# leosampaio/sketchformer

Hardware: AMD Instinct MI355X
Metric: stroke-tokens/sec training step, d_model=128 L=200 B=128, 1/2/4/8 GPU (higher is better)
Workload: dtype f32; 1 GPU; cfg2: sketch-transformer-tf2 4L/8H/d128/dff512 L=200 V=1004 C=345 dropout=0.1, fwd+bwd+Adam(WarmupDecay); global_batch=128, per_gpu_batch=128, seq_len=200, parallelism=dp1, hip_graph=0, dense_gemm_arithmetic=fp32 operands split exactly into 3 bf16 pieces, 6 product...

## Files before the change

### include/skf.h

```cpp
#ifndef SKF_H_
#define SKF_H_
#include <stddef.h>
#include <stdint.h>
#ifdef __cplusplus
extern "C" {
#endif

typedef void* skf_stream_t;

#define SKF_OK 0
#define SKF_EINVAL (-1)
#define SKF_EUNSUPPORTED (-2)
#define SKF_EHIP (-3)

const char* skf_last_error(void);
int skf_version(void);
int skf_device_info(char* name_host, size_t name_len, int* n_devices_host);

int skf_profiler_enable(int on);
int skf_profiler_report(char* buf_host, size_t len);

#define SKF_PREC_F32 0
#define SKF_PREC_BF16X3 3
#define SKF_PREC_BF16X6 6
// ... 25 lines not shown
                      int splits, float* bias_grad, int bias_grad_accumulate, void* workspace, size_t workspace_bytes,
                      int precision, const int* row_blocks, int row_block_rows, void* relu_bits_out, const void* relu_bits_in,
                      skf_stream_t stream);
int skf_gemm_ln_residual_supported(int M, int N, int K, int precision);
int skf_gemm_ln_residual_f32(int M, int N, int K, const float* A, int lda, const float* W, int ldw, const float* bias,
                             const float* x, const float* gamma, const float* beta, float* z, float* out, float* stats,
                             float rate, unsigned site, const void* step_state, int precision, skf_stream_t stream);
int skf_ffn_fused_supported(int M, int d, int dff, int precision);
size_t skf_ffn_image_bytes(int d, int dff, int precision);
size_t skf_ffn_relu_bits_bytes(int M, int d, int dff, int precision);
int skf_ffn_weight_images(int n, const float* const* W1, const int* ld1, const float* const* W2, const int* ld2,
                          const int* transpose, void* const* images, int d, int dff, int precision, skf_stream_t stream);
int skf_ffn_fused_fwd_f32(int M, int d, int dff, const float* x, const void* image, const float* b1, const float* b2,
                          float* h, void* relu_bits_out, const float* gamma, const float* beta, float* z, float* out,
                          float* stats, float rate, unsigned site, const void* step_state, int precision, skf_stream_t stream);
int skf_ffn_fused_bwd_f32(int M, int d, int dff, const float* dy, const void* image_t, const void* relu_bits_in,
                          float* dh, float* dx, int accumulate, const int* row_blocks, int row_block_rows,
                          int precision, skf_stream_t stream);
int skf_ffn_fused_fwd_proj_f32(int M, int d, int dff, const float* x, const void* image, const float* b1, const float* b2,
                               float* h, void* relu_bits_out, const float* gamma, const float* beta, float* z, float* out,
                               float* stats, float rate, unsigned site, const void* step_state, const void* proj_image,
                               const float* proj_bias, int proj_n, float* proj_out, int precision, skf_stream_t stream);
typedef struct SkfFfnBlockFwd {
  uint32_t struct_size; int32_t M, d, dff, precision;
  const float* x; const void* image; const float* b1; const float* b2; float* h; void* relu_bits_out;
  const float* gamma; const float* beta; float* z; float* out; float* stats;
  float rate; uint32_t site; const void* step_state;
  const void* pre_image; const float* pre_bias; const float* pre_residual; const float* pre_gamma; const float* pre_beta;
  float* pre_z; float* pre_out; float* pre_stats; uint32_t pre_site; int32_t proj_n;
  const void* proj_image; const float* proj_bias; float* proj_out;
} SkfFfnBlockFwd;
int skf_ffn_block_fwd_f32(const SkfFfnBlockFwd* block, skf_stream_t stream);
int skf_ffn_fused_ln_partials(int M);
int skf_ffn_fused_bwd_ln_f32(int M, int d, int dff, const float* dout, const float* z, const float* stats, const float* gamma,
                             float rate, unsigned site, const void* step_state, const void* image_t, const void* relu_bits_in,
                             float* dy, float* dh, float* dx, float* ln_partials, size_t ln_partials_bytes,
                             const int* row_blocks, int row_block_rows, int precision, skf_stream_t stream);
size_t skf_dense_image_bytes(int K, int N, int precision);
int skf_dense_weight_images(int n, const float* const* src, const int* ld, const int* transpose, const int* K, const int* N,
                            void* const* images, int precision, skf_stream_t stream);
int skf_layernorm_bwd_dgrad_supported(int M, int d, int precision);
int skf_layernorm_bwd_dgrad_partials(int M);
int skf_layernorm_bwd_dgrad_f32(int M, int d, const float* dout, const float* z, const float* stats, const float* gamma,
                                float rate, unsigned site, const void* step_state, const void* image_t, float* dz, float* dy,
                                float* da, float* ln_partials, size_t ln_partials_bytes, const int* row_blocks,
                                int row_block_rows, int precision, skf_stream_t stream);
int skf_layernorm_bwd_dgrad_lead_f32(int M, int d, const float* dout, const float* lead_a, const void* lead_image_t, const float* z,
                                     const float* stats, const float* gamma, float rate, unsigned site, const void* step_state,
                                     const void* image_t, float* dz, float* dy, float* da, float* ln_partials, size_t ln_partials_bytes,
                                     const int* row_blocks, int row_block_rows, int precision, skf_stream_t stream);
int skf_gemm_wgrad_partial_rows(int M, int N, int K, const float* A, int lda, const float* B, int ldb, int splits,
                                int with_bias_grad, float* slab, size_t slab_bytes, int* splits_used_host, int precision,
                                const int* row_blocks, int row_block_rows, skf_stream_t stream);
typedef struct SkfWgradProblem {
  const float* A; const float* B; float* slab; size_t slab_bytes; const int* row_blocks;
  int32_t M, N, K, lda, ldb, splits, with_bias_grad, row_block_rows, splits_used, pad;
} SkfWgradProblem;
int skf_gemm_wgrad_partial_group(SkfWgradProblem* probs, int n, int precision, skf_stream_t stream);
int skf_splitk_reduce(const float* slab, int splits, int M, int N, float* C, int ldc, int accumulate, float* bias_grad,
                      int bias_grad_accumulate, skf_stream_t stream);
int skf_splitk_reduce_blocks(int M, int N);
int skf_splitk_reduce_batch(const SkfReduceDesc* descs_dev, int ndesc, int total_blocks, skf_stream_t stream);

int skf_attention_fwd(const float* Q, int ldq, const float* K, int ldk, const float* V, int ldv,
                      const unsigned char* key_mask, int key_mask_ld, int causal, int B, int H, int Lq, int Lk, int dh,
                      float* O, int ldo, float* stats, int precision, skf_stream_t stream);
int skf_attention_bwd(const float* Q, int ldq, const float* K, int ldk, const float* V, int ldv, const float* O, int ldo,
                      const float* dO, int lddo, const float* stats, const unsigned char* key_mask, int key_mask_ld,
                      int causal, int B, int H, int Lq, int Lk, int dh, float* dQ, int lddq, float* dK, int lddk,
                      float* dV, int lddv, int precision, skf_stream_t stream);
int skf_attention_bwd_rows(const float* Q, int ldq, const float* K, int ldk, const float* V, int ldv, const float* O, int ldo,
                           const float* dO, int lddo, const float* stats, const unsigned char* key_mask, int key_mask_ld,
                           int causal, int B, int H, int Lq, int Lk, int dh, float* dQ, int lddq, float* dK, int lddk,
                           float* dV, int lddv, int precision, const int* q_live_len, skf_stream_t stream);
int skf_sample_order(const unsigned char* mask_a, int lda, int La, const unsigned char* mask_b, int ldb, int Lb, int B, int* order,
                     skf_stream_t stream);
int skf_attention_fwd_ordered(const float* Q, int ldq, const float* K, int ldk, const float* V, int ldv,
                              const unsigned char* key_mask, int key_mask_ld, int causal, int B, int H, int Lq, int Lk, int dh,
                              float* O, int ldo, float* stats, int precision, const int* sample_order, skf_stream_t stream);
int skf_attention_bwd_ordered(const float* Q, int ldq, const float* K, int ldk, const float* V, int ldv, const float* O, int ldo,
                              const float* dO, int lddo, const float* stats, const unsigned char* key_mask, int key_mask_ld,
                              int causal, int B, int H, int Lq, int Lk, int dh, float* dQ, int lddq, float* dK, int lddk,
                              float* dV, int lddv, int precision, const int* q_live_len, const int* sample_order, skf_stream_t stream);
int skf_attention_weights(const float* Q, int ldq, const float* K, int ldk, const unsigned char* key_mask, int key_mask_ld,
                          int causal, int B, int H, int Lq, int Lk, int dh, float* W, skf_stream_t stream);
int skf_attention_fwd_float_mask(const float* Q, int ldq, const float* K, int ldk, const float* V, int ldv, const float* mask,
                                 long mask_stride_b, long mask_stride_h, long mask_stride_q, int B, int H, int Lq, int Lk, int dh,
                                 float* O, int ldo, float* W, skf_stream_t stream);
int skf_row_mean(const float* a, const float* b, long rows, int cols, int mode, float* out, skf_stream_t stream);

int skf_embed_fwd(const long long* tokens, int tok_ld, int B, int L, const float* table, int vocab, int d,
                  const float* pos, float* out, float rate, unsigned site, const void* step_state, skf_stream_t stream);
int skf_embed_bwd(const long long* tokens, int tok_ld, int B, int L, const float* dx, int vocab, int d, float* dtable,
                  float rate, unsigned site, const void* step_state, skf_stream_t stream);
size_t skf_embed_sort_workspace_bytes(int B, int L, int vocab);
int skf_embed_sort(const long long* tokens, int tok_ld, int B, int L, int vocab, float* zero_table, int d, void* ws,
                   size_t ws_bytes, skf_stream_t stream);
int skf_embed_bwd_sorted(const void* ws, int B, int L, const float* dx, int vocab, int d, float* dtable, float rate,
                         unsigned site, const void* step_state, skf_stream_t stream);
int skf_padding_mask(const long long* tokens, int tok_ld, int B, int L, unsigned char* out, skf_stream_t stream);

int skf_layernorm_residual_fwd(const float* x, float* y_inout_z, const float* gamma, const float* beta, float* out,
                               float* stats, int rows, int d, float rate, unsigned site, const void* step_state,
                               skf_stream_t stream);
size_t skf_layernorm_bwd_workspace_bytes(int rows, int d);
int skf_layernorm_residual_bwd(const float* dout, const float* z, const float* stats, const float* gamma, float* dz,
                               float* dy, float* dgamma, float* dbeta, int rows, int d, float rate, unsigned site,
                               const void* step_state, void* workspace, size_t workspace_bytes, skf_stream_t stream);
int skf_layernorm_residual_bwd_rows(const float* dout, const float* z, const float* stats, const float* gamma, float* dz,
                                    float* dy, float* dgamma, float* dbeta, int rows, int d, float rate, unsigned site,
                                    const void* step_state, void* workspace, size_t workspace_bytes, const int* live_len,
                                    int rows_per_sample, skf_stream_t stream);
int skf_colsum(const float* in, int nrows, int ld, int ncols, float* out, int accumulate, skf_stream_t stream);

int skf_softmax_ce(float* logits, int ld, int rows, int ncls, const long long* target, int tgt_ld, int tgt_cols,
                   int tgt_off, int mask_pad, float scale, float* row_loss, float* row_hit, float* probs_out,
                   int write_grad, skf_stream_t stream);
int skf_metrics_update(const float* recon_loss, const float* recon_hit, int recon_rows, float recon_weight,
                       const float* class_loss, const float* class_hit, int class_rows, float class_weight,
                       const float* recon_scalar ,
                       float* metrics, skf_stream_t stream);

int skf_padding_mask_continuous(const float* x, int x_ld_rows, int B, int L, unsigned char* out, skf_stream_t stream);
int skf_embed_continuous_fwd(const float* x, int x_ld_rows, int B, int L, const float* W, const float* bias, int d,
                             const float* pos, float* out, float rate, unsigned site, const void* step_state,
                             skf_stream_t stream);
size_t skf_embed_continuous_bwd_workspace_bytes(int rows, int d);
int skf_embed_continuous_bwd(const float* x, int x_ld_rows, int B, int L, const float* dx, int d, float* dW, float* dbias,
                             float rate, unsigned site, const void* step_state, void* workspace, size_t workspace_bytes,
                             skf_stream_t stream);
int skf_continuous_loss(float* pred_inout_grad, const float* target, int tgt_ld_rows, int tgt_cols, int tgt_off, int rows,
                        float weight, float* row_loc, float* row_ce, float* row_mask, float* scalars, int write_grad,
                        skf_stream_t stream);

int skf_pool_fwd(const float* u, const float* Vw, const float* x, int B, int L, int U, int d, float* a_out, float* emb,
                 skf_stream_t stream);
int skf_pool_bwd(float* u_inout_dpre, const float* Vw, const float* x, const float* a, const float* demb, int B, int L,
                 int U, int d, float* dx, float* dV, void* workspace, size_t workspace_bytes, skf_stream_t stream);
int skf_expander_fwd(const float* emb, const float* w, const float* bias, int B, int L, int d, float* pre,
                     skf_stream_t stream);
int skf_expander_bwd(const float* dpre, const float* emb, const float* w, int B, int L, int d, float* demb,
                     int demb_accumulate, float* dw, float* dbias, void* workspace, size_t workspace_bytes,
                     skf_stream_t stream);

size_t skf_step_state_bytes(void);
int skf_step_prologue(void* step_state, int schedule, float p0, float p1, float p2, float p3, float beta1, float beta2,
                      unsigned seed, skf_stream_t stream);
int skf_step_epilogue(void* step_state, skf_stream_t stream);
unsigned skf_step_drop_key(unsigned seed, long long iterations, unsigned micro);
int skf_adam_step(float* w, const float* g, float* m, float* v, size_t n, const void* step_state, float grad_scale,
                  float beta1, float beta2, float eps, skf_stream_t stream);
int skf_sgd_momentum_step(float* w, const float* g, float* velocity, size_t n, const void* step_state, float grad_scale,
                          float momentum, skf_stream_t stream);
#define SKF_MICRO_KEEP 0
#define SKF_MICRO_NEXT 1
#define SKF_MICRO_ZERO 2
int skf_grad_accumulate(float* dst, const float* a, const float* b, size_t n, void* step_state, int micro_op, skf_stream_t stream);
int skf_weight_average_validate(float decay);
float skf_ema_decay_at(float decay, int num_updates, long long iterations);
int skf_ema_update(float* shadow, const float* w, size_t n, float decay, int num_updates, const void* step_state, const void* skip,
                   skf_stream_t stream);
int skf_buffer_swap(float* a, float* b, size_t n, skf_stream_t stream);

int skf_dropout(const float* x, float* y, size_t n, float rate, unsigned site, const void* step_state, skf_stream_t stream);
int skf_dropout_keep_mask(unsigned drop_key, unsigned site, float rate, size_t n, unsigned char* out_host);

// ... 358 lines not shown
```

### sketchformer_amd/_lib.py

```python
import ctypes as C
import os

HERE = os.path.dirname(os.path.abspath(__file__))
LIB_PATH = os.path.join(HERE, "libskf.so")

SKF_OK = 0
PREC_F32, PREC_BF16X3, PREC_BF16X6 = 0, 3, 6


def default_precision():
    e = os.environ.get("SKF_GEMM_PRECISION", "bf16x6").lower()
    try:
        return {"f32": PREC_F32, "bf16x6": PREC_BF16X6, "bf16x3": PREC_BF16X3, "0": 0, "3": 3, "6": 6}[e]
    except KeyError:
        raise ValueError("SKF_GEMM_PRECISION must be f32, bf16x6 or bf16x3 (got %r)" % e)


class SkfError(RuntimeError):
    pass


ATTN_TWO_PASS = 0x100
MODEL_DECODE_LAYERWISE = 1
MODEL_FFN_LAUNCHES = 2
# ... 65 lines not shown

    def __init__(self, *args, **kw):
        super().__init__(*args, **kw)
        if not self.struct_size:
            self.struct_size = C.sizeof(SkfPrefix)


class SkfReduceDesc(C.Structure):
    _fields_ = [("slab", C.c_void_p), ("C", C.c_void_p), ("bias_grad", C.c_void_p),
                ("splits", C.c_int32), ("M", C.c_int32), ("N", C.c_int32), ("ldc", C.c_int32), ("block_begin", C.c_int32),
                ("pad", C.c_int32)]


class SkfCastDesc(C.Structure):
    _fields_ = [("src", C.c_void_p), ("dst", C.c_void_p), ("dst_t", C.c_void_p),
                ("R", C.c_int32), ("C", C.c_int32), ("ld_src", C.c_int32), ("ld_dst", C.c_int32), ("ld_t", C.c_int32),
                ("block_begin", C.c_int32), ("blocks_x", C.c_int32), ("pad", C.c_int32)]


MICRO_KEEP, MICRO_NEXT, MICRO_ZERO = 0, 1, 2
ACCUM_FIRST, ACCUM_ADD, ACCUM_CLOSE, ACCUM_RESET = 0, 1, 2, 3
BEAM_MAX = 8


class SkfParamEntry(C.Structure):
    _fields_ = [("name", C.c_char * 96), ("offset", C.c_int64), ("rows", C.c_int32), ("cols", C.c_int32),
                ("row_stride", C.c_int32)]


_P = C.c_void_p
_I = C.c_int
_F = C.c_float
_Z = C.c_size_t
_U = C.c_uint
_L = C.c_longlong
_D = C.c_double

SIGNATURES = {
    "skf_last_error": (C.c_char_p, []),
    "skf_version": (_I, []),
    "skf_device_info": (_I, [C.c_char_p, _Z, C.POINTER(_I)]),
    "skf_profiler_enable": (_I, [_I]),
    "skf_profiler_report": (_I, [C.c_char_p, _Z]),
    "skf_gemm_workspace_bytes": (_Z, [_I, _I, _I, _I, _I]),
    "skf_gemm_default_splits": (_I, [_I, _I, _I]),
    "skf_gemm_wgrad_partial": (_I, [_I, _I, _I, _P, _I, _P, _I, _I, _I, _P, _Z, _P, _I, _P]),
    "skf_gemm_wgrad_partial_group": (_I, [_P, _I, _I, _P]),
    "skf_gemm_wgrad_partial_rows": (_I, [_I, _I, _I, _P, _I, _P, _I, _I, _I, _P, _Z, _P, _I, _P, _I, _P]),
    "skf_gemm_f32_rows": (_I, [_I, _I, _I, _I, _I, _P, _I, _P, _I, _P, _I, _P, _I, _P, _I, _I, _I, _P, _I, _P, _Z, _I, _P, _I, _P]),
    "skf_gemm_relu_bits_bytes": (_Z, [_I, _I, _I, _I]),
    "skf_gemm_f32_bits": (_I, [_I, _I, _I, _I, _I, _P, _I, _P, _I, _P, _I, _P, _I, _P, _I, _I, _I, _P, _I, _P, _Z, _I, _P, _I, _P, _P, _P]),
    "skf_gemm_ln_residual_supported": (_I, [_I, _I, _I, _I]),
    "skf_gemm_ln_residual_f32": (_I, [_I, _I, _I, _P, _I, _P, _I, _P, _P, _P, _P, _P, _P, _P, _F, _U, _P, _I, _P]),
    "skf_ffn_fused_supported": (_I, [_I, _I, _I, _I]),
    "skf_ffn_image_bytes": (_Z, [_I, _I, _I]),
    "skf_ffn_relu_bits_bytes": (_Z, [_I, _I, _I, _I]),
    "skf_ffn_weight_images": (_I, [_I, _P, _P, _P, _P, _P, _P, _I, _I, _I, _P]),
    "skf_ffn_fused_fwd_f32": (_I, [_I, _I, _I, _P, _P, _P, _P, _P, _P, _P, _P, _P, _P, _P, _F, _U, _P, _I, _P]),
    "skf_ffn_fused_bwd_f32": (_I, [_I, _I, _I, _P, _P, _P, _P, _P, _I, _P, _I, _I, _P]),
    "skf_ffn_fused_ln_partials": (_I, [_I]),
    "skf_ffn_fused_bwd_ln_f32": (_I, [_I, _I, _I, _P, _P, _P, _P, _F, _U, _P, _P, _P, _P, _P, _P, _P, _Z, _P, _I, _I, _P]),
    "skf_dense_image_bytes": (_Z, [_I, _I, _I]),
    "skf_dense_weight_images": (_I, [_I, _P, _P, _P, _P, _P, _P, _I, _P]),
    "skf_layernorm_bwd_dgrad_supported": (_I, [_I, _I, _I]),
    "skf_layernorm_bwd_dgrad_partials": (_I, [_I]),
    "skf_layernorm_bwd_dgrad_f32": (_I, [_I, _I, _P, _P, _P, _P, _F, _U, _P, _P, _P, _P, _P, _P, _Z, _P, _I, _I, _P]),
    "skf_layernorm_bwd_dgrad_lead_f32": (_I, [_I, _I, _P, _P, _P, _P, _P, _P, _F, _U, _P, _P, _P, _P, _P, _P, _Z, _P, _I, _I, _P]),
    "skf_ffn_fused_fwd_proj_f32": (_I, [_I, _I, _I, _P, _P, _P, _P, _P, _P, _P, _P, _P, _P, _P, _F, _U, _P, _P, _P, _I, _P, _I, _P]),
    "skf_ffn_block_fwd_f32": (_I, [C.POINTER(SkfFfnBlockFwd), _P]),
    "skf_target_live_len": (_I, [_P, _I, _I, _I, _P, _P]),
    "skf_row_blocks_bytes": (_Z, [_I, _I]),
    "skf_row_blocks_build": (_I, [_P, _I, _I, _I, _P, _P]),
    "skf_splitk_reduce": (_I, [_P, _I, _I, _I, _P, _I, _I, _P, _I, _P]),
    "skf_splitk_reduce_blocks": (_I, [_I, _I]),
    "skf_splitk_reduce_batch": (_I, [_P, _I, _I, _P]),
    "skf_gemm_f32": (_I, [_I, _I, _I, _I, _I, _P, _I, _P, _I, _P, _I, _P, _I, _P, _I, _I, _I, _P, _I, _P, _Z, _I, _P]),
    "skf_attention_fwd": (_I, [_P, _I, _P, _I, _P, _I, _P, _I, _I, _I, _I, _I, _I, _I, _P, _I, _P, _I, _P]),
    "skf_attention_bwd": (_I, [_P, _I, _P, _I, _P, _I, _P, _I, _P, _I, _P, _P, _I, _I, _I, _I, _I, _I, _I,
                               _P, _I, _P, _I, _P, _I, _I, _P]),
    "skf_attention_bwd_rows": (_I, [_P, _I, _P, _I, _P, _I, _P, _I, _P, _I, _P, _P, _I, _I, _I, _I, _I, _I, _I, _P, _I, _P, _I, _P, _I, _I, _P, _P]),
    "skf_attention_fwd_ordered": (_I, [_P, _I, _P, _I, _P, _I, _P, _I, _I, _I, _I, _I, _I, _I, _P, _I, _P, _I, _P, _P]),
    "skf_attention_bwd_ordered": (_I, [_P, _I, _P, _I, _P, _I, _P, _I, _P, _I, _P, _P, _I, _I, _I, _I, _I, _I, _I, _P, _I, _P, _I, _P, _I, _I, _P, _P, _P]),
    "skf_sample_order": (_I, [_P, _I, _I, _P, _I, _I, _I, _P, _P]),
    "skf_attention_weights": (_I, [_P, _I, _P, _I, _P, _I, _I, _I, _I, _I, _I, _I, _P, _P]),
    "skf_attention_fwd_float_mask": (_I, [_P, _I, _P, _I, _P, _I, _P, C.c_long, C.c_long, C.c_long, _I, _I, _I, _I, _I, _P, _I, _P, _P]),
    "skf_row_mean": (_I, [_P, _P, C.c_long, _I, _I, _P, _P]),
    "skf_embed_fwd": (_I, [_P, _I, _I, _I, _P, _I, _I, _P, _P, _F, _U, _P, _P]),
    "skf_embed_bwd": (_I, [_P, _I, _I, _I, _P, _I, _I, _P, _F, _U, _P, _P]),
    "skf_embed_sort_workspace_bytes": (_Z, [_I, _I, _I]),
    "skf_embed_sort": (_I, [_P, _I, _I, _I, _I, _P, _I, _P, _Z, _P]),
    "skf_embed_bwd_sorted": (_I, [_P, _I, _I, _P, _I, _I, _P, _F, _U, _P, _P]),
    "skf_padding_mask": (_I, [_P, _I, _I, _I, _P, _P]),
    "skf_layernorm_residual_fwd": (_I, [_P, _P, _P, _P, _P, _P, _I, _I, _F, _U, _P, _P]),
    "skf_layernorm_bwd_workspace_bytes": (_Z, [_I, _I]),
    "skf_layernorm_residual_bwd": (_I, [_P, _P, _P, _P, _P, _P, _P, _P, _I, _I, _F, _U, _P, _P, _Z, _P]),
    "skf_layernorm_residual_bwd_rows": (_I, [_P, _P, _P, _P, _P, _P, _P, _P, _I, _I, _F, _U, _P, _P, _Z, _P, _I, _P]),
    "skf_colsum": (_I, [_P, _I, _I, _I, _P, _I, _P]),
    "skf_softmax_ce": (_I, [_P, _I, _I, _I, _P, _I, _I, _I, _I, _F, _P, _P, _P, _I, _P]),
    "skf_metrics_update": (_I, [_P, _P, _I, _F, _P, _P, _I, _F, _P, _P, _P]),
    "skf_padding_mask_continuous": (_I, [_P, _I, _I, _I, _P, _P]),
    "skf_embed_continuous_fwd": (_I, [_P, _I, _I, _I, _P, _P, _I, _P, _P, _F, _U, _P, _P]),
    "skf_embed_continuous_bwd_workspace_bytes": (_Z, [_I, _I]),
    "skf_embed_continuous_bwd": (_I, [_P, _I, _I, _I, _P, _I, _P, _P, _F, _U, _P, _P, _Z, _P]),
    "skf_continuous_loss": (_I, [_P, _P, _I, _I, _I, _I, _F, _P, _P, _P, _P, _I, _P]),
    "skf_pool_fwd": (_I, [_P, _P, _P, _I, _I, _I, _I, _P, _P, _P]),
    "skf_pool_bwd": (_I, [_P, _P, _P, _P, _P, _I, _I, _I, _I, _P, _P, _P, _Z, _P]),
    "skf_expander_fwd": (_I, [_P, _P, _P, _I, _I, _I, _P, _P]),
    "skf_expander_bwd": (_I, [_P, _P, _P, _I, _I, _I, _P, _I, _P, _P, _P, _Z, _P]),
    "skf_config_size": (_Z, []),
    "skf_model_set_flags": (_I, [_P, C.c_uint32]),
    "skf_step_state_bytes": (_Z, []),
    "skf_step_prologue": (_I, [_P, _I, _F, _F, _F, _F, _F, _F, _U, _P]),
    "skf_step_epilogue": (_I, [_P, _P]),
    "skf_step_drop_key": (_U, [_U, _L, _U]),
    "skf_adam_step": (_I, [_P, _P, _P, _P, _Z, _P, _F, _F, _F, _F, _P]),
    "skf_sgd_momentum_step": (_I, [_P, _P, _P, _Z, _P, _F, _F, _P]),
    "skf_grad_accumulate": (_I, [_P, _P, _P, _Z, _P, _I, _P]),
    "skf_weight_average_validate": (_I, [_F]),
    "skf_ema_decay_at": (_F, [_F, _I, _L]),
    "skf_ema_update": (_I, [_P, _P, _Z, _F, _I, _P, _P, _P]),
    "skf_buffer_swap": (_I, [_P, _P, _Z, _P]),
    "skf_segment_plan_chunks": (_I, [_P, _I]),
    "skf_segment_plan_bytes": (_Z, [_I, _I]),
    "skf_segment_plan_build": (_I, [_P, _I, _P, _Z]),
    "skf_segment_norms_workspace_bytes": (_Z, [_I, _I]),
    "skf_segment_stats_floats": (_Z, [_I]),
    "skf_gradient_clip_validate": (_I, [_I, _F, _F]),
    "skf_segment_norms": (_I, [_P, _P, _I, _I, _F, _I, _F, _I, _P, _Z, _P, _P]),
    "skf_segment_scale": (_I, [_P, _P, _I, _I, _P, _P, _P]),
    "skf_adam_step_clipped": (_I, [_P, _P, _P, _P, _Z, _P, _F, _P, _F, _P, _F, _F, _F, _I, _P]),
    "skf_sgd_momentum_step_clipped": (_I, [_P, _P, _P, _Z, _P, _F, _P, _F, _P, _F, _I, _P]),
    "skf_dropout": (_I, [_P, _P, _Z, _F, _U, _P, _P]),
    "skf_dropout_keep_mask": (_I, [_U, _U, _F, _Z, _P]),
    "skf_attention_decode": (_I, [_P, _I, _P, _P, _I, C.c_longlong, _P, _I, _P, _I, _I, _I, _I, _I, _P, _I, _P, _P, _P, _I,
                                  _I, _P]),
    "skf_decode_init": (_I, [_P, _I, _P, _I, _P, _I, _P, _P, _I, C.c_longlong, _P, _P]),
    "skf_decode_embed": (_I, [_P, _P, _I, _I, _P, _I, _P, _P, _I, _P, _P, _P, _P]),
    "skf_decode_select_tokens": (_I, [_P, _I, _I, _I, _I, _I, C.c_longlong, _P, _I, _P, _I, _P, _P, _P, _P, _P]),
    "skf_sample_uniform": (_F, [_U, _U, _U]),
    "skf_decode_sample_tokens": (_I, [_P, _I, _I, _I, _I, _I, C.c_longlong, _P, _I, _P, _I, _P, _P, _P, _P, C.POINTER(SkfSampling), _P, _P]),
    "skf_decode_select_continuous": (_I, [_P, _I, _I, _I, _I, _P, _I, _P, _I, _P, _P, _P, _P]),
    "skf_gemm_bf16": (_I, [_I, _I, _I, _P, _I, _P, _I, _P, _I, _P, _I, _P, _I, _I, _P, _I, _P]),
    "skf_gemm_bf16_tile_rows": (_I, [_I, _I, _I, _I]),
    "skf_gemm_bf16_rows": (_I, [_I, _I, _I, _P, _I, _P, _I, _P, _I, _P, _I, _P, _I, _I, _P, _I, _P, _I, _P]),
    "skf_gemm_bf16_relu_bits_bytes": (_Z, [_I, _I]),
    "skf_gemm_bf16_bits": (_I, [_I, _I, _I, _P, _I, _P, _I, _P, _I, _P, _I, _P, _I, _I, _P, _I, _P, _I, _P, _P, _I, _P]),
    "skf_gemm_bf16_wgrad_rows": (_I, [_I, _I, _I, _P, _I, _P, _I, _P, _I, _P, _P, _Z, _P, _P]),
    "skf_gemm_bf16_wgrad_partial_rows": (_I, [_I, _I, _I, _P, _I, _P, _I, _I, _I, _P, _Z, _P, _P, _P]),
    "skf_gemm_bf16_wgrad_splits": (_I, [_I, _I, _I]),
    "skf_gemm_bf16_wgrad_workspace_bytes": (_Z, [_I, _I, _I, _I]),
    "skf_gemm_bf16_wgrad_partial": (_I, [_I, _I, _I, _P, _I, _P, _I, _I, _I, _P, _Z, _P, _P]),
    "skf_gemm_bf16_wgrad": (_I, [_I, _I, _I, _P, _I, _P, _I, _P, _I, _P, _P, _Z, _P]),
    "skf_attention_bf16_fwd": (_I, [_P, _I, _P, _I, _P, _I, _P, _I, _I, _I, _I, _I, _I, _I, _P, _I, _P, _P, _P]),
    "skf_attention_bf16_bwd_workspace_bytes": (_Z, [_I, _I, _I]),
    "skf_attention_bf16_bwd": (_I, [_P, _I, _P, _I, _P, _I, _P, _I, _P, _P, _I, _P, _P, _I, _I, _I, _I, _I, _I, _I,
                                    _P, _I, _P, _I, _P, _I, _P, _Z, _P]),
    "skf_attention_bf16_bwd_rows": (_I, [_P, _I, _P, _I, _P, _I, _P, _I, _P, _P, _I, _P, _P, _I, _I, _I, _I, _I, _I, _I, _P, _I, _P, _I, _P, _I, _P, _Z, _P, _P]),
    "skf_attention_bf16_fwd_ordered": (_I, [_P, _I, _P, _I, _P, _I, _P, _I, _I, _I, _I, _I, _I, _I, _P, _I, _P, _P, _P, _P]),
    "skf_attention_bf16_bwd_ordered": (_I, [_P, _I, _P, _I, _P, _I, _P, _I, _P, _P, _I, _P, _P, _I, _I, _I, _I, _I, _I, _I, _P, _I, _P, _I, _P, _I, _P, _Z, _P, _P, _P]),
    "skf_embed_fwd_bf16": (_I, [_P, _I, _I, _I, _P, _I, _I, _P, _P, _F, _U, _P, _P]),
    "skf_embed_bwd_sorted_bf16": (_I, [_P, _I, _I, _P, _I, _I, _P, _F, _U, _P, _P]),
    "skf_layernorm_residual_fwd_bf16": (_I, [_P, _P, _P, _P, _P, _P, _I, _I, _F, _U, _P, _P]),
    "skf_layernorm_bwd_bf16_workspace_bytes": (_Z, [_I, _I]),
    "skf_layernorm_residual_bwd_bf16": (_I, [_P, _P, _P, _P, _P, _P, _P, _P, _I, _I, _F, _U, _P, _P, _Z, _P]),
    "skf_layernorm_residual_bwd_bf16_rows": (_I, [_P, _P, _P, _P, _P, _P, _P, _P, _I, _I, _F, _U, _P, _P, _Z, _P, _I, _P]),
    "skf_softmax_ce_bf16": (_I, [_P, _I, _I, _I, _P, _I, _I, _I, _I, _F, _P, _P, _I, _P]),
# ... 118 lines not shown
```

### sketchformer_amd/csrc/skf_attention.hip

```cpp
#include <stdlib.h>
#include "skf_common.h"
#include <type_traits>
#include "skf_attention_params.h"

namespace {


__device__ __forceinline__ f32x4 mfma16(float a, float b, f32x4 c) {
  return __builtin_amdgcn_mfma_f32_16x16x4f32(a, b, c, 0, 0, 0);
}

typedef __bf16 attn_bf16x8 __attribute__((ext_vector_type(8)));
typedef unsigned attn_u32x4 __attribute__((ext_vector_type(4)));
typedef unsigned attn_u32x2 __attribute__((ext_vector_type(2)));
__device__ __forceinline__ f32x4 mfma_bf16(attn_u32x4 a, attn_u32x4 b, f32x4 c) {
  return __builtin_amdgcn_mfma_f32_16x16x32_bf16(__builtin_bit_cast(attn_bf16x8, a), __builtin_bit_cast(attn_bf16x8, b), c, 0, 0, 0);
}
constexpr int KPP = 32;

template <int DH, int MAXT, bool SPLIT>
__global__ __launch_bounds__(256, MAXT <= 13 ? 4 : 1) void attn_fwd_kernel(AttnParams p) {
  static_assert(!SPLIT || DH == 16, "split S^T path is written for dh = 16");
  constexpr int NC = DH / 16;
  constexpr int LD = SPLIT ? 3 * KPP / 4 : DH + 4;
  extern __shared__ __attribute__((aligned(16))) float smem[];
  int bh = skf_xcd_remap(blockIdx.x, gridDim.x);
  if (p.order) { const int k = skf_deal_rank(blockIdx.x, p.H); bh = min(max(p.order[k / p.H], 0), p.B - 1) * p.H + k % p.H; }
  const int b = bh / p.H, h = bh % p.H;
  const int nkt = (p.Lk + 15) >> 4, nqt = (p.Lq + 15) >> 4;
  const int VP = nkt * 16 + 8;
  float* Ks = smem;
  float* Vt = smem + nkt * 16 * LD;
  float* Ms = Vt + DH * VP;
  int* Tf = reinterpret_cast<int*>(Ms + nkt * 16);
  int* last_valid = Tf + nkt;
  const SkfSplitSel sel = skf_split_sel();
  const int tid = threadIdx.x, lane = tid & 63;
  const int wave = __builtin_amdgcn_readfirstlane(tid >> 6);
  const int i = lane & 15, g = lane >> 4;

  constexpr int NQ = SPLIT ? 2 : NC;
  float4 qnext[NQ];
  auto load_q = [&](int qt_, float4 (&dst)[NQ]) {
    const int row = qt_ * 16 + i, rc = row < p.Lq ? row : p.Lq - 1;
    const float* qp = p.Q + (size_t)(b * p.Lq + rc) * p.ldq + h * DH;
#pragma unroll
    for (int c = 0; c < NQ; ++c) {
      const float4 v = *reinterpret_cast<const float4*>(qp + (SPLIT ? (g & 1) * 8 + 4 * c : c * 16 + g * 4));
      dst[c] = row < p.Lq ? v : make_float4(0.f, 0.f, 0.f, 0.f);
    }
  };
  load_q((wave + bh) & 3, qnext);
  const int last_key = p.Lk - 1;
  const unsigned char* kmp = p.key_mask ? p.key_mask + (size_t)b * p.key_mask_ld
                                        : reinterpret_cast<const unsigned char*>(p.K + (size_t)b * p.Lk * p.ldk);
  const unsigned char mk0 = kmp[min(tid, last_key)];
  constexpr int SB = 4;
  const int stage_total = nkt * 16 * (DH / 4);
  for (int e0 = tid; e0 < stage_total; e0 += 256 * SB) {
    float4 kvb[SB], vvb[SB];
#pragma unroll
    for (int u = 0; u < SB; ++u) {
      const int e = e0 + u * 256, rc = min(e / (DH / 4), last_key), c4 = (e % (DH / 4)) * 4;
      kvb[u] = *reinterpret_cast<const float4*>(p.K + (size_t)(b * p.Lk + rc) * p.ldk + h * DH + c4);
      vvb[u] = *reinterpret_cast<const float4*>(p.V + (size_t)(b * p.Lk + rc) * p.ldv + h * DH + c4);
    }
#pragma unroll
    for (int u = 0; u < SB; ++u) {
      const int e = e0 + u * 256, row = e / (DH / 4), c4 = (e % (DH / 4)) * 4;
      if (e >= stage_total) continue;
      float4 kv = kvb[u], vv = vvb[u];
      if (row >= p.Lk) { kv = make_float4(0.f, 0.f, 0.f, 0.f); vv = kv; }
      if constexpr (SPLIT) {
        unsigned lo[3], hi[3];
        skf_split2<3>(kv.x, kv.y, lo, sel);
        skf_split2<3>(kv.z, kv.w, hi, sel);
        char* kp = reinterpret_cast<char*>(Ks);
#pragma unroll
        for (int q = 0; q < 3; ++q)
          *reinterpret_cast<attn_u32x2*>(kp + (size_t)q * nkt * 16 * KPP + row * KPP + c4 * 2) = (attn_u32x2){lo[q], hi[q]};
      } else {
        *reinterpret_cast<float4*>(&Ks[row * LD + c4]) = kv;
      }
      Vt[(c4 + 0) * VP + row] = vv.x; Vt[(c4 + 1) * VP + row] = vv.y; Vt[(c4 + 2) * VP + row] = vv.z; Vt[(c4 + 3) * VP + row] = vv.w;
    }
  }
  {
    int lv = -1;
    auto mask_keys = [&](int key0 , unsigned char mb) {
      const int key = key0 + lane;
      float mv = -INFINITY;
      if (key < p.Lk) mv = (p.key_mask && mb) ? -1e9f : 0.f;
      if (key < nkt * 16) Ms[key] = mv;
      const unsigned long long open = __ballot(mv == 0.f), masked = __ballot(key < nkt * 16 && mv != 0.f);
      if (open) lv = key0 + 63 - __builtin_clzll(open);
      const int t = (key0 >> 4) + (lane & 3);
      if (lane < 4 && t < nkt) Tf[t] = ((unsigned)(masked >> (16 * (lane & 3))) & 0xffffu) != 0u;
    };
    mask_keys(64 * wave, mk0);
    if constexpr (MAXT * 16 > 256)
      for (int key0 = 64 * wave + 256; key0 < nkt * 16; key0 += 256) mask_keys(key0, kmp[min(key0 + lane, last_key)]);
    if (lane == 0) last_valid[wave] = lv;
  }
  __syncthreads();

  const bool can_skip = p.causal && Ms[0] == 0.f;
  const int lastk = max(max(last_valid[0], last_valid[1]), max(last_valid[2], last_valid[3]));
  const int nkt_eff = (lastk >= 0 && (!p.causal || can_skip)) ? (lastk >> 4) + 1 : nkt;
  const float c2 = 1.44269504088896340736f / sqrtf((float)DH);

  const char* kp = reinterpret_cast<const char*>(Ks);
  const int plane_b = nkt * 16 * KPP, lane_k = i * KPP + (g & 1) * 16;
  const char* ka3 = kp + (g < 2 ? plane_b : 0) + lane_k;
  const char* ka2 = kp + (g < 2 ? plane_b : 2 * plane_b) + lane_k;
  const char* ka1 = kp + lane_k;
  const __amdgpu_buffer_rsrc_t o_rsrc = __builtin_amdgcn_make_buffer_rsrc(p.O + (size_t)b * p.Lq * p.ldo, 0, (unsigned)(p.Lq * p.ldo) * 4u, 0x00020000);
  const __amdgpu_buffer_rsrc_t st_rsrc = __builtin_amdgcn_make_buffer_rsrc(p.stats ? p.stats + (size_t)bh * p.Lq * 2 : p.O, 0,
                                                                           p.stats ? (unsigned)p.Lq * 8u : 0u, 0x00020000);
  for (int qt = (wave + bh) & 3; qt < nqt; qt += 4) {
    const int q0 = qt * 16, qrow = q0 + i;
    const bool qok = qrow < p.Lq;
    float4 qcur[NQ];
#pragma unroll
    for (int c = 0; c < NQ; ++c) qcur[c] = qnext[c];
    load_q(qt + 4, qnext);
    float4 qf[NC];
    attn_u32x4 qb1, qb2, qb3;
    if constexpr (SPLIT) {
      const float4 qa = make_float4(qcur[0].x * c2, qcur[0].y * c2, qcur[0].z * c2, qcur[0].w * c2);
      const float4 qc = make_float4(qcur[1].x * c2, qcur[1].y * c2, qcur[1].z * c2, qcur[1].w * c2);
      unsigned d0[3], d1[3], d2[3], d3[3];
      skf_split2<3>(qa.x, qa.y, d0, sel); skf_split2<3>(qa.z, qa.w, d1, sel);
      skf_split2<3>(qc.x, qc.y, d2, sel); skf_split2<3>(qc.z, qc.w, d3, sel);
      const attn_u32x4 p0 = {d0[0], d1[0], d2[0], d3[0]}, p1 = {d0[1], d1[1], d2[1], d3[1]}, p2 = {d0[2], d1[2], d2[2], d3[2]};
      const bool first = g < 2;
      qb1 = first ? p0 : p1; qb2 = p0; qb3 = first ? p1 : p2;
    } else {
#pragma unroll
      for (int c = 0; c < NC; ++c) qf[c] = qcur[c];
    }
    const int nt = min(can_skip ? qt + 1 : nkt, nkt_eff);
    float s[MAXT][4];
    float mx = -INFINITY;
#pragma unroll
    for (int kt = 0; kt < MAXT; ++kt) {
      if (kt < nt) {
        f32x4 acc = {0.f, 0.f, 0.f, 0.f};
        if constexpr (SPLIT) {
          const attn_u32x4 a3 = *reinterpret_cast<const attn_u32x4*>(ka3 + kt * 16 * KPP);
          const attn_u32x4 a2 = *reinterpret_cast<const attn_u32x4*>(ka2 + kt * 16 * KPP);
          const attn_u32x4 a1 = *reinterpret_cast<const attn_u32x4*>(ka1 + kt * 16 * KPP);
          acc = mfma_bf16(a3, qb3, acc);
          acc = mfma_bf16(a2, qb2, acc);
          acc = mfma_bf16(a1, qb1, acc);
        } else {
#pragma unroll
          for (int c = 0; c < NC; ++c) {
            const float4 kf = *reinterpret_cast<const float4*>(&Ks[(kt * 16 + i) * LD + c * 16 + g * 4]);
            acc = mfma16(kf.x, qf[c].x, acc);
            acc = mfma16(kf.y, qf[c].y, acc);
            acc = mfma16(kf.z, qf[c].z, acc);
            acc = mfma16(kf.w, qf[c].w, acc);
          }
        }
        const bool need_mask = __builtin_amdgcn_readfirstlane(Tf[kt]) != 0 || (p.causal && kt >= qt);
        if (need_mask) {
          const float4 m4 = *reinterpret_cast<const float4*>(&Ms[kt * 16 + g * 4]);
          const float mr[4] = {m4.x, m4.y, m4.z, m4.w};
#pragma unroll
          for (int r = 0; r < 4; ++r) {
            const int key = kt * 16 + g * 4 + r;
            const float m = fminf(mr[r], (p.causal && key > qrow) ? -1e9f : 0.f);
            const float v = m < 0.f ? m : (SPLIT ? acc[r] : acc[r] * c2);
            s[kt][r] = v;
            mx = fmaxf(mx, v);
          }
        } else {
#pragma unroll
          for (int r = 0; r < 4; ++r) { s[kt][r] = SPLIT ? acc[r] : acc[r] * c2; mx = fmaxf(mx, s[kt][r]); }
        }
      }
    }
    mx = fmaxf(mx, __shfl_xor(mx, 16, 64));
    mx = fmaxf(mx, __shfl_xor(mx, 32, 64));
    float sum = 0.f;
    f32x4 o[NC];
#pragma unroll
    for (int c = 0; c < NC; ++c) o[c] = (f32x4){0.f, 0.f, 0.f, 0.f};
#pragma unroll
    for (int kt = 0; kt < MAXT; ++kt)
      if (kt < nt) {
        float pe[4];
#pragma unroll
        for (int r = 0; r < 4; ++r) { pe[r] = __builtin_amdgcn_exp2f(s[kt][r] - mx); sum += pe[r]; }
#pragma unroll
        for (int c = 0; c < NC; ++c) {
          const float4 vt = *reinterpret_cast<const float4*>(&Vt[(c * 16 + i) * VP + kt * 16 + g * 4]);
          o[c] = mfma16(vt.x, pe[0], o[c]);
          o[c] = mfma16(vt.y, pe[1], o[c]);
          o[c] = mfma16(vt.z, pe[2], o[c]);
          o[c] = mfma16(vt.w, pe[3], o[c]);
        }
      }
    sum += __shfl_xor(sum, 16, 64);
    sum += __shfl_xor(sum, 32, 64);
    const float rinv = 1.0f / sum;
#pragma unroll
    for (int c = 0; c < NC; ++c) {
      const f32x4 ov = {o[c][0] * rinv, o[c][1] * rinv, o[c][2] * rinv, o[c][3] * rinv};
      __builtin_amdgcn_raw_buffer_store_b128(__builtin_bit_cast(attn_u32x4, ov), o_rsrc,
                                             qok ? (unsigned)(qrow * p.ldo + h * DH + c * 16 + g * 4) * 4u : 0x7ffffff0u, 0, 0);
    }
    __builtin_amdgcn_raw_buffer_store_b64((attn_u32x2){__builtin_bit_cast(unsigned, mx), __builtin_bit_cast(unsigned, rinv)}, st_rsrc,
                                          (qok && g == 0) ? (unsigned)qrow * 8u : 0x7ffffff0u, 0, 0);
  }
}

constexpr int kAttnBwdWaves = 2;
template <int DH, int KTW, bool CAUSAL>
__global__ __launch_bounds__(256, kAttnBwdWaves) void attn_bwd_kernel(AttnParams p) {
  constexpr int NC = DH / 16;
  constexpr int LD = DH + 4;
  constexpr int TLD = 20;
  extern __shared__ __attribute__((aligned(16))) float smem[];
  int bh = skf_xcd_remap(blockIdx.x, gridDim.x);
  if (p.order) { const int k = skf_deal_rank(blockIdx.x, p.H); bh = min(max(p.order[k / p.H], 0), p.B - 1) * p.H + k % p.H; }
  const int b = bh / p.H, h = bh % p.H;
  const int nkt = (p.Lk + 15) >> 4, nqt_all = (p.Lq + 15) >> 4;
  const int nqt = p.q_live ? min(nqt_all, (max(p.q_live[b], 0) + 15) >> 4) : nqt_all;
  const int QR = nqt_all * 16;
  constexpr int RLD = DH + 1;
  float* Qs = smem;
  float* dOs = Qs + QR * LD;
  float* Red = dOs + QR * LD;
  float* Mx = Red + 2 * 4 * 16 * RLD;
  float* Ri = Mx + QR;
  float* Dl = Ri + QR;
  float* Tr = Dl + QR;
  const int tid = threadIdx.x, lane = tid & 63;
  const int wave = __builtin_amdgcn_readfirstlane(tid >> 6);
  const int i = lane & 15, g = lane >> 4;

  const unsigned char* km = p.key_mask ? p.key_mask + (size_t)b * p.key_mask_ld : nullptr;
  const int last_row = p.Lk - 1;
  const unsigned char* kmp = km ? km : reinterpret_cast<const unsigned char*>(p.K + (size_t)b * p.Lk * p.ldk);
  const int wv = (wave + bh) & 3;
  float4 kb[KTW][NC], vb[KTW][NC];
  float kraw[KTW][NC][4];
// ... 210 lines not shown
          *reinterpret_cast<float4*>(p.dV + (size_t)(b * p.Lk + krow) * p.lddv + h * DH + c * 16 + g * 4) =
              make_float4(dVt[j][c][0], dVt[j][c][1], dVt[j][c][2], dVt[j][c][3]);
        }
      }
    }
  };
  kg_pass(0, std::true_type());
  for (int kg = 4 * KTW; kg < nkt; kg += 4 * KTW) kg_pass(kg, std::false_type());
  __syncthreads();
  if (!CAUSAL && KTW > 1 && nkt == 4 * (KTW - 1) + 1) {
    float* sh = Qs + wave * 2 * DH * 16;
#pragma unroll
    for (int c = 0; c < NC; ++c)
#pragma unroll
      for (int r = 0; r < 4; ++r) {
        sh[(c * 16 + g * 4 + r) * 16 + i] = dK_shared[c][r];
        sh[DH * 16 + (c * 16 + g * 4 + r) * 16 + i] = dV_shared[c][r];
      }
    __syncthreads();
    const int krow0 = (nkt - 1) * 16;
    for (int e = tid; e < 2 * DH * 16; e += 256) {
      const int which = e / (DH * 16), dd = (e % (DH * 16)) / 16, kk = e % 16;
      const float v = Qs[e] + Qs[2 * DH * 16 + e] + Qs[4 * DH * 16 + e] + Qs[6 * DH * 16 + e];
      if (krow0 + kk < p.Lk) {
        float* dst = which ? p.dV : p.dK;
        const int ld = which ? p.lddv : p.lddk;
        dst[(size_t)(b * p.Lk + krow0 + kk) * ld + h * DH + dd] = v;
      }
    }
    __syncthreads();
  }
}

size_t fwd_smem(int DH, int Lk, bool split) {
  const size_t n16 = (size_t)(Lk + 15) / 16 * 16;
  const size_t krow = split ? 3 * KPP / 4 : DH + 4;
  return (n16 * krow + (size_t)DH * (n16 + 8) + n16 + n16 / 16 + 4) * sizeof(float);
}
size_t bwd_smem(int DH, int Lq) {
  const size_t QR = (size_t)(Lq + 15) / 16 * 16;
  return (2 * QR * (DH + 4) + (size_t)2 * 4 * 16 * (DH + 1) + 3 * QR + (size_t)4 * (64 / DH) * 16 * 20 + 4) * sizeof(float);
}

template <typename K>
int set_smem(K kfn, size_t bytes) {
  SKF_HIP(hipFuncSetAttribute((const void*)kfn, hipFuncAttributeMaxDynamicSharedMemorySize, (int)bytes));
  return SKF_OK;
}

inline bool mfma_head(int dh) { return dh == 16 || dh == 32 || dh == 64; }
bool fwd_split(int dh, int precision) { return dh == 16 && precision != SKF_PREC_F32; }
int check_common(const AttnParams& p, int dh) {
  SKF_CHECK_ARG(mfma_head(dh) || skf_attention_any_supported(dh, p.Lq, p.Lk), "head dim must be 16, 32, 64 (MFMA kernels) or any size <= 128 with sequences <= 1024 (fallback)");
  SKF_CHECK_ARG(p.B > 0 && p.H > 0 && p.Lq > 0 && p.Lk > 0, "empty problem");
  SKF_CHECK_ARG((p.ldq & 3) == 0 && (p.ldk & 3) == 0 && (p.ldv & 3) == 0 && (p.ldo & 3) == 0, "row strides must be multiples of 4");
  SKF_CHECK_ARG(!p.causal || p.Lq == p.Lk, "causal attention needs Lq == Lk");
  return SKF_OK;
}

}

int skf_attention_fwd_max_lk(int dh, int precision) {
  int best = 0;
  for (int L = 16; L <= 512; L += 16)
    if (fwd_smem(dh, L, fwd_split(dh, precision)) <= kAttnLdsBytes) best = L;
  return best;
}
int skf_attention_bwd_max_lq(int dh) {
  int best = 0;
  for (int L = 16; L <= 512; L += 16)
    if (bwd_smem(dh, L) <= kAttnLdsBytes) best = L;
  return best;
}

extern "C" int skf_attention_fwd(const float* Q, int ldq, const float* K, int ldk, const float* V, int ldv,
                                 const unsigned char* key_mask, int key_mask_ld, int causal, int B, int H, int Lq, int Lk,
                                 int dh, float* O, int ldo, float* stats, int precision, skf_stream_t stream) {
  return skf_attention_fwd_ordered(Q, ldq, K, ldk, V, ldv, key_mask, key_mask_ld, causal, B, H, Lq, Lk, dh, O, ldo, stats, precision, nullptr, stream);
}

extern "C" int skf_attention_fwd_ordered(const float* Q, int ldq, const float* K, int ldk, const float* V, int ldv,
                                         const unsigned char* key_mask, int key_mask_ld, int causal, int B, int H, int Lq, int Lk,
                                         int dh, float* O, int ldo, float* stats, int precision, const int* sample_order, skf_stream_t stream) {
  AttnParams p{};
  p.order = (B & 7) == 0 ? sample_order : nullptr;
  p.Q = Q; p.K = K; p.V = V; p.O = O; p.ldq = ldq; p.ldk = ldk; p.ldv = ldv; p.ldo = ldo;
  p.key_mask = key_mask; p.key_mask_ld = key_mask_ld; p.causal = causal; p.B = B; p.H = H; p.Lq = Lq; p.Lk = Lk; p.stats = stats;
  int rc = check_common(p, dh);
  if (rc) return rc;
  SKF_CHECK_ARG(Q && K && V && O, "null operand");
  if (!mfma_head(dh)) return skf_attention_fwd_any(p, dh, (hipStream_t)stream);
  SKF_CHECK_ARG(Lk <= 512, "Lk > 512 not supported");
  SKF_CHECK_ARG((double)Lq * ldo * 4 < 2147483648.0, "one sample's output rows exceed 32-bit byte offsets");
  const bool split = fwd_split(dh, precision);
  const size_t smem = fwd_smem(dh, Lk, split);
  SKF_CHECK_ARG(smem <= kAttnLdsBytes, "K/V of one head do not fit in LDS");
  hipStream_t st = (hipStream_t)stream;
  dim3 grid(B * H), block(256);
#define SKF_ATTN_FWD(DHV, MT, SP)                               \
  {                                                             \
    auto kfn = attn_fwd_kernel<DHV, MT, SP>;                    \
    if ((rc = set_smem(kfn, smem))) return rc;                  \
    hipLaunchKernelGGL(kfn, grid, block, smem, st, p);          \
  }
  static const char* const tags[3] = {"attn_fwd<dh16>", "attn_fwd<dh32>", "attn_fwd<dh64>"};
  const double visited = skf_prof_attention_fraction(key_mask, key_mask_ld, causal, B, Lq, Lk, nullptr, 16, 16);
  SkfProfScope ps(st, tags[dh == 16 ? 0 : dh == 32 ? 1 : 2], 4.0 * B * H * (double)Lq * Lk * dh,
                  4.0 * B * H * dh * (2.0 * Lq + 2.0 * Lk));
  ps.done(4.0 * B * H * (double)Lq * Lk * dh * visited, 4.0 * B * H * dh * (2.0 * Lq + 2.0 * Lk));
  const bool small = Lk <= 208;
  if (dh == 16 && split) { if (small) SKF_ATTN_FWD(16, 13, true) else SKF_ATTN_FWD(16, 32, true) }
  else if (dh == 16) { if (small) SKF_ATTN_FWD(16, 13, false) else SKF_ATTN_FWD(16, 32, false) }
  else if (dh == 32) { if (small) SKF_ATTN_FWD(32, 13, false) else SKF_ATTN_FWD(32, 32, false) }
  else { if (small) SKF_ATTN_FWD(64, 13, false) else SKF_ATTN_FWD(64, 32, false) }
#undef SKF_ATTN_FWD
  SKF_LAUNCH_CHECK();
  return SKF_OK;
}

extern "C" int skf_attention_bwd(const float* Q, int ldq, const float* K, int ldk, const float* V, int ldv,
                                 const float* O, int ldo, const float* dO, int lddo, const float* stats,
                                 const unsigned char* key_mask, int key_mask_ld, int causal, int B, int H, int Lq, int Lk,
                                 int dh, float* dQ, int lddq, float* dK, int lddk, float* dV, int lddv, int precision, skf_stream_t stream) {
  return skf_attention_bwd_ordered(Q, ldq, K, ldk, V, ldv, O, ldo, dO, lddo, stats, key_mask, key_mask_ld, causal, B, H, Lq, Lk, dh, dQ, lddq,
                                   dK, lddk, dV, lddv, precision, nullptr, nullptr, stream);
}

extern "C" int skf_attention_bwd_rows(const float* Q, int ldq, const float* K, int ldk, const float* V, int ldv,
                                      const float* O, int ldo, const float* dO, int lddo, const float* stats,
                                      const unsigned char* key_mask, int key_mask_ld, int causal, int B, int H, int Lq, int Lk,
                                      int dh, float* dQ, int lddq, float* dK, int lddk, float* dV, int lddv, int precision,
                                      const int* q_live_len, skf_stream_t stream) {
  return skf_attention_bwd_ordered(Q, ldq, K, ldk, V, ldv, O, ldo, dO, lddo, stats, key_mask, key_mask_ld, causal, B, H, Lq, Lk, dh, dQ, lddq,
                                   dK, lddk, dV, lddv, precision, q_live_len, nullptr, stream);
}

extern "C" int skf_attention_bwd_ordered(const float* Q, int ldq, const float* K, int ldk, const float* V, int ldv,
                                         const float* O, int ldo, const float* dO, int lddo, const float* stats,
                                         const unsigned char* key_mask, int key_mask_ld, int causal, int B, int H, int Lq, int Lk,
                                         int dh, float* dQ, int lddq, float* dK, int lddk, float* dV, int lddv, int precision,
                                         const int* q_live_len, const int* sample_order, skf_stream_t stream) {
  const bool two_pass = (precision & SKF_ATTN_TWO_PASS) != 0;
  precision &= ~SKF_ATTN_TWO_PASS;
  AttnParams p{};
  p.order = (B & 7) == 0 ? sample_order : nullptr;
  p.q_live = q_live_len;
  p.Q = Q; p.K = K; p.V = V; p.O = const_cast<float*>(O); p.ldq = ldq; p.ldk = ldk; p.ldv = ldv; p.ldo = ldo;
  p.key_mask = key_mask; p.key_mask_ld = key_mask_ld; p.causal = causal; p.B = B; p.H = H; p.Lq = Lq; p.Lk = Lk;
  p.stats = const_cast<float*>(stats);
  p.dO = dO; p.lddo = lddo; p.dQ = dQ; p.dK = dK; p.dV = dV; p.lddq = lddq; p.lddk = lddk; p.lddv = lddv;
  int rc = check_common(p, dh);
  if (rc) return rc;
  SKF_CHECK_ARG(Q && K && V && O && dO && stats && dQ && dK && dV, "null operand");
  SKF_CHECK_ARG((lddo & 3) == 0 && (lddq & 3) == 0 && (lddk & 3) == 0 && (lddv & 3) == 0, "row strides must be multiples of 4");
  if (!mfma_head(dh)) return skf_attention_bwd_any(p, dh, (hipStream_t)stream);
  SKF_CHECK_ARG(Lk <= 512, "Lk > 512 not supported");
  const bool split_mode = precision != SKF_PREC_F32;
  if (skf_attention_bwd3_supported(dh, Lq, Lk) && split_mode && !two_pass) return skf_attention_bwd3_launch(p, (hipStream_t)stream);
  const bool bwd2_shape = (dh == 16 && two_pass) || (dh == 32 && Lk <= 256 && Lq <= 256);
  if (bwd2_shape && split_mode && Lq <= 512) return skf_attention_bwd2_launch(p, dh, (hipStream_t)stream);
  const size_t smem = bwd_smem(dh, Lq);
  SKF_CHECK_ARG(smem <= kAttnLdsBytes, "Q/dO/dQ of one head do not fit in LDS");
  hipStream_t st = (hipStream_t)stream;
  dim3 grid(B * H), block(256);
#define SKF_ATTN_BWD(DHV)                                       \
  {                                                             \
    if (causal) {                                               \
      auto kfn = attn_bwd_kernel<DHV, 64 / DHV, true>;          \
      if ((rc = set_smem(kfn, smem))) return rc;                \
      hipLaunchKernelGGL(kfn, grid, block, smem, st, p);        \
    } else {                                                    \
      auto kfn = attn_bwd_kernel<DHV, 64 / DHV, false>;         \
      if ((rc = set_smem(kfn, smem))) return rc;                \
      hipLaunchKernelGGL(kfn, grid, block, smem, st, p);        \
    }                                                           \
  }
  static const char* const tags[3] = {"attn_bwd<dh16>", "attn_bwd<dh32>", "attn_bwd<dh64>"};
  const double visited = skf_prof_attention_fraction(key_mask, key_mask_ld, causal, B, Lq, Lk, q_live_len, 16, 16);
  SkfProfScope ps(st, tags[dh == 16 ? 0 : dh == 32 ? 1 : 2], 8.0 * B * H * (double)Lq * Lk * dh,
                  4.0 * B * H * dh * (4.0 * Lq + 4.0 * Lk));
  ps.done(8.0 * B * H * (double)Lq * Lk * dh * visited, 4.0 * B * H * dh * (4.0 * Lq + 4.0 * Lk));
  if (dh == 16) SKF_ATTN_BWD(16) else if (dh == 32) SKF_ATTN_BWD(32) else SKF_ATTN_BWD(64)
#undef SKF_ATTN_BWD
  SKF_LAUNCH_CHECK();
  return SKF_OK;
}
```

### sketchformer_amd/csrc/skf_attention_bwd3.hip

```cpp
#include <stdlib.h>
#include "skf_attention_params.h"

namespace {

typedef __bf16 b3_bf16x8 __attribute__((ext_vector_type(8)));
typedef unsigned b3_u32x8 __attribute__((ext_vector_type(8)));
typedef unsigned b3_u32x4 __attribute__((ext_vector_type(4)));
typedef unsigned b3_u32x2 __attribute__((ext_vector_type(2)));
typedef short b3_s4 __attribute__((ext_vector_type(4)));

constexpr int RP = 32;
constexpr int MAXT = 13;
constexpr int RMAX = MAXT * 16;
constexpr int PB = RMAX * RP;
constexpr int K_OFF = 0, V_OFF = 3 * PB, Q_OFF = 6 * PB, G_OFF = 9 * PB;
constexpr int NMX_OFF = 12 * PB, NDL_OFF = NMX_OFF + RMAX * 4, KBITS_OFF = NDL_OFF + RMAX * 4, CTL_OFF = KBITS_OFF + 16 * 4;
constexpr int SMEM_BYTES = CTL_OFF + 16 + 32;
constexpr float kLog2e = 1.44269504088896340736f, kLn2 = 0.69314718055994530942f;

__device__ __forceinline__ f32x4 mfma_x(b3_u32x4 a, b3_u32x4 b, f32x4 c) {
  return __builtin_amdgcn_mfma_f32_16x16x32_bf16(__builtin_bit_cast(b3_bf16x8, a), __builtin_bit_cast(b3_bf16x8, b), c, 0, 0, 0);
}
#define SKF_LDS(T, a) (*reinterpret_cast<T __attribute__((address_space(3)))*>(static_cast<uintptr_t>(a)))
__device__ __forceinline__ b3_u32x2 tr_read(unsigned a) {
  const b3_s4 v = __builtin_amdgcn_ds_read_tr16_b64_v4i16(reinterpret_cast<b3_s4 __attribute__((address_space(3)))*>(static_cast<uintptr_t>(a)));
  return __builtin_bit_cast(b3_u32x2, v);
}
__device__ __forceinline__ b3_u32x4 rd128(unsigned a) { return SKF_LDS(const b3_u32x4, a); }
__device__ __forceinline__ b3_u32x4 cat(b3_u32x2 a, b3_u32x2 b) { return (b3_u32x4){a[0], a[1], b[0], b[1]}; }

struct YOps { b3_u32x4 y00, y11, y20; };
__device__ __forceinline__ YOps y_ops(unsigned base , bool first) {
  YOps o;
  o.y00 = rd128(base);
  o.y11 = rd128(base + PB);
  o.y20 = rd128(base + (first ? 2 * PB : 0));
  return o;
}
__device__ __forceinline__ f32x4 dot_d(const b3_u32x4& x01, const b3_u32x4& x02, const YOps& y, f32x4 acc) {
  acc = mfma_x(x02, y.y20, acc);
  acc = mfma_x(x01, y.y11, acc);
  acc = mfma_x(x01, y.y00, acc);
  return acc;
}
struct TOps { b3_u32x4 x02, x11, x00; };
__device__ __forceinline__ TOps tr_ops(unsigned tr ) {
  TOps o;
  o.x02 = cat(tr_read(tr), tr_read(tr + 2 * PB));
  unsigned trb = tr;
  asm volatile("" : "+v"(trb));
  o.x11 = cat(tr_read(tr + PB), tr_read(trb + PB));
  unsigned trc = tr;
  asm volatile("" : "+v"(trc));
  o.x00 = cat(tr_read(trb), tr_read(trc));
  return o;
}
__device__ __forceinline__ f32x4 dot_rows(const TOps& t, const f32x4& y, f32x4 acc, const SkfSplitSel& sel) {
  unsigned lo[3], hi[3];
  skf_split2<3>(y[0], y[1], lo, sel);
  skf_split2<3>(y[2], y[3], hi, sel);
  const b3_u32x4 y01 = {lo[0], hi[0], lo[1], hi[1]}, y20 = {lo[2], hi[2], lo[0], hi[0]};
  acc = mfma_x(t.x02, y20, acc);
  acc = mfma_x(t.x11, y01, acc);
  acc = mfma_x(t.x00, y01, acc);
  return acc;
}

__device__ __forceinline__ void put_planes(unsigned dst, int row, int c4, const float4& v, const SkfSplitSel& sel) {
  unsigned lo[3], hi[3];
  skf_split2<3>(v.x, v.y, lo, sel);
  skf_split2<3>(v.z, v.w, hi, sel);
#pragma unroll
  for (int q = 0; q < 3; ++q) SKF_LDS(b3_u32x2, dst + q * PB + row * RP + c4 * 2) = (b3_u32x2){lo[q], hi[q]};
}
__device__ __forceinline__ float4 scaled(const float4& v, float s) { return make_float4(v.x * s, v.y * s, v.z * s, v.w * s); }

template <bool CAUSAL>
__global__ __launch_bounds__(512, 4) void attn_bwd3_kernel(AttnParams p) {
  extern __shared__ __attribute__((aligned(16))) char smem[];
  const int nkt = (p.Lk + 15) >> 4, nqt_all = (p.Lq + 15) >> 4;
  constexpr unsigned sbase = 0u;
  if ((unsigned)(uintptr_t)(__attribute__((address_space(3))) char*)smem != sbase) __builtin_trap();
  unsigned* Kbits = reinterpret_cast<unsigned*>(smem + KBITS_OFF);
  int* ctl = reinterpret_cast<int*>(smem + CTL_OFF);
  int* kscan = ctl + 4;
  const SkfSplitSel sel = skf_split_sel();
  const int tid = threadIdx.x, lane = tid & 63;
  const int wave = __builtin_amdgcn_readfirstlane(tid >> 6);
  const int j = lane & 15, g = lane >> 4;
  const bool first = g < 2;
  const float c2 = kLog2e * 0.25f;
  int bh = skf_xcd_remap(blockIdx.x, gridDim.x);
  if (p.order) { const int k = skf_deal_rank(blockIdx.x, p.H); bh = min(max(p.order[k / p.H], 0), p.B - 1) * p.H + k % p.H; }
  const int b = bh / p.H, h = bh % p.H;
  const int nqt = p.q_live ? min(nqt_all, (max(p.q_live[b], 0) + 15) >> 4) : nqt_all;
  const unsigned char mb = p.key_mask ? p.key_mask[(size_t)b * p.key_mask_ld + min(tid, p.Lk - 1)] : (unsigned char)0;
  if (tid == 256) { ctl[1] = 0; ctl[2] = 8; }
  if (wave < 4) {
    const unsigned long long padded = __ballot(tid < p.Lk && mb != 0), open = __ballot(tid < p.Lk && mb == 0);
    const unsigned word = (unsigned)(padded >> (16 * (lane & 3))) & 0xffffu;
    if (lane < 4) Kbits[4 * wave + lane] = word;
    const unsigned tiles = (unsigned)__ballot(lane < 4 && word != 0u);
    if (lane == 0) { kscan[wave] = (int)(tiles << (4 * wave)); kscan[4 + wave] = open ? 64 * wave + 63 - __builtin_clzll(open) : -1; }
  }
  __syncthreads();
  const b3_u32x4 kw = *reinterpret_cast<const b3_u32x4*>(kscan), lw = *reinterpret_cast<const b3_u32x4*>(kscan + 4);
  const unsigned k_masked = __builtin_amdgcn_readfirstlane((kw[0] | kw[1]) | (kw[2] | kw[3])) | ((p.Lk & 15) ? 1u << (nkt - 1) : 0u);
  const int lastk = __builtin_amdgcn_readfirstlane(max(max((int)lw[0], (int)lw[1]), max((int)lw[2], (int)lw[3])));
  const bool can_skip = CAUSAL && !(Kbits[0] & 1u);
  const int nkt_eff = (lastk >= 0 && (!CAUSAL || can_skip)) ? (lastk >> 4) + 1 : nkt;
  float4 kv[2], vv[2], qv[2], gv[2], ov[2];
  float2 sv[2];
  {
    const float* Qb = p.Q + (size_t)b * p.Lq * p.ldq + h * 16;
    const float* Kb = p.K + (size_t)b * p.Lk * p.ldk + h * 16;
    const float* Vb = p.V + (size_t)b * p.Lk * p.ldv + h * 16;
    const float* Ob = p.O + (size_t)b * p.Lq * p.ldo + h * 16;
    const float* dOb = p.dO + (size_t)b * p.Lq * p.lddo + h * 16;
    const float2* stats = reinterpret_cast<const float2*>(p.stats) + (size_t)bh * p.Lq;
#pragma unroll
    for (int u = 0; u < 2; ++u) {
      const int e = tid + 512 * u, row = e >> 2, c4 = (e & 3) * 4;
      const int rk = min(row, p.Lk - 1), rq = min(row, p.Lq - 1);
      kv[u] = vv[u] = qv[u] = gv[u] = ov[u] = make_float4(0.f, 0.f, 0.f, 0.f);
      sv[u] = make_float2(0.f, 0.f);
      if (row < nkt_eff * 16) {
        kv[u] = *reinterpret_cast<const float4*>(Kb + (size_t)rk * p.ldk + c4);
        vv[u] = *reinterpret_cast<const float4*>(Vb + (size_t)rk * p.ldv + c4);
      }
      if (row < nqt * 16) {
        qv[u] = *reinterpret_cast<const float4*>(Qb + (size_t)rq * p.ldq + c4);
        gv[u] = *reinterpret_cast<const float4*>(dOb + (size_t)rq * p.lddo + c4);
        ov[u] = *reinterpret_cast<const float4*>(Ob + (size_t)rq * p.ldo + c4);
        sv[u] = stats[rq];
      }
    }
  }
#pragma unroll
  for (int u = 0; u < 2; ++u) {
    const int e = tid + 512 * u, row = e >> 2;
    const bool nz = row < p.Lq && (gv[u].x != 0.f || gv[u].y != 0.f || gv[u].z != 0.f || gv[u].w != 0.f);
    if (__ballot(nz) != 0ull && lane == 0 && (e >> 6) < nqt) atomicOr(reinterpret_cast<unsigned*>(&ctl[1]), 1u << (e >> 6));
  }
#pragma unroll
  for (int u = 0; u < 2; ++u) {
    const int e = tid + 512 * u, row = e >> 2, c4 = (e & 3) * 4;
    if (row < nkt_eff * 16) {
      const float z = row < p.Lk ? 1.f : 0.f;
      put_planes(sbase + K_OFF, row, c4, scaled(kv[u], z), sel);
      __builtin_amdgcn_sched_barrier(0);
      put_planes(sbase + V_OFF, row, c4, scaled(vv[u], z), sel);
      __builtin_amdgcn_sched_barrier(0);
    } else if (row < p.Lk) {
      *reinterpret_cast<float4*>(p.dK + (size_t)(b * p.Lk + row) * p.lddk + h * 16 + c4) = make_float4(0.f, 0.f, 0.f, 0.f);
      *reinterpret_cast<float4*>(p.dV + (size_t)(b * p.Lk + row) * p.lddv + h * 16 + c4) = make_float4(0.f, 0.f, 0.f, 0.f);
    }
    const bool qok = row < p.Lq;
    const float ri = qok ? sv[u].y : 0.f;
    float dl = gv[u].x * ov[u].x + gv[u].y * ov[u].y + gv[u].z * ov[u].z + gv[u].w * ov[u].w;
    dl += __shfl_xor(dl, 1, 64);
    dl += __shfl_xor(dl, 2, 64);
    if (row < nqt * 16) {
      put_planes(sbase + Q_OFF, row, c4, scaled(qv[u], qok ? c2 : 0.f), sel);
      __builtin_amdgcn_sched_barrier(0);
      put_planes(sbase + G_OFF, row, c4, scaled(gv[u], ri), sel);
      __builtin_amdgcn_sched_barrier(0);
      if (c4 == 0) { SKF_LDS(float, sbase + NMX_OFF + row * 4) = qok ? -sv[u].x : -INFINITY; SKF_LDS(float, sbase + NDL_OFF + row * 4) = qok ? -dl * ri : 0.f; }
    } else if (qok) {
      *reinterpret_cast<float4*>(p.dQ + (size_t)(b * p.Lq + row) * p.lddq + h * 16 + c4) = make_float4(0.f, 0.f, 0.f, 0.f);
    }
  }
  __syncthreads();
  const unsigned q_live = (unsigned)ctl[1];

  const int nA = nqt, nB = nkt_eff, nm = nA < nB ? nA : nB, n_items = nA + nB;
  const int lane_d = j * RP + (g & 1) * 16;
  const int x01 = lane_d + (first ? 0 : PB), x02 = lane_d + (first ? 0 : 2 * PB);
  const int lane_t = (4 * g + (j >> 2)) * RP + (j & 3) * 8;

  for (int item = wave; item < n_items;) {
    int is_b, t;
    if (item < 2 * nm) { is_b = !(item & 1); t = item >> 1; }
    else { is_b = nB > nA; t = nm + (item - 2 * nm); }
    if (!is_b) {
      const int qt = nA - 1 - t, q = qt * 16 + j;
      const bool live = ((q_live >> qt) & 1u) != 0u;
      const unsigned qrow = sbase + qt * 16 * RP + lane_d;
      const YOps qo = y_ops(qrow + Q_OFF, first), go = y_ops(qrow + G_OFF, first);
      const float nmx = SKF_LDS(const float, sbase + NMX_OFF + q * 4), ndl = SKF_LDS(const float, sbase + NDL_OFF + q * 4);
      const int nt = min(can_skip ? qt + 1 : nkt, live ? nkt_eff : 0);
      const f32x4 s_seed = {nmx, nmx, nmx, nmx}, d_seed = {ndl, ndl, ndl, ndl};
      f32x4 dq = {0.f, 0.f, 0.f, 0.f};
      unsigned a1 = sbase + x01, a2 = sbase + x02, tr = sbase + lane_t;
      for (int kt = 0; kt < nt; ++kt, a1 += 16 * RP, a2 += 16 * RP, tr += 16 * RP) {
        const f32x4 sacc = dot_d(rd128(a1 + K_OFF), rd128(a2 + K_OFF), qo, s_seed);
        const f32x4 dpacc = dot_d(rd128(a1 + V_OFF), rd128(a2 + V_OFF), go, d_seed);
        const TOps kw = tr_ops(tr + K_OFF);
        f32x4 ds;
        if (((k_masked >> kt) & 1u) || (CAUSAL && kt >= qt)) {
          const unsigned bits = __builtin_amdgcn_readfirstlane(Kbits[kt]);
          const float mx = -nmx;
#pragma unroll
          for (int r4 = 0; r4 < 4; ++r4) {
            const int key = kt * 16 + 4 * g + r4;
            float m = key < p.Lk ? (((bits >> (4 * g + r4)) & 1u) ? -1e9f : 0.f) : -INFINITY;
            if (CAUSAL && key > q) m = fminf(m, -1e9f);
            const float tt = m < 0.f ? m - mx : sacc[r4];
            ds[r4] = __builtin_amdgcn_exp2f(tt) * dpacc[r4];
          }
        } else {
#pragma unroll
          for (int r4 = 0; r4 < 4; ++r4) ds[r4] = __builtin_amdgcn_exp2f(sacc[r4]) * dpacc[r4];
        }
        dq = dot_rows(kw, ds, dq, sel);
      }
      if (q < p.Lq)
        *reinterpret_cast<float4*>(p.dQ + (size_t)(b * p.Lq + q) * p.lddq + h * 16 + 4 * g) =
            make_float4(dq[0] * 0.25f, dq[1] * 0.25f, dq[2] * 0.25f, dq[3] * 0.25f);
    } else {
      const int kt = t, key = kt * 16 + j;
      const unsigned krow = sbase + kt * 16 * RP + lane_d;
      const YOps ko = y_ops(krow + K_OFF, first), vo = y_ops(krow + V_OFF, first);
      const unsigned kbits = __builtin_amdgcn_readfirstlane(Kbits[kt]);
      const float kadd = key < p.Lk ? (((kbits >> j) & 1u) ? -1e9f : 0.f) : -INFINITY;
      const bool tile_masked = ((k_masked >> kt) & 1u) != 0u;
      f32x4 dkt = {0.f, 0.f, 0.f, 0.f}, dvt = dkt;
      const int qt0 = (CAUSAL && can_skip) ? kt : 0;
      unsigned a1 = sbase + Q_OFF + x01 + qt0 * 16 * RP, a2 = sbase + Q_OFF + x02 + qt0 * 16 * RP, tr = sbase + Q_OFF + lane_t + qt0 * 16 * RP;
      unsigned st = sbase + NMX_OFF + (qt0 * 16 + 4 * g) * 4;
      for (int qt = qt0; qt < nqt; ++qt, a1 += 16 * RP, a2 += 16 * RP, tr += 16 * RP, st += 64) {
        if (!((q_live >> qt) & 1u)) continue;
        const f32x4 s_seed = SKF_LDS(const f32x4, st), d_seed = SKF_LDS(const f32x4, st + (NDL_OFF - NMX_OFF));
        const f32x4 sacc = dot_d(rd128(a1), rd128(a2), ko, s_seed);
        const f32x4 dpacc = dot_d(rd128(a1 + 3 * PB), rd128(a2 + 3 * PB), vo, d_seed);
        const TOps gw = tr_ops(tr + 3 * PB), qw = tr_ops(tr);
        f32x4 pr, ds;
        if (tile_masked || (CAUSAL && kt >= qt)) {
#pragma unroll
          for (int r4 = 0; r4 < 4; ++r4) {
            const float m = CAUSAL ? fminf(kadd, key > qt * 16 + 4 * g + r4 ? -1e9f : 0.f) : kadd;
            const float tt = m < 0.f ? m + s_seed[r4] : sacc[r4];
            pr[r4] = __builtin_amdgcn_exp2f(tt);
            ds[r4] = pr[r4] * dpacc[r4];
          }
        } else {
#pragma unroll
          for (int r4 = 0; r4 < 4; ++r4) { pr[r4] = __builtin_amdgcn_exp2f(sacc[r4]); ds[r4] = pr[r4] * dpacc[r4]; }
        }
        dvt = dot_rows(gw, pr, dvt, sel);
        dkt = dot_rows(qw, ds, dkt, sel);
      }
      if (key < p.Lk) {
        *reinterpret_cast<float4*>(p.dK + (size_t)(b * p.Lk + key) * p.lddk + h * 16 + 4 * g) =
            make_float4(dkt[0] * kLn2, dkt[1] * kLn2, dkt[2] * kLn2, dkt[3] * kLn2);
        *reinterpret_cast<float4*>(p.dV + (size_t)(b * p.Lk + key) * p.lddv + h * 16 + 4 * g) = make_float4(dvt[0], dvt[1], dvt[2], dvt[3]);
      }
// ... 27 lines not shown
```

### sketchformer_amd/csrc/skf_attention_params.h

```cpp
#pragma once
#include "skf_common.h"

struct AttnParams {
  const float* Q; const float* K; const float* V; float* O;
  int ldq, ldk, ldv, ldo;
  const unsigned char* key_mask;
  int key_mask_ld;
  int causal;
  int B, H, Lq, Lk;
  float* stats;
  const float* dO; int lddo;
  float* dQ; float* dK; float* dV;
  int lddq, lddk, lddv;
  const int* order;
  const int* q_live;
};

constexpr size_t kAttnLdsBytes = 160 * 1024;
int skf_attention_fwd_max_lk(int dh, int precision);
int skf_attention_bwd_max_lq(int dh);
size_t skf_attention_bwd2_smem(int dh, int Lq, int Lk);

int skf_attention_bwd2_launch(const AttnParams& p, int dh, hipStream_t st);

int skf_attention_bwd3_supported(int dh, int Lq, int Lk);
int skf_attention_bwd3_launch(const AttnParams& p, hipStream_t st);

int skf_attention_any_supported(int dh, int Lq, int Lk);
int skf_attention_fwd_any(const AttnParams& p, int dh, hipStream_t st);
int skf_attention_bwd_any(const AttnParams& p, int dh, hipStream_t st);
```

### sketchformer_amd/csrc/skf_common.h

```cpp
#pragma once
#include <hip/hip_runtime.h>
#include <hip/hip_ext.h>
#include <stdint.h>
#include <stdio.h>
#include "../../include/skf.h"

typedef float f32x4 __attribute__((ext_vector_type(4)));
typedef float f32x16 __attribute__((ext_vector_type(16)));

#define SKF_WAVE 64

void skf_set_error(const char* fmt, ...);

#define SKF_CHECK_ARG(cond, msg)                                   \
  do {                                                             \
    if (!(cond)) {                                                 \
      skf_set_error("%s: %s (%s)", __func__, msg, #cond);          \
      return SKF_EINVAL;                                           \
    }                                                              \
  } while (0)

#define SKF_LAUNCH_CHECK()                                          \
  do {                                                              \
    hipError_t e__ = hipGetLastError();                             \
    if (e__ != hipSuccess) {                                        \
      skf_set_error("%s: launch failed: %s", __func__, hipGetErrorString(e__)); \
      return SKF_EHIP;                                              \
    }                                                               \
  } while (0)

#define SKF_HIP(call)                                               \
  do {                                                              \
    hipError_t e__ = (call);                                        \
    if (e__ != hipSuccess) {                                        \
      skf_set_error("%s: %s failed: %s", __func__, #call, hipGetErrorString(e__)); \
      return SKF_EHIP;                                              \
    }                                                               \
  } while (0)

struct SkfProfScope {
  SkfProfScope(hipStream_t st, const char* tag, double flops, double bytes);
  ~SkfProfScope();
  void done(double flops_done, double bytes_done);
  bool active() const { return idx_ >= 0; }
  hipStream_t st_;
  int idx_;
};
double skf_prof_list_fraction(const int* list);
double skf_prof_attention_fraction(const unsigned char* key_mask, int mask_ld, int causal, int B, int Lq, int Lk,
                                   const int* q_live, int qtile, int ktile);

int skf_adam_step_launch(float* w, const float* g, float* m, float* v, size_t n, void* step_state, float grad_scale, float beta1, float beta2,
                         float eps, int advance, hipStream_t stream);
int skf_pool_bwd_partials(float* u_inout_dpre, const float* Vw, const float* x, const float* a, const float* demb, int B, int L, int U, int d,
                          float* dx, float* dV_part, hipStream_t s);
int skf_expander_bwd_partials(const float* dpre, const float* emb, const float* w, int B, int L, int d, float* demb, int demb_accumulate,
                              float* p1, float* p2, hipStream_t s);
int skf_stage_inputs_launch(const void* inp, void* dinp, const void* tar, void* dtar, size_t row, size_t src_row, size_t copy, int batch,
                            const void* labels, void* dlabels, hipStream_t st, unsigned char* emask = nullptr, unsigned char* dmask = nullptr,
                            int mask_L = 0);
int skf_counts_to_offsets_launch(const int* counts, int N, long long* out_offsets, hipStream_t stream);

static inline int skf_cdiv(long a, long b) { return (int)((a + b - 1) / b); }

constexpr size_t skf_ws_align(size_t n) { return (n + 255) & ~(size_t)255; }
struct SkfWsCarver {
  uintptr_t base;
  size_t used = 0;
  explicit SkfWsCarver(void* ws) : base((uintptr_t)ws) {}
  template <class T> T* take(size_t count) { T* p = (T*)(base + used); used += skf_ws_align(count * sizeof(T)); return p; }
};

struct SkfTailSlot {
  hipEvent_t event = nullptr;
  bool attached = false;
};
extern thread_local SkfTailSlot skf_tls_tail;
struct SkfTailScope {
  explicit SkfTailScope(hipEvent_t e) : saved_(skf_tls_tail) { skf_tls_tail = SkfTailSlot{e, false}; }
  ~SkfTailScope() { skf_tls_tail = saved_; }
  SkfTailScope(const SkfTailScope&) = delete;
  SkfTailScope& operator=(const SkfTailScope&) = delete;
  bool attached() const { return skf_tls_tail.attached; }
 private:
  SkfTailSlot saved_;
};
inline hipEvent_t skf_tail_defer() { hipEvent_t e = skf_tls_tail.event; skf_tls_tail.event = nullptr; return e; }
inline void skf_tail_resume(hipEvent_t e) { skf_tls_tail.event = e; }
inline hipEvent_t skf_tail_attach() {
  hipEvent_t e = skf_tls_tail.event;
  if (e) skf_tls_tail = SkfTailSlot{nullptr, true};
  return e;
}
#define SKF_LAUNCH_TAIL(kernel, grid, block, smem, stream, ...)                                        \
  do {                                                                                                 \
    if (hipEvent_t ev__ = skf_tail_attach()) {                                                         \
      hipExtLaunchKernelGGL(kernel, grid, block, smem, stream, nullptr, ev__, 0, __VA_ARGS__);         \
    } else {                                                                                           \
      hipLaunchKernelGGL(kernel, grid, block, smem, stream, __VA_ARGS__);                              \
    }                                                                                                  \
  } while (0)

struct SkfOncePerDevice {
  unsigned long long done = 0;
  static int device() {
    int dev = 0;
    return (hipGetDevice(&dev) == hipSuccess && dev >= 0 && dev < 64) ? dev : -1;
  }
  bool needed() const {
    const int dev = device();
    return dev < 0 || !((__atomic_load_n(&done, __ATOMIC_ACQUIRE) >> dev) & 1ull);
  }
  void mark() {
    const int dev = device();
    if (dev >= 0) __atomic_fetch_or(&done, 1ull << dev, __ATOMIC_RELEASE);
  }
};

__device__ __forceinline__ int skf_xcd_remap(int orig, int nwg) {
  const int xcd = orig & 7, q = nwg >> 3, r = nwg & 7;
  return (xcd < r ? xcd * (q + 1) : r * (q + 1) + (xcd - r) * q) + (orig >> 3);
}
__device__ __forceinline__ void skf_part_major(int lid, int ngroups, int nparts, int* g, int* w) {
  constexpr int G = 32;
  const int chunk = lid / (G * nparts), j = lid - chunk * G * nparts;
  const int gc = min(G, ngroups - chunk * G);
  *w = j / gc;
  *g = chunk * G + j - *w * gc;
}
__device__ __forceinline__ int skf_deal_rank(int bid, int H) {
  const int x = bid & 7, i = bid >> 3, m = i / H;
  return (x + 8 * m) * H + (i - m * H);
}
__device__ __forceinline__ float wave_sum(float v) {
#pragma unroll
  for (int o = 32; o > 0; o >>= 1) v += __shfl_xor(v, o, 64);
  return v;
}
__device__ __forceinline__ double wave_sum(double v) {
#pragma unroll
  for (int o = 32; o > 0; o >>= 1) v += __shfl_xor(v, o, 64);
  return v;
}
// ... 72 lines not shown
```

### sketchformer_amd/csrc/skf_model_bwd.hip

```cpp
#include "skf_model_internal.h"

namespace skf_model_detail {
namespace {

template <typename F>
int with_ready_event(SkfModel* M, bool want, hipEvent_t* ready, F call) {
  hipEvent_t e = (want && may_park(M)) ? M->sched.take_event() : nullptr;
  bool rode = false;
  const int rc = with_tail_event(M, e, &rode, call);
  *ready = rode ? e : nullptr;
  return rc;
}

int ffn_bwd(SkfModel* M, const DenseP& f1, const DenseP& f2, const float* x_in, const float* h, const float* dy,
            float* dh, float* dx_acc, int rows, hipStream_t s, const void* hbits, const void* image_t) {
  if (M->ctx.ffn_fused) {
    SKF_TRY(dense_wgrad(M, f2, h, f2.in, dy, f2.out, rows, s));
    SKF_TRY(M->sched.before_write(M, dh, s));
    SKF_TRY(M->sched.before_write(M, dx_acc, s));
    const int* blocks = M->ctx.live_blocks(rows, 16);
    hipEvent_t ready = nullptr;
    SKF_TRY(with_ready_event(M, M->sched.holding(), &ready, [&] {
      return skf_ffn_fused_bwd_f32(rows, M->cfg.d_model, M->cfg.dff, dy, image_t, hbits, dh, dx_acc, 1, blocks, blocks ? 16 : 0,
                                   M->cfg.gemm_precision, s);
// ... 90 lines not shown
    SKF_CHECK_ARG(!lead_a && !lead_image_t, "a lead operand needs the fused launch");
    SKF_TRY(ln_bwd(M, ln, dout, z, st, dz, dy, rows, rate, site, s));
    SKF_TRY(dense_wgrad(M, o, a_in, d, dy, d, rows, s));
    return dense_dgrad(M, o, dy, d, rows, da, d, 0, nullptr, 0, s);
  }
  float* part = M->red.take_ln_partial(M);
  if (!part) return SKF_EINVAL;
  SKF_TRY(M->sched.before_write(M, dz, s));
  SKF_TRY(M->sched.before_write(M, dy, s));
  SKF_TRY(M->sched.before_write(M, da, s));
  const int* blocks = M->ctx.live_blocks(rows, 16);
  SKF_TRY(skf_layernorm_bwd_dgrad_lead_f32(rows, d, dout, lead_a, lead_image_t, z, st, M->P(ln.g), rate, site, M->state, image_t, dz, dy, da, part,
                                           pbytes, blocks, blocks ? 16 : 0, M->cfg.gemm_precision, s));
  SKF_TRY(ln_partials_desc(M, ln, part, skf_layernorm_bwd_dgrad_partials(rows)));
  return dense_wgrad(M, o, a_in, d, dy, d, rows, s);
}

int build_row_lists(SkfModel* M, hipStream_t s) {
  const SkfConfig& c = M->cfg;
  const Plan& P = M->plan;
  M->ctx.lists_built = false;
  if (c.continuous || !do_recon(c) || c.gemm_precision == SKF_PREC_F32) return SKF_OK;
  const int B = c.batch, Le = c.seq_len, Ld = c.seq_len - 1;
  SKF_TRY(skf_target_live_len(M->at<long long>(P.tar), Le, B, Ld, M->at<int>(P.live_len), s));
  SKF_TRY(skf_row_blocks_build(M->at<int>(P.live_len), B, Ld, 16, M->at<int>(P.live16), s));
  SKF_TRY(skf_row_blocks_build(M->at<int>(P.live_len), B, Ld, 32, M->at<int>(P.live32), s));
  M->ctx.lists_built = true;
  return SKF_OK;
}

}

int run_backward(SkfModel* M, hipStream_t s) {
  M->ctx.begin_backward();
  M->sched.begin_backward();
  M->red.begin_step();
  const SkfConfig& c = M->cfg;
  const Layout& L = M->lay;
  const Plan& P = M->plan;
  const int B = c.batch, Le = c.seq_len, Ld = c.seq_len - 1, d = c.d_model, H = c.num_heads, dh = d / H;
  const int Me = B * Le, Md = B * Ld, N = c.num_layers;
  const float rate = c.dropout_rate;
  const long long* inp = M->at<long long>(P.inp);
  const long long* tar = M->at<long long>(P.tar);
  const unsigned char* emask = M->at<unsigned char>(P.enc_mask);
  const unsigned char* dmask = M->at<unsigned char>(P.dec_mask);
  float* G = M->at<float>(P.gA);
  float* G2 = M->at<float>(P.gB);
  float* dO = M->at<float>(P.do_);
  float* dpre = M->at<float>(P.dpre);
  float* demb = M->at<float>(P.demb);
  int layer_no = 0;

  const bool bott = has_bott(c), cls = has_cls(c), recon = do_recon(c);
  float* enc_out = M->at<float>(P.enc[N - 1].x2);
  const float* pre = bott ? M->at<float>(P.pre) : enc_out;
  const bool dec_emb_on_side = recon && M->sched.side && !c.continuous && P.emb_sort_bytes;
  if (recon) {
  if (!M->ctx.lists_built) SKF_TRY(build_row_lists(M, s));
  if (M->ctx.lists_built) M->ctx.set_live(Md, M->at<int>(P.live_len), 16, M->at<int>(P.live16), 32, M->at<int>(P.live32));
  M->ctx.lists_built = false;
  const float* dlog = M->at<float>(P.logits);
  SKF_TRY(dense_wgrad(M, L.out, M->at<float>(P.dec[N - 1].out3), d, dlog, L.out.out, Md, s));
  {
    hipEvent_t ready = nullptr;
    SKF_TRY(with_ready_event(M, true, &ready, [&] { return dense_dgrad(M, L.out, dlog, L.out.out, Md, G, d, 0, nullptr, 0, s); }));
    SKF_TRY(M->sched.issue(M, s, ready));
  }
  const unsigned char* cross_mask = c.blind_decoder_mask ? nullptr : emask;
  for (int i = N - 1; i >= 0; --i, ++layer_no) {
    const DecLayerP& w = L.dec[i];
    const DecAct& a = P.dec[i];
    const Plan::GradSet& gs = P.gs[layer_no % P.n_gs];
    float* dy3 = M->at<float>(gs.dy[0]); float* dy2 = M->at<float>(gs.dy[1]); float* dy1 = M->at<float>(gs.dy[2]);
    float* dqkv = M->at<float>(gs.dqkv); float* dkv2 = M->at<float>(gs.dkv2); float* dq2 = M->at<float>(gs.dq2);
    SKF_TRY(ffn_ln_bwd(M, w.ln3, w.f1, w.f2, G, M->at<float>(a.z3), M->at<float>(a.st3), M->at<float>(a.out2), M->at<float>(a.h), dy3,
                       M->at<float>(gs.dh), G2, Md, rate, site_dec(N, i, 2), s, hbits_of(M, a.hbits, Md), M->at<char>(a.img[1])));
    SKF_TRY(ln_oproj_bwd(M, w.ln2, w.mha2.o, G2, M->at<float>(a.z2), M->at<float>(a.st2), M->at<float>(a.o2), G, dy2, dO, Md, rate,
                         site_dec(N, i, 1), s, M->at<char>(a.img_o2)));
    const float* kv2 = M->at<float>(a.kv2);
    SKF_TRY(M->sched.before_write(M, dq2, s));
    SKF_TRY(M->sched.before_write(M, dkv2, s));
    const int* qlive = M->ctx.live_lengths(Md);
    SKF_TRY(skf_attention_bwd_ordered(M->at<float>(a.q2), d, kv2, 2 * d, kv2 + d, 2 * d, M->at<float>(a.o2), d, dO, d,
                                      M->at<float>(a.astats2), cross_mask, Le, 0, B, H, Ld, Le, dh, dq2, d, dkv2, 2 * d,
                                      dkv2 + d, 2 * d, M->cfg.gemm_precision, qlive, M->ctx.order, s));
    SKF_TRY(dense_wgrad(M, w.mha2.q, M->at<float>(a.out1), d, dq2, d, Md, s));
    const bool lead = row_owner_takes_ln(M, w.ln1, ln_oproj_partial_bytes(M, Md), Md, &w.mha1.o, &w.mha2.q);
    if (!lead) SKF_TRY(dense_dgrad(M, w.mha2.q, dq2, d, Md, G, d, 1, nullptr, 0, s));
    SKF_TRY(dense_wgrad(M, w.mha2.kv, pre, L.E, dkv2, 2 * d, Me, s));
    if (i == 0) {
      SKF_TRY(M->sched.before_read(M, dpre, s));
      SKF_TRY(dense_dgrad(M, w.mha2.kv, dkv2, 2 * d, Me, dpre, L.E, i != N - 1, nullptr, 0, s));
    } else SKF_TRY(dense_dgrad_deferred(M, w.mha2.kv, dkv2, 2 * d, Me, dpre, L.E, i != N - 1, s));
    SKF_TRY(ln_oproj_bwd(M, w.ln1, w.mha1.o, G, M->at<float>(a.z1), M->at<float>(a.st1), M->at<float>(a.o1), G2, dy1, dO, Md, rate,
                         site_dec(N, i, 0), s, M->at<char>(a.img_o1), lead ? dq2 : nullptr, lead ? M->at<char>(a.img_q2t) : nullptr));
    const float* qkv = M->at<float>(a.qkv);
    SKF_TRY(M->sched.before_write(M, dqkv, s));
    SKF_TRY(skf_attention_bwd_ordered(qkv, 3 * d, qkv + d, 3 * d, qkv + 2 * d, 3 * d, M->at<float>(a.o1), d, dO, d,
                                      M->at<float>(a.astats1), dmask, Ld, 1, B, H, Ld, Ld, dh, dqkv, 3 * d, dqkv + d, 3 * d,
                                      dqkv + 2 * d, 3 * d, M->cfg.gemm_precision, qlive, M->ctx.order, s));
    SKF_TRY(dense_wgrad(M, w.mha1.qkv, M->at<float>(a.x_in), d, dqkv, 3 * d, Md, s));
    const bool hold = M->ctx.ffn_fused && i > 0;
    hipEvent_t ready = nullptr;
    SKF_TRY(with_ready_event(M, !hold, &ready, [&] { return dense_dgrad(M, w.mha1.qkv, dqkv, 3 * d, Md, G2, d, 1, nullptr, 0, s); }));
    float* t = G; G = G2; G2 = t;
    if (i == 0 && dec_emb_on_side) {
      const float* dx0 = G;
      char* sorted = M->at<char>(P.emb_sort[1]);
      float* dtable = M->G(L.dec_emb);
      const int V = c.vocab_size;
      M->sched.queue_launch(dx0, [M, sorted, dtable, dx0, B, Ld, V, d, rate, N](hipStream_t on) {
        return skf_embed_bwd_sorted(sorted, B, Ld, dx0, V, d, dtable, rate, site_dec_embed(N), M->state, on);
      });
    }
    if (hold) SKF_TRY(M->sched.hold(M, s));
    else SKF_TRY(M->sched.issue(M, s, ready));
  }
  M->ctx.clear_live();
  if (M->ctx.metrics_deferred) {
    M->ctx.metrics_deferred = false;
    SKF_TRY(metrics_update(M, M->sched.side));
  }
  if (c.continuous) {
    SKF_TRY(skf_embed_continuous_bwd(M->at<float>(P.tar), Le, B, Ld, G, d, M->G(L.dec_embd.w), M->G(L.dec_embd.b), rate,
                                     site_dec_embed(N), M->state, M->at<char>(P.small_ws), P.small_ws_bytes, s));
  } else if (dec_emb_on_side) {
  } else if (P.emb_sort_bytes) {
    SKF_TRY(skf_embed_bwd_sorted(M->at<char>(P.emb_sort[1]), B, Ld, G, c.vocab_size, d, M->G(L.dec_emb), rate, site_dec_embed(N), M->state, s));
  } else {
    SKF_HIP(hipMemsetAsync(M->G(L.dec_emb), 0, (size_t)c.vocab_size * d * sizeof(float), s));
    SKF_TRY(skf_embed_bwd(tar, Le, B, Ld, G, c.vocab_size, d, M->G(L.dec_emb), rate, site_dec_embed(N), M->state, s));
  }
  if (M->n_buckets == 2) SKF_TRY(flush_wgrads(M, s, 0, false, true, dec_emb_on_side));
  SKF_TRY(M->sched.before_read(M, dpre, s));
  }
  const int E = L.E, Ua = L.Ua, U = c.lowerdim, NB = c.class_buffer_layers;
  hipEvent_t bott_ready = nullptr;
  if (bott) {
    const bool defer_sums = M->sched.side && Ua <= 4096;
    float* xp1 = M->at<float>(P.bott_part);
    float* xp2 = xp1 + (size_t)B * Le;
    float* pvp = xp2 + (size_t)B * Le;
    if (recon && defer_sums) {
      SKF_TRY(skf_expander_bwd_partials(dpre, M->at<float>(P.emb), M->P(L.exp_w), B, Le, E, demb, 0, xp1, xp2, s));
      SKF_TRY(colsum_desc(M, xp1, B, Le, M->G(L.exp_w)));
      SKF_TRY(colsum_desc(M, xp2, B, Le, M->G(L.exp_b)));
    } else if (recon)
      SKF_TRY(skf_expander_bwd(dpre, M->at<float>(P.emb), M->P(L.exp_w), B, Le, E, demb, 0, M->G(L.exp_w), M->G(L.exp_b),
                               M->at<char>(P.small_ws), P.small_ws_bytes, s));
    const int acc_emb = recon ? 1 : 0;
    const float* dcls = M->at<float>(P.cls_logits);
    if (cls && NB == 0) {
      SKF_TRY(dense_wgrad(M, L.cls, M->at<float>(P.emb), E, dcls, c.n_classes, B, s));
      SKF_TRY(dense_dgrad(M, L.cls, dcls, c.n_classes, B, demb, E, acc_emb, nullptr, 0, s));
    } else if (cls) {
      float* dz = M->at<float>(P.dcb[0]);
      float* dz2 = M->at<float>(P.dcb[1]);
      SKF_TRY(M->sched.before_write(M, dz, s));
      SKF_TRY(dense_wgrad(M, L.cls, M->at<float>(P.cb_f[NB - 1]), U, dcls, c.n_classes, B, s));
      SKF_TRY(dense_dgrad(M, L.cls, dcls, c.n_classes, B, dz, U, 0, M->at<float>(P.cb_h[NB - 1]), U, s));
      for (int i = NB - 1; i >= 0; --i) {
        SKF_TRY(skf_dropout(dz, dz, (size_t)B * U, c.class_dropout, site_class(N, i), M->state, s));
        const float* in = i == 0 ? M->at<float>(P.emb) : M->at<float>(P.cb_f[i - 1]);
        const int in_w = i == 0 ? E : U;
        SKF_TRY(dense_wgrad(M, L.cbuf[i], in, in_w, dz, U, B, s));
        if (i == 0) {
          SKF_TRY(dense_dgrad(M, L.cbuf[0], dz, U, B, demb, E, acc_emb, nullptr, 0, s));
        } else {
          SKF_TRY(M->sched.before_write(M, dz2, s));
          SKF_TRY(dense_dgrad(M, L.cbuf[i], dz, U, B, dz2, U, 0, M->at<float>(P.cb_h[i - 1]), U, s));
          float* t = dz; dz = dz2; dz2 = t;
        }
      }
    }
    const float* dpool = demb;
    if (c.attn_version == 2) {
      SKF_TRY(M->sched.before_write(M, M->at<float>(P.dpooled), s));
      SKF_TRY(dense_wgrad(M, L.bott_e, M->at<float>(P.pooled), d, demb, U, B, s));
      SKF_TRY(dense_dgrad(M, L.bott_e, demb, U, B, M->at<float>(P.dpooled), d, 0, nullptr, 0, s));
      dpool = M->at<float>(P.dpooled);
    }
    if (dec_emb_on_side) { G = G2; G2 = M->at<float>(P.gC); }
    SKF_TRY(M->sched.before_write(M, G, s));
    if (defer_sums) {
      SKF_TRY(skf_pool_bwd_partials(M->at<float>(P.u), M->P(L.bott_v), enc_out, M->at<float>(P.pool_a), dpool, B, Le, Ua, d, G, pvp, s));
      SKF_TRY(colsum_desc(M, pvp, B, Ua, M->G(L.bott_v)));
    } else
    SKF_TRY(skf_pool_bwd(M->at<float>(P.u), M->P(L.bott_v), enc_out, M->at<float>(P.pool_a), dpool, B, Le, Ua, d,
                         G, M->G(L.bott_v), M->at<char>(P.small_ws), P.small_ws_bytes, s));
    SKF_TRY(dense_wgrad(M, L.bott_w, enc_out, d, M->at<float>(P.u), Ua, Me, s));
    SKF_TRY(with_ready_event(M, true, &bott_ready, [&] { return dense_dgrad(M, L.bott_w, M->at<float>(P.u), Ua, Me, G, d, 1, nullptr, 0, s); }));
  } else {
    float* spare = (G == M->at<float>(P.gA)) ? M->at<float>(P.gB) : M->at<float>(P.gA);
    G = dpre; G2 = spare;
  }
  SKF_TRY(M->sched.issue(M, s, bott_ready));
  for (int i = N - 1; i >= 0; --i, ++layer_no) {
    const EncLayerP& w = L.enc[i];
    const EncAct& a = P.enc[i];
    const Plan::GradSet& gs = P.gs[layer_no % P.n_gs];
    float* dy2 = M->at<float>(gs.dy[0]); float* dy1 = M->at<float>(gs.dy[1]);
    float* dqkv = M->at<float>(gs.dqkv);
    SKF_TRY(ffn_ln_bwd(M, w.ln2, w.f1, w.f2, G, M->at<float>(a.z2), M->at<float>(a.st2), M->at<float>(a.x1), M->at<float>(a.h), dy2,
                       M->at<float>(gs.dh), G2, Me, rate, site_enc(i, 1), s, hbits_of(M, a.hbits, Me), M->at<char>(a.img[1])));
    if (i == 0) SKF_TRY(M->sched.issue(M, s, M->ctx.last_ready));
    M->ctx.last_ready = nullptr;
    {
      hipEvent_t ready = nullptr;
      SKF_TRY(with_ready_event(M, i == 0, &ready, [&] {
        return ln_oproj_bwd(M, w.ln1, w.mha.o, G2, M->at<float>(a.z1), M->at<float>(a.st1), M->at<float>(a.o), G, dy1, dO, Me, rate,
                            site_enc(i, 0), s, M->at<char>(a.img_o));
      }));
      if (i == 0) SKF_TRY(M->sched.issue(M, s, ready));
    }
    const float* qkv = M->at<float>(a.qkv);
    SKF_TRY(M->sched.before_write(M, dqkv, s));
    SKF_TRY(skf_attention_bwd_ordered(qkv, 3 * d, qkv + d, 3 * d, qkv + 2 * d, 3 * d, M->at<float>(a.o), d, dO, d,
                                      M->at<float>(a.astats), emask, Le, 0, B, H, Le, Le, dh, dqkv, 3 * d, dqkv + d, 3 * d,
                                      dqkv + 2 * d, 3 * d, M->cfg.gemm_precision, nullptr, M->ctx.order, s));
    SKF_TRY(dense_wgrad(M, w.mha.qkv, M->at<float>(a.x_in), d, dqkv, 3 * d, Me, s));
    if (i == 0) SKF_TRY(M->sched.issue(M, s, nullptr, !M->sched.holding()));
    SKF_TRY(dense_dgrad(M, w.mha.qkv, dqkv, 3 * d, Me, G, d, 1, nullptr, 0, s));
    if (M->ctx.ffn_fused && i > 0) SKF_TRY(M->sched.hold(M, s));
    else SKF_TRY(M->sched.issue(M, s));
    if (!M->ctx.ffn_fused && M->sched.side && N >= 2 && i == N / 2) SKF_TRY(flush_wgrads(M, s, -1, false, !M->sched.holding()));
  }
  if (c.continuous) {
    SKF_TRY(skf_embed_continuous_bwd(M->at<float>(P.inp), Le, B, Le, G, d, M->G(L.enc_embd.w), M->G(L.enc_embd.b), rate,
                                     site_enc_embed(), M->state, M->at<char>(P.small_ws), P.small_ws_bytes, s));
  } else {
    if (P.emb_sort_bytes) {
      SKF_TRY(skf_embed_bwd_sorted(M->at<char>(P.emb_sort[0]), B, Le, G, c.vocab_size, d, M->G(L.enc_emb), rate, site_enc_embed(),
                                   M->state, s));
    } else {
      SKF_HIP(hipMemsetAsync(M->G(L.enc_emb), 0, (size_t)c.vocab_size * d * sizeof(float), s));
      SKF_TRY(skf_embed_bwd(inp, Le, B, Le, G, c.vocab_size, d, M->G(L.enc_emb), rate, site_enc_embed(), M->state, s));
    }
  }
  return flush_wgrads(M, s, M->n_buckets - 1, true);
}

int issue_embed_sorts(SkfModel* M, hipStream_t s) {
  const SkfConfig& c = M->cfg;
  const Layout& L = M->lay;
  const Plan& P = M->plan;
  if (!P.emb_sort_bytes) return SKF_OK;
  const int B = c.batch, Le = c.seq_len, Ld = c.seq_len - 1, d = c.d_model;
  hipStream_t ss = s;
  if (M->sched.side && do_recon(c)) {
    hipEvent_t staged = (M->inputs_staged && M->inputs_staged_valid && !g_capturing) ? M->inputs_staged : nullptr;
    if (!staged) {
      staged = M->sched.take_event();
      SKF_CHECK_ARG(staged, "event allocation failed");
      SKF_HIP(hipEventRecord(staged, s));
    }
    SKF_HIP(hipStreamWaitEvent(M->sched.side, staged, 0));
    ss = M->sched.side;
    hipEvent_t masks = M->sched.take_event(), ready = M->sched.take_event();
    SKF_CHECK_ARG(masks && ready, "event allocation failed");
    SKF_TRY(forward_preamble(M, true, false, ss, masks));
    SKF_HIP(hipEventRecord(ready, ss));
    M->ctx.masks_ready = masks; M->ctx.pre_ready = ready;
  }
  SKF_TRY(skf_embed_sort(M->at<long long>(P.inp), Le, B, Le, c.vocab_size, M->G(L.enc_emb), d, M->at<char>(P.emb_sort[0]),
                         P.emb_sort_bytes, ss));
  if (do_recon(c))
    SKF_TRY(skf_embed_sort(M->at<long long>(P.tar), Le, B, Ld, c.vocab_size, M->G(L.dec_emb), d, M->at<char>(P.emb_sort[1]),
                           P.emb_sort_bytes, ss));
  return build_row_lists(M, ss);
}
}
```

### sketchformer_amd/csrc/skf_model_fwd.hip

```cpp
#include "skf_model_internal.h"

namespace skf_model_detail {

int classify_fwd(SkfModel* M, bool training, hipStream_t s) {
  const SkfConfig& c = M->cfg;
  const Layout& L = M->lay;
  const Plan& P = M->plan;
  const float* fc = M->at<float>(P.emb);
  for (int i = 0; i < c.class_buffer_layers; ++i) {
    float* h = M->at<float>(P.cb_h[i]);
    float* fdrop = M->at<float>(P.cb_f[i]);
    SKF_TRY(dense_fwd(M, L.cbuf[i], fc, c.batch, h, 1, s));
    const float r = training ? c.class_dropout : 0.f;
    SKF_TRY(skf_dropout(h, fdrop, (size_t)c.batch * c.lowerdim, r, site_class(c.num_layers, i), M->state, s));
    fc = fdrop;
  }
  return dense_fwd(M, L.cls, fc, c.batch, M->at<float>(P.cls_logits), 0, s);
}

int metrics_update(SkfModel* M, hipStream_t s) {
  const SkfConfig& c = M->cfg;
  const Plan& P = M->plan;
  const bool recon = do_recon(c);
  const float* recon_scalar = recon && c.continuous ? M->at<float>(P.cont_scal) + 3 : nullptr;
// ... 30 lines not shown
    if (with_backward) { one(f2, 1, d, F, M->at<char>(im[1])); one(f1, 1, F, d, M->at<char>(im[1]) + half); }
  };
  const bool dec = !encoder_only && do_recon(c);
  for (int i = 0; i < c.num_layers; ++i) {
    ffn(L.enc[i].f1, L.enc[i].f2, P.enc[i].img);
    if (i > 0) one(L.enc[i].mha.qkv, 0, d, 3 * d, M->at<char>(P.enc[i].img_qkv));
    one(L.enc[i].mha.o, 0, d, d, M->at<char>(P.enc[i].img_of));
    if (with_backward) one(L.enc[i].mha.o, 1, d, d, M->at<char>(P.enc[i].img_o));
  }
  if (dec)
    for (int i = 0; i < c.num_layers; ++i) {
      ffn(L.dec[i].f1, L.dec[i].f2, P.dec[i].img);
      if (i > 0) one(L.dec[i].mha1.qkv, 0, d, 3 * d, M->at<char>(P.dec[i].img_qkv));
      one(L.dec[i].mha2.o, 0, d, d, M->at<char>(P.dec[i].img_o2f));
      one(L.dec[i].mha1.o, 0, d, d, M->at<char>(P.dec[i].img_o1f)); one(L.dec[i].mha2.q, 0, d, d, M->at<char>(P.dec[i].img_q2));
      if (with_backward) { one(L.dec[i].mha1.o, 1, d, d, M->at<char>(P.dec[i].img_o1)); one(L.dec[i].mha2.o, 1, d, d, M->at<char>(P.dec[i].img_o2)); }
      if (with_backward) one(L.dec[i].mha2.q, 1, d, d, M->at<char>(P.dec[i].img_q2t));
    }
  return skf_dense_weight_images((int)src.size(), src.data(), ld.data(), tr.data(), K.data(), N.data(), img.data(), c.gemm_precision, s);
}
bool chains(const SkfModel* M, const DenseP& next) {
  return next.in == M->cfg.d_model && (next.out == 128 || next.out == 256 || next.out == 384) && next.ld == next.out;
}
int ffn_ln_fwd(SkfModel* M, const DenseP& f1, const DenseP& f2, const LnP& ln, const float* x, int rows, float* h, void* bits,
               const void* image, float* z, float* out, float* stats, float rate, unsigned site, hipStream_t s,
               const DenseP* next = nullptr, const void* next_image = nullptr, float* next_out = nullptr, bool* next_done = nullptr) {
  const int d = M->cfg.d_model;
  if (next_done) *next_done = false;
  if (M->ctx.ffn_fused && next && chains(M, *next)) {
    if (next_done) *next_done = true;
    return skf_ffn_fused_fwd_proj_f32(rows, d, M->cfg.dff, x, image, M->P(f1.b), M->P(f2.b), h, bits, M->P(ln.g), M->P(ln.b), z, out, stats,
                                      rate, site, M->state, next_image, M->P(next->b), next->out, next_out, M->cfg.gemm_precision, s);
  }
  if (M->ctx.ffn_fused)
    return skf_ffn_fused_fwd_f32(rows, d, M->cfg.dff, x, image, M->P(f1.b), M->P(f2.b), h, bits, M->P(ln.g), M->P(ln.b), z, out, stats,
                                 rate, site, M->state, M->cfg.gemm_precision, s);
  SKF_TRY(dense_fwd_relu_bits(M, f1, x, rows, h, bits, s));
  SKF_TRY(dense_fwd(M, f2, h, rows, z, 0, s));
  return skf_layernorm_residual_fwd(x, z, M->P(ln.g), M->P(ln.b), out, stats, rows, d, rate, site, M->state, s);
}

int attn_tail_ffn_fwd(SkfModel* M, const DenseP& o, const LnP& ln_a, const float* a, const float* x, float* z1, float* x1, float* st1,
                      unsigned site_a, const void* o_image, const DenseP& f1, const DenseP& f2, const LnP& ln, float* h, void* bits,
                      const void* image, float* z, float* out, float* stats, unsigned site, int rows, float rate, hipStream_t s,
                      const DenseP* next, const void* next_image, float* next_out, bool* next_done) {
  const int d = M->cfg.d_model;
  if (!M->ctx.ffn_fused || o.in != d || o.out != d || ln_a.b != ln_a.g + (size_t)d) {
    SKF_TRY(dense_ln_fwd(M, o, a, rows, x, z1, ln_a, x1, st1, rate, site_a, s));
    return ffn_ln_fwd(M, f1, f2, ln, x1, rows, h, bits, image, z, out, stats, rate, site, s, next, next_image, next_out, next_done);
  }
  SkfFfnBlockFwd b{};
  b.struct_size = sizeof(SkfFfnBlockFwd); b.M = rows; b.d = d; b.dff = M->cfg.dff; b.precision = M->cfg.gemm_precision;
  b.x = a; b.image = image; b.b1 = M->P(f1.b); b.b2 = M->P(f2.b); b.h = h; b.relu_bits_out = bits;
  b.gamma = M->P(ln.g); b.beta = M->P(ln.b); b.z = z; b.out = out; b.stats = stats; b.rate = rate; b.site = site; b.step_state = M->state;
  b.pre_image = o_image; b.pre_bias = M->P(o.b); b.pre_residual = x; b.pre_gamma = M->P(ln_a.g); b.pre_beta = M->P(ln_a.b);
  b.pre_z = z1; b.pre_out = x1; b.pre_stats = st1; b.pre_site = site_a;
  const bool chain = next && chains(M, *next);
  if (chain) { b.proj_image = next_image; b.proj_bias = M->P(next->b); b.proj_out = next_out; b.proj_n = next->out; }
  if (next_done) *next_done = chain;
  return skf_ffn_block_fwd_f32(&b, s);
}

}

int forward_preamble(SkfModel* M, bool with_backward, bool encoder_only, hipStream_t s, hipEvent_t masks_ready) {
  const SkfConfig& c = M->cfg;
  const Plan& P = M->plan;
  const int B = c.batch, Le = c.seq_len, Ld = c.seq_len - 1;
  unsigned char* emask = M->at<unsigned char>(P.enc_mask);
  unsigned char* dmask = M->at<unsigned char>(P.dec_mask);
  if (M->ctx.masks_staged) {
  } else if (c.continuous) {
    SKF_TRY(skf_padding_mask_continuous(M->at<float>(P.inp), Le, B, Le, emask, s));
    SKF_TRY(skf_padding_mask_continuous(M->at<float>(P.tar), Le, B, Ld, dmask, s));
  } else {
    SKF_TRY(skf_padding_mask(M->at<long long>(P.inp), Le, B, Le, emask, s));
    SKF_TRY(skf_padding_mask(M->at<long long>(P.tar), Le, B, Ld, dmask, s));
  }
  M->ctx.order = nullptr;
  if (B <= 4096) {
    SKF_TRY(skf_sample_order(emask, Le, Le, encoder_only ? nullptr : dmask, Ld, Ld, B, M->at<int>(P.order), s));
    M->ctx.order = M->at<int>(P.order);
  }
  if (masks_ready) SKF_HIP(hipEventRecord(masks_ready, s));
  M->ctx.ffn_fused = ffn_fused_on(M);
  if (M->ctx.ffn_fused) SKF_TRY(build_ffn_images(M, with_backward, encoder_only, s));
  return SKF_OK;
}

int run_forward(SkfModel* M, bool training, bool with_loss, hipStream_t s, bool encoder_only) {
  const SkfConfig& c = M->cfg;
  const Layout& L = M->lay;
  const Plan& P = M->plan;
  const int B = c.batch, Le = c.seq_len, Ld = c.seq_len - 1, d = c.d_model, H = c.num_heads, dh = d / H;
  const int Me = B * Le, Md = B * Ld, N = c.num_layers;
  const float rate = training ? c.dropout_rate : 0.f;
  const long long* inp = M->at<long long>(P.inp);
  const long long* tar = M->at<long long>(P.tar);
  unsigned char* emask = M->at<unsigned char>(P.enc_mask);
  unsigned char* dmask = M->at<unsigned char>(P.dec_mask);

  const float* inpf = M->at<float>(P.inp);
  const float* tarf = M->at<float>(P.tar);
  const hipEvent_t images_ready = M->ctx.pre_ready, masks_ready = M->ctx.masks_ready;
  if (!images_ready) SKF_TRY(forward_preamble(M, training && with_loss, encoder_only, s));
  const int* order = M->ctx.order;

  if (c.continuous)
    SKF_TRY(skf_embed_continuous_fwd(inpf, Le, B, Le, M->P(L.enc_embd.w), M->P(L.enc_embd.b), d, M->pos,
                                     M->at<float>(P.enc[0].x_in), rate, site_enc_embed(), M->state, s));
  else
    SKF_TRY(skf_embed_fwd(inp, Le, B, Le, M->P(L.enc_emb), c.vocab_size, d, M->pos, M->at<float>(P.enc[0].x_in), rate,
                          site_enc_embed(), M->state, s));
  bool enc_qkv_done = false;
  for (int i = 0; i < N; ++i) {
    const EncLayerP& w = L.enc[i];
    const EncAct& a = P.enc[i];
    float* x = M->at<float>(a.x_in);
    float* qkv = M->at<float>(a.qkv);
    if (!enc_qkv_done) SKF_TRY(dense_fwd(M, w.mha.qkv, x, Me, qkv, 0, s));
    if (i == 0 && images_ready) SKF_HIP(hipStreamWaitEvent(s, masks_ready, 0));
    SKF_TRY(skf_attention_fwd_ordered(qkv, 3 * d, qkv + d, 3 * d, qkv + 2 * d, 3 * d, emask, Le, 0, B, H, Le, Le, dh,
                                      M->at<float>(a.o), d, M->at<float>(a.astats), M->cfg.gemm_precision, order, s));
    const bool has_next = i + 1 < N;
    if (i == 0 && images_ready) SKF_HIP(hipStreamWaitEvent(s, images_ready, 0));
    SKF_TRY(attn_tail_ffn_fwd(M, w.mha.o, w.ln1, M->at<float>(a.o), x, M->at<float>(a.z1), M->at<float>(a.x1), M->at<float>(a.st1),
                              site_enc(i, 0), M->at<char>(a.img_of), w.f1, w.f2, w.ln2, M->at<float>(a.h), hbits_of(M, a.hbits, Me),
                              M->at<char>(a.img[0]), M->at<float>(a.z2), M->at<float>(a.x2), M->at<float>(a.st2), site_enc(i, 1), Me, rate, s,
                              has_next ? &L.enc[i + 1].mha.qkv : nullptr, has_next ? M->at<char>(P.enc[i + 1].img_qkv) : nullptr,
                              has_next ? M->at<float>(P.enc[i + 1].qkv) : nullptr, &enc_qkv_done));
  }
  float* enc_out = M->at<float>(P.enc[N - 1].x2);
  const int E = L.E, Ua = L.Ua;
  const bool bott = has_bott(c), cls = has_cls(c), recon = do_recon(c);
  if (bott) {
    SKF_TRY(dense_fwd(M, L.bott_w, enc_out, Me, M->at<float>(P.u), 2, s));
    SKF_TRY(skf_pool_fwd(M->at<float>(P.u), M->P(L.bott_v), enc_out, B, Le, Ua, d, M->at<float>(P.pool_a),
                         M->at<float>(c.attn_version == 2 ? P.pooled : P.emb), s));
    if (c.attn_version == 2)
      SKF_TRY(dense_fwd(M, L.bott_e, M->at<float>(P.pooled), B, M->at<float>(P.emb), 0, s));
  }
  const bool heads_on_side = with_loss && recon && M->sched.side;
  if (cls && !heads_on_side) SKF_TRY(classify_fwd(M, training, s));
  if (encoder_only || !recon) {
    if (encoder_only || !with_loss) {
      if (!cls) return SKF_OK;
      return skf_softmax_ce(M->at<float>(P.cls_logits), c.n_classes, B, c.n_classes, M->at<long long>(P.labels), 1, 1, 0, 0, 0.f,
                            M->at<float>(P.cls_loss), M->at<float>(P.cls_hit), M->at<float>(P.cls_probs), 0, s);
    }
  }
  float* pre = bott ? M->at<float>(P.pre) : enc_out;
  hipEvent_t dec_in_ready = nullptr;
  bool dec_in_recorded = false;
  if (recon && M->sched.side) {
    M->sched.rewind_events();
    dec_in_ready = M->sched.take_event();
    SKF_CHECK_ARG(dec_in_ready, "event allocation failed");
  }
  if (recon && bott) {
    SKF_TRY(with_tail_event(M, dec_in_ready, &dec_in_recorded,
                            [&] { return skf_expander_fwd(M->at<float>(P.emb), M->P(L.exp_w), M->P(L.exp_b), B, Le, E, pre, s); }));
  }

  if (recon) {
  if (c.continuous)
    SKF_TRY(skf_embed_continuous_fwd(tarf, Le, B, Ld, M->P(L.dec_embd.w), M->P(L.dec_embd.b), d, M->pos,
                                     M->at<float>(P.dec[0].x_in), rate, site_dec_embed(N), M->state, s));
  else
    SKF_TRY(skf_embed_fwd(tar, Le, B, Ld, M->P(L.dec_emb), c.vocab_size, d, M->pos, M->at<float>(P.dec[0].x_in), rate,
                          site_dec_embed(N), M->state, s));
  const unsigned char* cross_mask = c.blind_decoder_mask ? nullptr : emask;
  hipEvent_t kv_done = nullptr, kv_first = nullptr;
  if (M->sched.side) {
    kv_done = M->sched.take_event();
    kv_first = N > 1 ? M->sched.take_event() : kv_done;
    SKF_CHECK_ARG(dec_in_ready && kv_done && kv_first, "event allocation failed");
    if (!dec_in_recorded) SKF_HIP(hipEventRecord(dec_in_ready, s));
    SKF_HIP(hipStreamWaitEvent(M->sched.side, dec_in_ready, 0));
    if (cls && heads_on_side) {
      SKF_TRY(classify_fwd(M, training, M->sched.side));
      SKF_TRY(class_ce_with_grad(M, M->sched.side));
    }
    for (int i = 0; i < N; ++i) {
      SKF_TRY(dense_fwd(M, L.dec[i].mha2.kv, pre, Me, M->at<float>(P.dec[i].kv2), 0, M->sched.side));
      if (i == 0 && kv_first != kv_done) SKF_HIP(hipEventRecord(kv_first, M->sched.side));
    }
    SKF_HIP(hipEventRecord(kv_done, M->sched.side));
  }
  bool dec_qkv_done = false;
  for (int i = 0; i < N; ++i) {
    const DecLayerP& w = L.dec[i];
    const DecAct& a = P.dec[i];
    float* x = M->at<float>(a.x_in);
    float* qkv = M->at<float>(a.qkv);
    if (!dec_qkv_done) SKF_TRY(dense_fwd(M, w.mha1.qkv, x, Md, qkv, 0, s));
    SKF_TRY(skf_attention_fwd_ordered(qkv, 3 * d, qkv + d, 3 * d, qkv + 2 * d, 3 * d, dmask, Ld, 1, B, H, Ld, Ld, dh,
                                      M->at<float>(a.o1), d, M->at<float>(a.astats1), M->cfg.gemm_precision, order, s));
    const bool tail_proj = M->ctx.ffn_fused && w.mha1.o.in == d && w.mha1.o.out == d && chains(M, w.mha2.q) && w.mha2.q.out == d &&
                           w.ln1.b == w.ln1.g + (size_t)d;
    if (tail_proj) {
      SkfFfnBlockFwd tb{};
      tb.struct_size = sizeof(SkfFfnBlockFwd); tb.M = Md; tb.d = d; tb.dff = c.dff; tb.precision = c.gemm_precision;
      tb.x = M->at<float>(a.o1); tb.rate = rate; tb.step_state = M->state;
      tb.pre_image = M->at<char>(a.img_o1f); tb.pre_bias = M->P(w.mha1.o.b); tb.pre_residual = x; tb.pre_gamma = M->P(w.ln1.g); tb.pre_beta = M->P(w.ln1.b);
      tb.pre_z = M->at<float>(a.z1); tb.pre_out = M->at<float>(a.out1); tb.pre_stats = M->at<float>(a.st1); tb.pre_site = site_dec(N, i, 0);
      tb.proj_image = M->at<char>(a.img_q2); tb.proj_bias = M->P(w.mha2.q.b); tb.proj_out = M->at<float>(a.q2); tb.proj_n = d;
      SKF_TRY(skf_ffn_block_fwd_f32(&tb, s));
    } else {
      SKF_TRY(dense_ln_fwd(M, w.mha1.o, M->at<float>(a.o1), Md, x, M->at<float>(a.z1), w.ln1, M->at<float>(a.out1), M->at<float>(a.st1),
                           rate, site_dec(N, i, 0), s));
      SKF_TRY(dense_fwd(M, w.mha2.q, M->at<float>(a.out1), Md, M->at<float>(a.q2), 0, s));
    }
    float* kv2 = M->at<float>(a.kv2);
    if (!kv_done) SKF_TRY(dense_fwd(M, w.mha2.kv, pre, Me, kv2, 0, s));
    else if (i == 0) SKF_HIP(hipStreamWaitEvent(s, kv_first, 0));
    else if (i == 1) SKF_HIP(hipStreamWaitEvent(s, kv_done, 0));
    SKF_TRY(skf_attention_fwd_ordered(M->at<float>(a.q2), d, kv2, 2 * d, kv2 + d, 2 * d, cross_mask, Le, 0, B, H, Ld, Le, dh,
                                      M->at<float>(a.o2), d, M->at<float>(a.astats2), M->cfg.gemm_precision, order, s));
    const bool has_next = i + 1 < N;
    SKF_TRY(attn_tail_ffn_fwd(M, w.mha2.o, w.ln2, M->at<float>(a.o2), M->at<float>(a.out1), M->at<float>(a.z2), M->at<float>(a.out2),
                              M->at<float>(a.st2), site_dec(N, i, 1), M->at<char>(a.img_o2f), w.f1, w.f2, w.ln3, M->at<float>(a.h),
                              hbits_of(M, a.hbits, Md), M->at<char>(a.img[0]), M->at<float>(a.z3), M->at<float>(a.out3), M->at<float>(a.st3),
                              site_dec(N, i, 2), Md, rate, s, has_next ? &L.dec[i + 1].mha1.qkv : nullptr,
                              has_next ? M->at<char>(P.dec[i + 1].img_qkv) : nullptr, has_next ? M->at<float>(P.dec[i + 1].qkv) : nullptr,
                              &dec_qkv_done));
  }
  SKF_TRY(dense_fwd(M, L.out, M->at<float>(P.dec[N - 1].out3), Md, M->at<float>(P.logits), 0, s));
  }

  const long long* labels = M->at<long long>(P.labels);
  if (with_loss) {
    if (recon) {
      if (c.continuous) {
        SKF_TRY(skf_continuous_loss(M->at<float>(P.logits), tarf, Le, Ld, 1, Md, c.recon_weight, M->at<float>(P.recon_loss),
                                    M->at<float>(P.recon_hit), M->at<float>(P.row_mask), M->at<float>(P.cont_scal), 1, s));
      } else {
        SKF_TRY(skf_softmax_ce(M->at<float>(P.logits), c.vocab_size, Md, c.vocab_size, tar, Le, Ld, 1, 1,
                               c.recon_weight / (float)Md, M->at<float>(P.recon_loss), M->at<float>(P.recon_hit), nullptr, 1, s));
      }
    }
    if (cls && !heads_on_side) SKF_TRY(class_ce_with_grad(M, s));
    if (heads_on_side) M->ctx.metrics_deferred = true;
    else SKF_TRY(metrics_update(M, s));
  } else if (cls) {
    SKF_TRY(skf_softmax_ce(M->at<float>(P.cls_logits), c.n_classes, B, c.n_classes, labels, 1, 1, 0, 0, 0.f,
                           M->at<float>(P.cls_loss), M->at<float>(P.cls_hit), M->at<float>(P.cls_probs), 0, s));
  }
  return SKF_OK;
}

}
```

### sketchformer_amd/csrc/skf_model_internal.h

```cpp
#pragma once
#include <stdarg.h>
#include <stdlib.h>
#include <string.h>
#include <string>
#include <vector>
#include <map>
#include <algorithm>
#include <functional>
#include "skf_common.h"
#include "skf_attention_params.h"
#include "skf_decode_fused.h"

namespace skf_model_detail {

struct DenseP { size_t w, b; int in, out, ld; };
struct LnP { size_t g, b; };
struct SelfMhaP { DenseP qkv, o; };
struct CrossMhaP { DenseP q, kv, o; };
struct EncLayerP { SelfMhaP mha; DenseP f1, f2; LnP ln1, ln2; };
struct DecLayerP { SelfMhaP mha1; CrossMhaP mha2; DenseP f1, f2; LnP ln1, ln2, ln3; };

inline bool has_bott(const SkfConfig& c) { return c.lowerdim > 0; }
inline bool has_cls(const SkfConfig& c) { return c.lowerdim > 0 && c.do_classification != 0; }
inline bool do_recon(const SkfConfig& c) { return c.do_reconstruction != 0; }

struct Layout {
  size_t total = 0;
  size_t enc_emb = 0, dec_emb = 0;
  DenseP enc_embd{}, dec_embd{};
  std::vector<EncLayerP> enc;
  std::vector<DecLayerP> dec;
  DenseP bott_w{};
  size_t bott_v = 0;
  DenseP bott_e{};
  std::vector<DenseP> cbuf;
  size_t dec_off = 0;
  int E = 0, Ua = 0;
  DenseP cls{}, out{};
  size_t exp_w = 0, exp_b = 0;
  std::vector<SkfParamEntry> entries;
};

struct Bump {
  size_t off = 0;
  size_t take(size_t bytes) { size_t o = off; off += (bytes + 255) & ~(size_t)255; return o; }
};

struct DecodeAreas {
  size_t pre = 0;
  std::vector<size_t> kv2;
  std::vector<size_t> cache;
  size_t img = 0;
  size_t mask = 0, flags = 0;
  size_t limit = 0;
  size_t dyn = 0;
  size_t anc = 0, cand = 0, beam = 0;
  size_t pfx_tok = 0, pfx_len = 0;
};

struct EncAct { size_t x_in, qkv, o, z1, st1, astats, x1, h, z2, st2, x2, hbits, img[2], img_o, img_qkv, img_of; };
struct DecAct { size_t x_in, qkv, o1, z1, st1, astats1, out1, q2, kv2, o2, astats2, z2, st2, out2, h, z3, st3, out3, hbits, img[2], img_o1, img_o2, img_qkv, img_o2f, img_o1f, img_q2, img_q2t; };

struct Plan {
  size_t bytes = 0;
  size_t inp, tar, labels, enc_mask, dec_mask;
  size_t order;
  std::vector<EncAct> enc;
  std::vector<DecAct> dec;
  size_t u, pool_a, emb, pooled, dpooled, cls_logits, cls_probs, pre, logits;
  std::vector<size_t> cb_h, cb_f;
  size_t dcb[2];
  size_t recon_loss, recon_hit, cls_loss, cls_hit, row_mask, cont_scal;
  size_t gA, gB, gC, dqkv, dh, do_, dpre, dkv2, dq2, demb;
  struct GradSet { size_t dy[3], dh, dq2, dkv2, dqkv; };
  std::vector<GradSet> gs;
  int n_gs = 2;
  size_t gemm_ws, gemm_ws_bytes, small_ws, small_ws_bytes;
  size_t emb_sort[2] = {0, 0}, emb_sort_bytes = 0;
  size_t slab_arena, slab_arena_bytes, descs, n_wgrads;
  size_t ln_part, ln_part_stride;
  size_t bott_part = 0;
  DecodeAreas dca;
  size_t dc_x[2], dc_q, dc_o, dc_z, dc_out1, dc_out2, dc_h, dc_logits, dc_stats, dc_kvnew;
  size_t live_len = 0, live16 = 0, live32 = 0;
};

struct Img16 { size_t w = 0, wt = 0; int in = 0, out = 0, ld_src = 0, ldw = 0, ldt = 0; size_t src = 0; };
struct Enc16 { size_t x_in, qkv, o, olo, z1, st1, astats, x1, h, z2, st2, x2, hbits; };
struct Dec16 { size_t x_in, qkv, o1, olo1, z1, st1, astats1, out1, q2, kv2, o2, olo2, astats2, z2, st2, out2, h, z3, st3, out3, hbits; };

struct Plan16 {
  size_t bytes = 0;
  size_t inp = 0, tar = 0, labels = 0, enc_mask = 0, dec_mask = 0;
  std::vector<Enc16> enc;
  std::vector<Dec16> dec;
  size_t u = 0, pool_a = 0, emb = 0, cls_logits = 0, cls_probs = 0, pre = 0, logits = 0;
  int ld_logits = 0;
  size_t recon_loss = 0, recon_hit = 0, cls_loss = 0, cls_hit = 0;
  size_t gA = 0, gB = 0, dy = 0, dqkv = 0, dh = 0, dO = 0, dpre = 0, dkv2 = 0, dq2 = 0, demb = 0;
  size_t slab = 0, slab_bytes = 0, small_ws = 0, small_ws_bytes = 0, attn_ws = 0, attn_ws_bytes = 0, ln_ws = 0, ln_ws_bytes = 0;
  size_t cast_descs = 0, cast_descs_bytes = 0; int cast_n = 0, cast_blocks = 0; const float* cast_for = nullptr;
  const char* tables_ws = nullptr;
  size_t ln_slabs = 0, ln_descs = 0; int ln_n = 0, ln_n_dec = 0, ln_blocks_dec = 0, ln_blocks_enc = 0, ln_cursor = 0; bool ln_batched = false;
  DecodeAreas dca;
  size_t order = 0;
  size_t live_len = 0, live1 = 0, live64 = 0;
  size_t emb_sort[2] = {0, 0}, emb_sort_bytes = 0;
  std::map<size_t, Img16> img;
};

struct ReduceBatch {
  std::vector<SkfReduceDesc> descs;
  bool descs_uploaded = false;
  size_t slab_cursor = 0, desc_cursor = 0, ln_cursor = 0;
  int reduce_blocks = 0;
  size_t phase_desc_begin = 0;
  bool side_used = false;

  void begin_step();
  void reset();
  int add(const SkfReduceDesc& d, int blocks);
  float* take_ln_partial(SkfModel* M);
  float* take_slab(SkfModel* M, size_t bytes, size_t queued);
  size_t begin() const { return phase_desc_begin; }
  size_t end() const { return desc_cursor; }
  int blocks() const { return reduce_blocks; }
  void end_phase(bool final);
};

struct SideSched {
  hipStream_t side = nullptr;
  hipEvent_t fork_event = nullptr, join_event = nullptr;
  std::vector<hipEvent_t> events;
  size_t next_event = 0;
  struct SideEvent { hipEvent_t e; long seq; };
  long side_seq = 0, side_waited = 0;
  std::map<const void*, SideEvent> pending_readers;
  std::map<const void*, SideEvent> pending_writers;
  struct Queued { DenseP w; const float* x; int ldx; const float* dy; int lddy; int rows; int kind = 0; float* dx = nullptr; int lddx = 0; int accumulate = 0; const int* blocks32 = nullptr; std::function<int(hipStream_t)> run; };
  std::vector<Queued> wq;
  std::vector<Queued> wq_held;

  int create(bool captured);
  void destroy();
  hipEvent_t take_event();
  void rewind_events() { next_event = 0; }
  void begin_backward() { wq.clear(); wq_held.clear(); pending_readers.clear(); pending_writers.clear(); rewind_events(); }
  void queue_wgrad(const DenseP& w, const float* x, int ldx, const float* dy, int lddy, int rows, const int* blocks32) { wq.push_back(Queued{w, x, ldx, dy, lddy, rows, 0, nullptr, 0, 0, blocks32}); }
  void queue_dgrad(const DenseP& w, const float* dy, int lddy, int rows, float* dx, int lddx, int accumulate) { wq.push_back(Queued{w, nullptr, 0, dy, lddy, rows, 1, dx, lddx, accumulate}); }
  void queue_launch(const float* reads, std::function<int(hipStream_t)> run) { Queued q{}; q.dy = reads; q.kind = 2; q.run = std::move(run); wq.push_back(std::move(q)); }
  bool holding() const { return !wq_held.empty(); }
  int hold(SkfModel* M, hipStream_t s);
  int issue(SkfModel* M, hipStream_t s, hipEvent_t ready_recorded = nullptr, bool on_main = false);
  int issue_held(SkfModel* M, hipStream_t s, hipEvent_t ready_recorded = nullptr);
  int before_write(SkfModel* M, const void* buf, hipStream_t s) { return wait_side(M, false, buf, s); }
  int before_read(SkfModel* M, const void* buf, hipStream_t s) { return wait_side(M, true, buf, s); }
  int wait_side(SkfModel* M, bool writers, const void* buf, hipStream_t s);
  int join(hipStream_t s);
  bool fork_into_capture(hipStream_t s) { return hipEventRecord(fork_event, s) == hipSuccess && hipStreamWaitEvent(side, fork_event, 0) == hipSuccess; }
  bool join_capture(hipStream_t s) { return hipEventRecord(join_event, side) == hipSuccess && hipStreamWaitEvent(s, join_event, 0) == hipSuccess; }
};

struct StepCtx {
  bool lists_set = false;
  int live_rows = 0;
  const int* live_len = nullptr;
  struct LiveList { int granule; const int* blocks; } lists[2] = {};
  const int* order = nullptr;
  hipEvent_t pre_ready = nullptr, masks_ready = nullptr;
  bool lists_built = false;
  bool masks_staged = false;
  bool ffn_fused = false;
  bool metrics_deferred = false;
  hipEvent_t last_ready = nullptr;

  void reset() { *this = StepCtx(); }
  void begin_backward() { clear_live(); last_ready = nullptr; }
  void set_live(int rows, const int* len, int g0, const int* b0, int g1, const int* b1) { lists_set = true; live_rows = rows; live_len = len; lists[0] = {g0, b0}; lists[1] = {g1, b1}; }
  void clear_live() { lists_set = false; live_rows = 0; live_len = nullptr; lists[0] = lists[1] = LiveList{}; }
  bool live(int rows) const { return lists_set && rows == live_rows; }
  const int* live_lengths(int rows) const { return live(rows) ? live_len : nullptr; }
  const int* live_blocks(int rows, int granule) const {
    return !live(rows) ? nullptr : lists[0].granule == granule ? lists[0].blocks : lists[1].granule == granule ? lists[1].blocks : nullptr;
  }
};

}

struct SkfModel {
  SkfConfig cfg;
  uint32_t flags = 0;
  bool no_ln_fuse = false, no_relu_bits = false;
  skf_model_detail::StepCtx ctx;
  skf_model_detail::Layout lay;
  skf_model_detail::Plan plan;
  skf_model_detail::Plan16 p16;
  bool bf16 = false;
  float *params = nullptr, *grads = nullptr, *m = nullptr, *v = nullptr, *metrics = nullptr;
  const float* pos = nullptr;
  char* ws = nullptr;
  void* state = nullptr;
  hipGraphExec_t g_fb = nullptr, g_opt = nullptr, g_dec = nullptr;
  long long dec_dyn_host[2] = {0, 0};
  std::vector<int> dec_stream_host;
  std::vector<int> dec_pfx_len_host;
  float g_opt_scale = 0.f;
  struct Clip { bool on = false; int mode = 0, skip_nonfinite = 0, monitor = 0, n_chunks = 0; float threshold = 0.f, clipvalue = 0.f;
                float* stats = nullptr; void* plan = nullptr; void* norm_ws = nullptr; size_t norm_ws_bytes = 0; };
  Clip clip;
  hipGraphExec_t g_clip = nullptr;
  float g_clip_scale = 0.f;
  struct Avg { float* shadow = nullptr; float decay = 0.f; int num_updates = 0; bool live = false; };
  Avg avg;
  skf_model_detail::SideSched sched;
  hipEvent_t inputs_staged = nullptr;
  bool inputs_staged_valid = false;
  skf_model_detail::ReduceBatch red;
  hipEvent_t bucket_ready[2] = {nullptr, nullptr};
  int n_buckets = 1;

  struct Named { size_t off; int rows, cols, ld, bf16; };
  std::map<std::string, Named> named;
  void reg(const std::string& name, size_t off, size_t rows, size_t cols, size_t ld, int is_bf16) {
    named[name] = {off, (int)rows, (int)cols, (int)ld, is_bf16};
  }

  template <typename T> T* at(size_t off) const { return reinterpret_cast<T*>(ws + off); }
  float* P(size_t off) const { return params + off; }
  float* G(size_t off) const { return grads + off; }
};

#define SKF_TRY(call)            \
  do {                           \
    int rc__ = (call);           \
    if (rc__ != SKF_OK) return rc__; \
  } while (0)

namespace skf_model_detail {

extern thread_local int g_capturing;

inline unsigned site_enc_embed() { return 0; }
inline unsigned site_enc(int layer, int j) { return 1 + 2 * layer + j; }
inline unsigned site_dec_embed(int N) { return 1 + 2 * N; }
inline unsigned site_class(int N, int i) { return 2 + 5 * N + i; }
inline unsigned site_dec(int N, int layer, int j) { return 2 + 2 * N + 3 * layer + j; }

inline bool may_park(const SkfModel* M, bool needs_side = true) { return !g_capturing && (M->sched.side || !needs_side); }
template <typename F>
int with_tail_event(SkfModel* M, hipEvent_t e, bool* rode, F call, bool needs_side = true) {
  SkfTailScope scope(may_park(M, needs_side) ? e : nullptr);
// ... 55 lines not shown
```

### sketchformer_amd/csrc/skf_model_layout.hip

```cpp
#include "skf_model_internal.h"

namespace skf_model_detail {
namespace {

inline size_t pad4(size_t n) { return (n + 3) & ~(size_t)3; }

void add_entry(Layout& L, const std::string& name, size_t off, int rows, int cols, int stride) {
  SkfParamEntry e;
  memset(&e, 0, sizeof(e));
  snprintf(e.name, sizeof(e.name), "%s", name.c_str());
  e.offset = (int64_t)off; e.rows = rows; e.cols = cols; e.row_stride = stride;
  L.entries.push_back(e);
}

size_t alloc(Layout& L, size_t n) { size_t o = L.total; L.total += pad4(n); return o; }

DenseP dense(Layout& L, const std::string& name, int in, int out) {
  DenseP d; d.in = in; d.out = out; d.ld = out;
  d.w = alloc(L, (size_t)in * out); d.b = alloc(L, out);
  add_entry(L, name + "/kernel", d.w, in, out, out);
  add_entry(L, name + "/bias", d.b, 1, out, out);
  return d;
}

// ... 155 lines not shown
    a.img_qkv = b.take(skf_dense_image_bytes((int)d, 3 * (int)d, c.gemm_precision));
    a.img_of = b.take(skf_dense_image_bytes((int)d, (int)d, c.gemm_precision));
    a.x2 = 0;
    P.enc.push_back(a);
  }
  const size_t enc_out = b.take(Me * d * f);
  for (int i = 0; i < c.num_layers; ++i) P.enc[i].x2 = (i + 1 < c.num_layers) ? P.enc[i + 1].x_in : enc_out;
  P.u = b.take(Me * Ua * f); P.pool_a = b.take(B * L * f); P.emb = b.take(B * E * f);
  P.pooled = b.take(B * d * f); P.dpooled = b.take(B * d * f);
  for (int i = 0; i < c.class_buffer_layers; ++i) { P.cb_h.push_back(b.take(B * U * f)); P.cb_f.push_back(b.take(B * U * f)); }
  P.dcb[0] = b.take(B * U * f); P.dcb[1] = b.take(B * U * f);
  P.cls_logits = b.take(B * c.n_classes * f); P.cls_probs = b.take(B * c.n_classes * f);
  P.pre = b.take(Me * E * f);
  for (int i = 0; i < c.num_layers; ++i) {
    DecAct a;
    a.x_in = b.take(Md * d * f); a.qkv = b.take(Md * 3 * d * f); a.o1 = b.take(Md * d * f); a.z1 = b.take(Md * d * f);
    a.st1 = b.take(Md * 2 * f); a.astats1 = b.take(B * H * Ld * 2 * f); a.out1 = b.take(Md * d * f);
    a.q2 = b.take(Md * d * f); a.kv2 = b.take(Me * 2 * d * f); a.o2 = b.take(Md * d * f);
    a.astats2 = b.take(B * H * Ld * 2 * f); a.z2 = b.take(Md * d * f); a.st2 = b.take(Md * 2 * f);
    a.out2 = b.take(Md * d * f); a.h = b.take(Md * F * f); a.z3 = b.take(Md * d * f); a.st3 = b.take(Md * 2 * f);
    a.hbits = b.take(std::max(skf_gemm_relu_bits_bytes((int)Md, (int)F, (int)d, c.gemm_precision),
                              skf_ffn_relu_bits_bytes((int)Md, (int)d, (int)F, c.gemm_precision)));
    a.img[0] = b.take(skf_ffn_image_bytes((int)d, (int)F, c.gemm_precision)); a.img[1] = b.take(skf_ffn_image_bytes((int)d, (int)F, c.gemm_precision));
    a.img_o1 = b.take(skf_dense_image_bytes((int)d, (int)d, c.gemm_precision)); a.img_o2 = b.take(skf_dense_image_bytes((int)d, (int)d, c.gemm_precision));
    a.img_qkv = b.take(skf_dense_image_bytes((int)d, 3 * (int)d, c.gemm_precision));
    a.img_o2f = b.take(skf_dense_image_bytes((int)d, (int)d, c.gemm_precision));
    a.img_o1f = b.take(skf_dense_image_bytes((int)d, (int)d, c.gemm_precision)); a.img_q2 = b.take(skf_dense_image_bytes((int)d, (int)d, c.gemm_precision));
    a.img_q2t = b.take(skf_dense_image_bytes((int)d, (int)d, c.gemm_precision));
    a.out3 = 0;
    P.dec.push_back(a);
  }
  const size_t dec_out = b.take(Md * d * f);
  for (int i = 0; i < c.num_layers; ++i) P.dec[i].out3 = (i + 1 < c.num_layers) ? P.dec[i + 1].x_in : dec_out;
  P.logits = b.take(Md * Vout * f);
  P.recon_loss = b.take(Md * f); P.recon_hit = b.take(Md * f); P.cls_loss = b.take(B * f); P.cls_hit = b.take(B * f);
  P.row_mask = b.take(Md * f); P.cont_scal = b.take(64);
  P.gA = b.take(Me * d * f); P.gB = b.take(Me * d * f); P.gC = b.take(Me * d * f);
  P.dqkv = b.take(Me * 3 * d * f); P.dh = b.take(Me * F * f); P.do_ = b.take(Me * d * f);
  P.dpre = b.take(Me * E * f); P.dkv2 = b.take(Me * 2 * d * f); P.dq2 = b.take(Md * d * f); P.demb = b.take(B * E * f);
  {
    const size_t per_set = (3 * Me * d + Me * F + Md * d + Me * 2 * d + Me * 3 * d) * f;
    const size_t layers = (size_t)c.num_layers * (do_recon(c) ? 2 : 1);
    P.n_gs = (per_set * layers > ((size_t)8 << 30) || layers < 2) ? 2 : (int)layers;
    P.gs.resize(P.n_gs);
  }
  for (int k = 0; k < P.n_gs; ++k) {
    for (int j = 0; j < 3; ++j) P.gs[k].dy[j] = b.take(Me * d * f);
    P.gs[k].dh = k == 0 ? P.dh : b.take(Me * F * f);
    P.gs[k].dq2 = k == 0 ? P.dq2 : b.take(Md * d * f);
    P.gs[k].dkv2 = k == 0 ? P.dkv2 : b.take(Me * 2 * d * f);
    P.gs[k].dqkv = k == 0 ? P.dqkv : b.take(Me * 3 * d * f);
  }
  size_t g = 0;
  auto mx = [&](size_t v) { if (v > g) g = v; };
  mx(wgrad_ws(d, 3 * d, Me)); mx(wgrad_ws(d, d, Me)); mx(wgrad_ws(d, F, Me)); mx(wgrad_ws(F, d, Me));
  mx(wgrad_ws((int)E, 2 * d, Me)); mx(wgrad_ws(d, (int)Vout, Md));
  if (has_bott(c)) {
    mx(wgrad_ws(d, (int)Ua, Me));
    mx(wgrad_ws((int)E, c.n_classes, B)); mx(wgrad_ws(U, c.n_classes, B)); mx(wgrad_ws(d, U, B)); mx(wgrad_ws((int)E, U, B)); mx(wgrad_ws(U, U, B));
  }
  P.gemm_ws_bytes = g; P.gemm_ws = b.take(g);
  P.n_wgrads = 4 + 11 * (size_t)c.num_layers + (size_t)c.class_buffer_layers + 5 * (size_t)c.num_layers + 3;
  P.bott_part = b.take((2 * B * L + B * 4096) * f);
  P.ln_part_stride = (skf_layernorm_bwd_workspace_bytes((int)Me, (int)d) + 255) & ~(size_t)255;
  P.ln_part = b.take(5 * (size_t)c.num_layers * P.ln_part_stride);
  P.slab_arena_bytes = P.n_wgrads * ((g + 255) & ~(size_t)255);
  P.slab_arena = b.take(P.slab_arena_bytes);
  P.descs = b.take(P.n_wgrads * sizeof(SkfReduceDesc));
  size_t s = skf_layernorm_bwd_workspace_bytes((int)Me, (int)d);
  if (B * Ua * f > s) s = B * Ua * f;
  if (2 * B * L * f > s) s = 2 * B * L * f;
  if (c.continuous && skf_embed_continuous_bwd_workspace_bytes((int)Me, (int)d) > s) s = skf_embed_continuous_bwd_workspace_bytes((int)Me, (int)d);
  P.small_ws_bytes = s; P.small_ws = b.take(s);
  if (!c.continuous && c.vocab_size <= 12288 && c.d_model <= 512) {
    P.emb_sort_bytes = (skf_embed_sort_workspace_bytes((int)B, (int)L, c.vocab_size) + 255) & ~(size_t)255;
    P.emb_sort[0] = b.take(P.emb_sort_bytes); P.emb_sort[1] = b.take(P.emb_sort_bytes);
  }
  P.dca = take_decode_areas(b, c, false);
  P.dc_x[0] = b.take(B * d * f); P.dc_x[1] = b.take(B * d * f); P.dc_q = b.take(B * d * f); P.dc_o = b.take(B * d * f);
  P.dc_z = b.take(B * d * f); P.dc_out1 = b.take(B * d * f); P.dc_out2 = b.take(B * d * f); P.dc_h = b.take(B * F * f);
  P.dc_logits = b.take(B * Vout * f); P.dc_stats = b.take(B * 2 * f); P.dc_kvnew = b.take(B * 2 * d * f);
  P.live_len = b.take(B * sizeof(int));
  P.order = b.take(B * sizeof(int));
  P.live16 = b.take(skf_row_blocks_bytes(B * (L - 1), 16)); P.live32 = b.take(skf_row_blocks_bytes(B * (L - 1), 32));
  P.bytes = b.off;
  return P;
}

namespace {

inline int pad8(int n) { return (n + 7) & ~7; }

void add_img(Plan16& P, Bump& b, const DenseP& w) {
  Img16 im;
  im.in = w.in; im.out = w.out; im.ld_src = w.ld; im.src = w.w;
  im.ldw = pad8(w.out); im.ldt = pad8(w.in);
  im.w = b.take((size_t)w.in * im.ldw * 2);
  im.wt = b.take((size_t)w.out * im.ldt * 2);
  P.img[w.w] = im;
}

}

Plan16 build_plan16(const SkfConfig& c, const Layout& L) {
  Plan16 P;
  Bump b;
  const size_t B = c.batch, Ls = c.seq_len, Ld = c.seq_len - 1, d = c.d_model, F = c.dff, U = c.lowerdim;
  const size_t Me = B * Ls, Md = B * Ld, H = c.num_heads, f = sizeof(float), h2 = 2;
  const int N = c.num_layers;
  P.inp = b.take(B * Ls * 8); P.tar = b.take(B * Ls * 8); P.labels = b.take(B * 8);
  P.enc_mask = b.take(B * Ls); P.dec_mask = b.take(B * Ls);
  for (int i = 0; i < N; ++i) {
    Enc16 a;
    a.x_in = b.take(Me * d * h2); a.qkv = b.take(Me * 3 * d * h2); a.o = b.take(Me * d * h2); a.olo = b.take(Me * d * h2); a.z1 = b.take(Me * d * h2);
    a.st1 = b.take(Me * 2 * f); a.astats = b.take(B * H * Ls * 2 * f); a.x1 = b.take(Me * d * h2);
    a.h = b.take(Me * F * h2); a.z2 = b.take(Me * d * h2); a.st2 = b.take(Me * 2 * f); a.x2 = 0;
    a.hbits = b.take(skf_gemm_bf16_relu_bits_bytes((int)Me, (int)F));
    P.enc.push_back(a);
  }
  const size_t enc_out = b.take(Me * d * h2);
  for (int i = 0; i < N; ++i) P.enc[i].x2 = (i + 1 < N) ? P.enc[i + 1].x_in : enc_out;
  P.u = b.take(Me * U * h2); P.pool_a = b.take(B * Ls * f); P.emb = b.take(B * d * f);
  P.cls_logits = b.take(B * c.n_classes * f); P.cls_probs = b.take(B * c.n_classes * f);
  P.pre = b.take(Me * d * h2);
  for (int i = 0; i < N; ++i) {
    Dec16 a;
    a.x_in = b.take(Md * d * h2); a.qkv = b.take(Md * 3 * d * h2); a.o1 = b.take(Md * d * h2); a.olo1 = b.take(Md * d * h2); a.z1 = b.take(Md * d * h2);
    a.st1 = b.take(Md * 2 * f); a.astats1 = b.take(B * H * Ld * 2 * f); a.out1 = b.take(Md * d * h2);
    a.q2 = b.take(Md * d * h2); a.kv2 = b.take(Me * 2 * d * h2); a.o2 = b.take(Md * d * h2); a.olo2 = b.take(Md * d * h2);
    a.astats2 = b.take(B * H * Ld * 2 * f); a.z2 = b.take(Md * d * h2); a.st2 = b.take(Md * 2 * f);
    a.out2 = b.take(Md * d * h2); a.h = b.take(Md * F * h2); a.z3 = b.take(Md * d * h2); a.st3 = b.take(Md * 2 * f);
    a.hbits = b.take(skf_gemm_bf16_relu_bits_bytes((int)Md, (int)F));
    a.out3 = 0;
    P.dec.push_back(a);
  }
  const size_t dec_out = b.take(Md * d * h2);
  for (int i = 0; i < N; ++i) P.dec[i].out3 = (i + 1 < N) ? P.dec[i + 1].x_in : dec_out;
  P.ld_logits = pad8(c.vocab_size);
  P.logits = b.take(Md * (size_t)P.ld_logits * h2);
  P.recon_loss = b.take(Md * f); P.recon_hit = b.take(Md * f); P.cls_loss = b.take(B * f); P.cls_hit = b.take(B * f);
  P.gA = b.take(Me * d * h2); P.gB = b.take(Me * d * h2); P.dy = b.take(Me * d * h2); P.dO = b.take(Me * d * h2);
  P.dqkv = b.take(Me * 3 * d * h2); P.dh = b.take(Me * F * h2); P.dpre = b.take(Me * d * h2);
  P.dkv2 = b.take(Me * 2 * d * h2); P.dq2 = b.take(Md * d * h2); P.demb = b.take(B * d * f);
  size_t g = 0;
  auto mx = [&](int in, int out, size_t rows) {
    const size_t v = skf_gemm_bf16_wgrad_workspace_bytes(in, out, (int)rows, skf_gemm_bf16_wgrad_splits(in, out, (int)rows));
    if (v > g) g = v;
  };
  mx((int)d, (int)(3 * d), Me); mx((int)d, (int)d, Me); mx((int)d, (int)F, Me); mx((int)F, (int)d, Me); mx((int)d, (int)(2 * d), Me);
  mx((int)d, c.vocab_size, Md); mx((int)d, (int)U, Me);
  const size_t small = skf_gemm_workspace_bytes((int)d, c.n_classes, (int)B, 8, 1);
  if (small > g) g = small;
  P.slab_bytes = g; P.slab = b.take(g);
  size_t s = B * U * f;
  if (2 * B * Ls * f > s) s = 2 * B * Ls * f;
  P.small_ws_bytes = s; P.small_ws = b.take(s);
  P.attn_ws_bytes = skf_attention_bf16_bwd_workspace_bytes((int)B, (int)H, (int)Ls); P.attn_ws = b.take(P.attn_ws_bytes);
  P.ln_ws_bytes = skf_layernorm_bwd_bf16_workspace_bytes((int)Me, (int)d); P.ln_ws = b.take(P.ln_ws_bytes);
  P.cast_descs_bytes = 256 * sizeof(SkfCastDesc); P.cast_descs = b.take(P.cast_descs_bytes);
  P.ln_n = 5 * (int)c.num_layers; P.ln_n_dec = 3 * (int)c.num_layers;
  P.ln_slabs = b.take((size_t)P.ln_n * P.ln_ws_bytes); P.ln_descs = b.take((size_t)P.ln_n * sizeof(SkfReduceDesc));
  P.dca = take_decode_areas(b, c, true);
  P.live_len = b.take(B * sizeof(int));
  P.order = b.take(B * sizeof(int));
  P.live1 = b.take(skf_row_blocks_bytes((int)Md, 1)); P.live64 = b.take(skf_row_blocks_bytes((int)Md, 64));
  if (c.vocab_size <= 12288) {
// ... 15 lines not shown
```

### sketchformer_amd/csrc/skf_row_blocks.hip

```cpp
#include "skf_common.h"
#include "../../include/skf.h"

namespace {

__global__ __launch_bounds__(256) void target_live_len_kernel(const long long* __restrict__ tar, int tar_ld, int B, int Ld,
                                                              int* __restrict__ live_len) {
  const int lane = threadIdx.x & 63, b = blockIdx.x * 4 + (threadIdx.x >> 6);
  if (b >= B) return;
  int last = -1;
  for (int t = lane; t < Ld; t += 64)
    if (tar[(size_t)b * tar_ld + t + 1] != 0) last = t;
#pragma unroll
  for (int o = 32; o > 0; o >>= 1) last = max(last, __shfl_xor(last, o, 64));
  if (lane == 0) live_len[b] = last + 1;
}

__global__ __launch_bounds__(1024) void row_blocks_kernel(const int* __restrict__ live_len, int B, int rps, int g,
                                                          int* __restrict__ blocks) {
  __shared__ int part[1024];
  const int tid = threadIdx.x;
  const int rows = B * rps, nb = (rows + g - 1) / g;
  const int per = (nb + 1023) / 1024;
  auto is_live = [&](int k) -> bool {
    const int r0 = k * g, r1 = min(rows, r0 + g);
    for (int b = r0 / rps; b * rps < r1; ++b) {
      const int lo = max(r0, b * rps), hi = b * rps + live_len[b];
      if (lo < hi) return true;
    }
    return false;
  };
  int cnt = 0;
  for (int k = tid * per; k < min(nb, (tid + 1) * per); ++k) cnt += is_live(k) ? 1 : 0;
  part[tid] = cnt;
  __syncthreads();
  for (int off = 1; off < 1024; off <<= 1) {
    const int a = tid >= off ? part[tid - off] : 0;
    __syncthreads();
    part[tid] += a;
    __syncthreads();
  }
  const int nlive = part[1023];
  int lpos = part[tid] - cnt;
  for (int k = tid * per; k < min(nb, (tid + 1) * per); ++k) {
    const bool lv = is_live(k);
    blocks[2 + nb + k] = lv ? 1 : 0;
    if (lv) blocks[2 + lpos++] = k;
    else blocks[2 + nlive + (k - lpos)] = k;
  }
  if (tid == 0) { blocks[0] = nlive; blocks[1] = nb; }
}

__global__ __launch_bounds__(1024) void row_list_kernel(const int* __restrict__ live_len, int B, int rps, int* __restrict__ blocks) {
  extern __shared__ int pre[];
  __shared__ int part[1024];
  const int tid = threadIdx.x;
  const int per = (B + 1023) / 1024;
  int cnt = 0;
  for (int b = tid * per; b < min(B, (tid + 1) * per); ++b) cnt += min(max(live_len[b], 0), rps);
  part[tid] = cnt;
  __syncthreads();
  for (int off = 1; off < 1024; off <<= 1) {
    const int a = tid >= off ? part[tid - off] : 0;
    __syncthreads();
    part[tid] += a;
    __syncthreads();
  }
  int run = part[tid] - cnt;
  for (int b = tid * per; b < min(B, (tid + 1) * per); ++b) { pre[b] = run; run += min(max(live_len[b], 0), rps); }
  if (tid == 1023) pre[B] = part[1023];
  __syncthreads();
  const int rows = B * rps, nlive = pre[B];
  const int r = blockIdx.x * 1024 + tid;
  if (r < rows) {
    const int b = r / rps, t = r - b * rps, len = min(max(live_len[b], 0), rps);
    const bool lv = t < len;
    const int live_before = pre[b] + min(t, len);
    blocks[2 + (lv ? live_before : nlive + (r - live_before))] = r;
    blocks[2 + rows + r] = lv ? 1 : 0;
  }
  if (blockIdx.x == 0 && tid == 0) { blocks[0] = nlive; blocks[1] = rows; }
}

__device__ __forceinline__ void count_unmasked(const unsigned char* __restrict__ m, int ld, int L, int B, int* key, int tid) {
  if (!m) return;
  if (ld == L && L >= 4 && ((uintptr_t)m & 3) == 0) {
    const int total = B * L, n = (total + 3) >> 2;
    for (int i0 = tid; i0 < n; i0 += 4 * 1024) {
      unsigned v[4];
#pragma unroll
      for (int u = 0; u < 4; ++u) {
        const int i = i0 + 1024 * u, t0 = 4 * i;
        v[u] = 0x01010101u;
        if (t0 + 3 < total) v[u] = *reinterpret_cast<const unsigned*>(m + t0);
        else if (t0 < total) v[u] = (unsigned)m[t0] | (t0 + 1 < total ? (unsigned)m[t0 + 1] << 8 : 0x100u) | (t0 + 2 < total ? (unsigned)m[t0 + 2] << 16 : 0x10000u) | 0x1000000u;
      }
#pragma unroll
      for (int u = 0; u < 4; ++u) {
        const int t0 = 4 * (i0 + 1024 * u), b = t0 / L, split = (b + 1) * L - t0;
        int z0 = 0, z1 = 0;
#pragma unroll
        for (int e = 0; e < 4; ++e) {
          const int z = ((v[u] >> (8 * e)) & 0xffu) == 0u;
          if (e < split) z0 += z; else z1 += z;
        }
        if (z0) atomicAdd(&key[b], z0);
        if (z1) atomicAdd(&key[b + 1], z1);
      }
    }
  } else {
    const int n = B * L;
    for (int i = tid; i < n; i += 1024) {
      const int b = i / L, t = i - b * L;
      if (!m[(size_t)b * ld + t]) atomicAdd(&key[b], 1);
    }
  }
}
__global__ __launch_bounds__(1024) void sample_order_kernel(const unsigned char* __restrict__ ma, int lda, int La,
                                                            const unsigned char* __restrict__ mb, int ldb, int Lb, int B, int* __restrict__ order) {
  extern __shared__ int key[];
  int* rank = key + B;
  const int tid = threadIdx.x;
  for (int b = tid; b < 2 * B; b += 1024) key[b] = 0;
  __syncthreads();
  count_unmasked(ma, lda, La, B, key, tid);
  count_unmasked(mb, ldb, Lb, B, key, tid);
  __syncthreads();
  const int parts = B >= 1024 ? 1 : 1024 / B, per_pass = 1024 / parts;
  for (int b0 = 0; b0 < B; b0 += per_pass) {
    const int b = b0 + tid / parts, part = tid - (tid / parts) * parts;
    if (tid < per_pass * parts && b < B) {
      const int k = key[b];
      int cnt = 0;
      for (int j = part; j < B; j += parts) { const int kj = key[j]; cnt += (kj > k || (kj == k && j < b)) ? 1 : 0; }
      if (cnt) atomicAdd(&rank[b], cnt);
    }
  }
  __syncthreads();
  for (int b = tid; b < B; b += 1024) order[rank[b]] = b;
}

}

extern "C" int skf_sample_order(const unsigned char* mask_a, int lda, int La, const unsigned char* mask_b, int ldb, int Lb, int B, int* order,
                                skf_stream_t stream) {
  SKF_CHECK_ARG(order && B > 0 && B <= 4096 && (mask_a || mask_b), "bad argument (B <= 4096: the counts and ranks of a batch sit in 32 KB of LDS)");
  SKF_CHECK_ARG((!mask_a || (La > 0 && lda >= La)) && (!mask_b || (Lb > 0 && ldb >= Lb)), "bad mask shape");
  hipLaunchKernelGGL(sample_order_kernel, dim3(1), dim3(1024), (size_t)2 * B * sizeof(int), (hipStream_t)stream, mask_a, lda, La, mask_b, ldb, Lb, B, order);
  SKF_LAUNCH_CHECK();
  return SKF_OK;
}

extern "C" int skf_target_live_len(const long long* tar, int tar_ld, int B, int Ld, int* live_len, skf_stream_t stream) {
  SKF_CHECK_ARG(tar && live_len && B > 0 && Ld > 0 && tar_ld > Ld, "bad argument");
  hipLaunchKernelGGL(target_live_len_kernel, dim3(skf_cdiv(B, 4)), dim3(256), 0, (hipStream_t)stream, tar, tar_ld, B, Ld, live_len);
  SKF_LAUNCH_CHECK();
  return SKF_OK;
}

extern "C" size_t skf_row_blocks_bytes(int rows, int granule) {
  return granule > 0 ? (size_t)(2 + 2 * skf_cdiv(rows, granule)) * sizeof(int) : 0;
}

extern "C" int skf_row_blocks_build(const int* live_len, int B, int rows_per_sample, int granule, int* blocks, skf_stream_t stream) {
  SKF_CHECK_ARG(live_len && blocks && B > 0 && rows_per_sample > 0 && granule > 0, "bad argument");
  if (granule == 1 && B <= 8192)
    hipLaunchKernelGGL(row_list_kernel, dim3(skf_cdiv(B * rows_per_sample, 1024)), dim3(1024), (size_t)(B + 1) * sizeof(int), (hipStream_t)stream,
                       live_len, B, rows_per_sample, blocks);
  else
  hipLaunchKernelGGL(row_blocks_kernel, dim3(1), dim3(1024), 0, (hipStream_t)stream, live_len, B, rows_per_sample, granule, blocks);
  SKF_LAUNCH_CHECK();
  return SKF_OK;
}
```

### sketchformer_amd/ops.py

```python
import ctypes as C

import torch

from . import _lib


def _stream():
    return C.c_void_p(torch.cuda.current_stream().cuda_stream)


def _p(t):
    if t is None:
        return None
    if not t.is_cuda:
        raise _lib.SkfError("sketchformer_amd ops need CUDA(HIP) tensors; got a CPU tensor (no CPU fallback)")
    return C.c_void_p(t.data_ptr())


def _prec(precision):
    return _lib.default_precision() if precision is None else int(precision)


def _f32(t, name):
    if t.dtype != torch.float32:
# ... 102 lines not shown
def ema_update(shadow, w, decay, num_updates=False, state=None, skip=None):
    _flat_f32_pair(shadow, w, "shadow", "w")
    if num_updates and state is None:
        raise ValueError("num_updates reads `iterations`: it needs the step state")
    if skip is not None:
        _p(skip)
        if skip.element_size() != 4 or skip.numel() < 1 or skip.device != shadow.device:
            raise TypeError("skip must be a tensor of 4-byte words on the device of shadow")
    _lib.call("skf_ema_update", _p(shadow), _p(w), shadow.numel(), float(decay), int(bool(num_updates)), _p(state), _p(skip), _stream())
    return shadow


def buffer_swap(a, b):
    _flat_f32_pair(a, b, "a", "b")
    _lib.call("skf_buffer_swap", _p(a), _p(b), a.numel(), _stream())


def target_live_len(tar, Ld):
    assert tar.dtype == torch.int64 and tar.dim() == 2 and tar.shape[1] > Ld
    out = torch.empty(tar.shape[0], dtype=torch.int32, device=tar.device)
    _lib.call("skf_target_live_len", _p(tar), tar.stride(0), tar.shape[0], Ld, _p(out), _stream())
    return out


def row_blocks(live_len, rows_per_sample, granule):
    B = live_len.shape[0]
    n = _lib.load().skf_row_blocks_bytes(B * rows_per_sample, granule) // 4
    out = torch.empty(n, dtype=torch.int32, device=live_len.device)
    _lib.call("skf_row_blocks_build", _p(live_len), B, rows_per_sample, granule, _p(out), _stream())
    return out


def relu_bits(M, N, K, device, precision=None):
    n = _lib.load().skf_gemm_relu_bits_bytes(M, N, K, _prec(precision))
    return torch.zeros(n // 8, dtype=torch.int64, device=device) if n else None


def gemm(a, b, a_kcontig=True, b_kcontig=False, bias=None, act=0, relu_src=None, out=None, accumulate=False,
         splits=1, bias_grad=None, precision=None, row_blocks=None, row_block_rows=0, relu_bits_out=None, relu_bits_in=None):
    _f32(a, "a"); _f32(b, "b")
    M, K = (a.shape[0], a.shape[1]) if a_kcontig else (a.shape[1], a.shape[0])
    N = b.shape[0] if b_kcontig else b.shape[1]
    assert (b.shape[1] if b_kcontig else b.shape[0]) == K, "inner dimensions differ"
    if out is None:
        out = torch.empty(M, N, dtype=torch.float32, device=a.device)
    ws = None
    wsb = 0
    if splits > 1 or bias_grad is not None:
        wsb = _lib.load().skf_gemm_workspace_bytes(M, N, K, splits, 1)
        ws = _ws(wsb, a.device)
    if row_blocks is not None and (splits > 1 or bias_grad is not None):
        assert not a_kcontig and not b_kcontig
        used = C.c_int(0)
        _lib.call("skf_gemm_wgrad_partial_rows", M, N, K, _p(a), a.stride(0), _p(b), b.stride(0), splits,
                  int(bias_grad is not None), _p(ws), wsb, C.byref(used), _prec(precision), _p(row_blocks), row_block_rows, _stream())
        _lib.call("skf_splitk_reduce", _p(ws), used.value, M, N, _p(out), out.stride(0), int(accumulate), _p(bias_grad), 0, _stream())
        return out
    if relu_bits_out is not None or relu_bits_in is not None:
        _lib.call("skf_gemm_f32_bits", int(a_kcontig), int(b_kcontig), M, N, K, _p(a), a.stride(0), _p(b), b.stride(0),
                  _p(out), out.stride(0), _p(bias), act, _p(relu_src), relu_src.stride(0) if relu_src is not None else 0,
                  int(accumulate), splits, _p(bias_grad), 0, _p(ws), wsb, _prec(precision), _p(row_blocks), row_block_rows,
                  _p(relu_bits_out), _p(relu_bits_in), _stream())
        return out
    if row_blocks is not None:
        _lib.call("skf_gemm_f32_rows", int(a_kcontig), int(b_kcontig), M, N, K, _p(a), a.stride(0), _p(b), b.stride(0),
                  _p(out), out.stride(0), _p(bias), act, _p(relu_src), relu_src.stride(0) if relu_src is not None else 0,
                  int(accumulate), splits, _p(bias_grad), 0, _p(ws), wsb, _prec(precision), _p(row_blocks), row_block_rows, _stream())
        return out
    _lib.call("skf_gemm_f32", int(a_kcontig), int(b_kcontig), M, N, K, _p(a), a.stride(0), _p(b), b.stride(0),
              _p(out), out.stride(0), _p(bias), act, _p(relu_src), relu_src.stride(0) if relu_src is not None else 0,
              int(accumulate), splits, _p(bias_grad), 0, _p(ws), wsb, _prec(precision), _stream())
    return out


def sample_order(mask_a=None, mask_b=None):
    m = mask_a if mask_a is not None else mask_b
    out = torch.empty(m.shape[0], dtype=torch.int32, device=m.device)
    _lib.call("skf_sample_order", _p(mask_a), mask_a.stride(0) if mask_a is not None else 0, mask_a.shape[1] if mask_a is not None else 0,
              _p(mask_b), mask_b.stride(0) if mask_b is not None else 0, mask_b.shape[1] if mask_b is not None else 0, m.shape[0], _p(out),
              _stream())
    return out


def attention_fwd(q, k, v, num_heads, key_mask=None, causal=False, precision=None, sample_order=None):
    B, Lq, d = q.shape
    Lk = k.shape[1]
    o = torch.empty(B, Lq, d, dtype=torch.float32, device=q.device)
    stats = torch.empty(B, num_heads, Lq, 2, dtype=torch.float32, device=q.device)
    _lib.call("skf_attention_fwd_ordered", _p(q), q.stride(1), _p(k), k.stride(1), _p(v), v.stride(1), _p(key_mask),
              key_mask.stride(0) if key_mask is not None else 0, int(causal), B, num_heads, Lq, Lk, d // num_heads,
              _p(o), o.stride(1), _p(stats), _prec(precision), _p(sample_order), _stream())
    return o, stats


def attention_weights(q, k, num_heads, key_mask=None, causal=False):
    B, Lq, d = q.shape
    Lk = k.shape[1]
    w = torch.empty(B, num_heads, Lq, Lk, dtype=torch.float32, device=q.device)
    _lib.call("skf_attention_weights", _p(q), q.stride(1), _p(k), k.stride(1), _p(key_mask),
              key_mask.stride(0) if key_mask is not None else 0, int(causal), B, num_heads, Lq, Lk, d // num_heads, _p(w), _stream())
    return w


def attention_fwd_float_mask(q, k, v, num_heads, mask=None, return_weights=False):
    B, Lq, d = q.shape
    Lk = k.shape[1]
    o = torch.empty(B, Lq, d, dtype=torch.float32, device=q.device)
    w = torch.empty(B, num_heads, Lq, Lk, dtype=torch.float32, device=q.device) if return_weights else None
    sb = sh = sq = 0
    if mask is not None:
        mask = torch.as_tensor(mask, device=q.device).detach().to(torch.float32)
        while mask.dim() < 4:
            mask = mask[None]
        if mask.stride(-1) != 1 and mask.shape[-1] != 1:
            mask = mask.contiguous()
        mask = torch.broadcast_to(mask, (B, num_heads, Lq, Lk))
        if mask.stride(-1) != 1:
            mask = mask.contiguous()
        sb, sh, sq = mask.stride(0), mask.stride(1), mask.stride(2)
    _lib.call("skf_attention_fwd_float_mask", _p(q), q.stride(1), _p(k), k.stride(1), _p(v), v.stride(1), _p(mask), sb, sh, sq,
              B, num_heads, Lq, Lk, d // num_heads, _p(o), o.stride(1), _p(w), _stream())
    return o, w


def row_mean(a, b=None, mode=0):
    a = torch.as_tensor(a).detach().to(device="cuda", dtype=torch.float32).contiguous()
    if b is not None:
        b = torch.as_tensor(b, device=a.device).detach().to(torch.float32).expand_as(a).contiguous()
    cols = a.shape[-1]
    out = torch.empty(a.shape[:-1], dtype=torch.float32, device=a.device)
    _lib.call("skf_row_mean", _p(a), _p(b), a.numel() // cols, cols, int(mode), _p(out), _stream())
    return out


def attention_decode(q, k, v, num_heads, n_keys=None, key_mask=None, key_limit=None, key_limit_all=0, step=None,
                     k_new=None, v_new=None, limit_from_step=False):
    B, d = q.shape
    Lk = k.shape[1] if n_keys is None else int(n_keys)
    assert k.stride(0) == v.stride(0) and k.stride(1) == v.stride(1)
    o = torch.empty(B, d, dtype=torch.float32, device=q.device)
    _lib.call("skf_attention_decode", _p(q), q.stride(0), _p(k), _p(v), k.stride(1), k.stride(0), _p(key_mask),
              key_mask.stride(0) if key_mask is not None else 0, _p(key_limit), int(key_limit_all), B, num_heads, Lk,
              d // num_heads, _p(o), o.stride(0), _p(step), _p(k_new), _p(v_new), k_new.stride(0) if k_new is not None else 0,
              int(limit_from_step), _stream())
    return o


def attention_bwd(q, k, v, o, do, stats, num_heads, key_mask=None, causal=False, precision=None, q_live_len=None, two_pass=False,
                  sample_order=None):
    B, Lq, d = q.shape
    Lk = k.shape[1]
    dq = torch.full((B, Lq, d), float("nan"), dtype=torch.float32, device=q.device)
    dk = torch.empty(B, Lk, d, dtype=torch.float32, device=q.device)
    dv = torch.empty(B, Lk, d, dtype=torch.float32, device=q.device)
    _lib.call("skf_attention_bwd_ordered", _p(q), q.stride(1), _p(k), k.stride(1), _p(v), v.stride(1), _p(o), o.stride(1),
              _p(do), do.stride(1), _p(stats), _p(key_mask), key_mask.stride(0) if key_mask is not None else 0,
              int(causal), B, num_heads, Lq, Lk, d // num_heads, _p(dq), dq.stride(1), _p(dk), dk.stride(1),
              _p(dv), dv.stride(1), _prec(precision) | (_lib.ATTN_TWO_PASS if two_pass else 0), _p(q_live_len), _p(sample_order), _stream())
    return dq, dk, dv


def padding_mask(tokens, L=None):
    B, ld = tokens.shape
    L = L or ld
    out = torch.empty(B, L, dtype=torch.uint8, device=tokens.device)
    _lib.call("skf_padding_mask", _p(tokens), ld, B, L, _p(out), _stream())
    return out


def embed_fwd(tokens, table, pos, L=None, rate=0.0, site=0, state=None):
    B, ld = tokens.shape
    L = L or ld
    V, d = table.shape
    out = torch.empty(B, L, d, dtype=torch.float32, device=table.device)
    _lib.call("skf_embed_fwd", _p(tokens), ld, B, L, _p(table), V, d, _p(pos), _p(out), rate, site, _p(state), _stream())
    return out


def embed_bwd(tokens, dx, vocab, L=None, rate=0.0, site=0, state=None):
    B, ld = tokens.shape
    L = L or ld
    d = dx.shape[-1]
    dtable = torch.zeros(vocab, d, dtype=torch.float32, device=dx.device)
    _lib.call("skf_embed_bwd", _p(tokens), ld, B, L, _p(dx), vocab, d, _p(dtable), rate, site, _p(state), _stream())
    return dtable


def embed_bwd_sorted(tokens, dx, vocab, L=None, rate=0.0, site=0, state=None, prefill=None):
    B, ld = tokens.shape
    L = L or ld
    d = dx.shape[-1]
    dtable = torch.full((vocab, d), float("nan") if prefill is None else prefill, dtype=torch.float32, device=dx.device)
    nbytes = _lib.load().skf_embed_sort_workspace_bytes(B, L, vocab)
    ws = torch.empty((nbytes + 3) // 4, dtype=torch.int32, device=dx.device)
    _lib.call("skf_embed_sort", _p(tokens), ld, B, L, vocab, _p(dtable), d, _p(ws), nbytes, _stream())
    _lib.call("skf_embed_bwd_sorted", _p(ws), B, L, _p(dx), vocab, d, _p(dtable), rate, site, _p(state), _stream())
    return dtable


def layernorm_residual_fwd(x, y, gamma, beta, rate=0.0, site=0, state=None):
    d = x.shape[-1]
    rows = x.numel() // d
    z = y.clone()
    out = torch.empty_like(x)
    stats = torch.empty(rows, 2, dtype=torch.float32, device=x.device)
    _lib.call("skf_layernorm_residual_fwd", _p(x), _p(z), _p(gamma), _p(beta), _p(out), _p(stats), rows, d, rate, site,
              _p(state), _stream())
    return out, z, stats


def gemm_ln_residual(a, w, bias, x, gamma, beta, rate=0.0, site=0, state=None, precision=None):
    _f32(a, "a"); _f32(w, "w"); _f32(x, "x")
    M, K = a.shape
    N = w.shape[1]
    z = torch.empty(M, N, dtype=torch.float32, device=a.device)
    out = torch.empty_like(z)
    stats = torch.empty(M, 2, dtype=torch.float32, device=a.device)
    _lib.call("skf_gemm_ln_residual_f32", M, N, K, _p(a), a.stride(0), _p(w), w.stride(0), _p(bias), _p(x), _p(gamma), _p(beta),
              _p(z), _p(out), _p(stats), rate, site, _p(state), _prec(precision), _stream())
    return out, z, stats


def ffn_fused_supported(M, d, dff, precision=None):
    return bool(_lib.load().skf_ffn_fused_supported(M, d, dff, _prec(precision)))


def ffn_weight_images(pairs, transpose, precision=None):
    n = len(pairs)
    d, dff = pairs[0][0].shape
    nbytes = _lib.load().skf_ffn_image_bytes(d, dff, _prec(precision))
    if not nbytes:
        raise _lib.SkfError("no fused feed-forward path for d=%d dff=%d" % (d, dff))
    imgs = [torch.empty(nbytes, dtype=torch.uint8, device=pairs[0][0].device) for _ in range(n)]
    PA = C.c_void_p * n
    IA = C.c_int * n
    for w1, w2 in pairs:
        _f32(w1, "W1"); _f32(w2, "W2")
# ... 1036 lines not shown
```

Baseline: 7.283 million stroke-tokens/sec.

## Precompute per-sample key-mask scan table shared by attention forward and backward

Adds a small kernel that scans each key-padding mask once per step, in sample order, and writes a 64-byte record per sample: batch index, last valid key, key0 status, a bitmap of masked tiles, and packed per-key pad bits. The attention forward and backward kernels then read this record through scalar constant loads instead of loading and ballot-reducing the mask themselves, which drops a global load and a block barrier from each kernel's prologue. The forward kernel also uses the precomputed last key to limit K/V staging before the barrier. In exchange there is an extra launch, extra workspace, and more code paths guarded by dh, Lk and split conditions.

```diff
diff --git a/include/skf.h b/include/skf.h
--- a/include/skf.h
+++ b/include/skf.h
@@ -131,6 +131,18 @@
                               const float* dO, int lddo, const float* stats, const unsigned char* key_mask, int key_mask_ld,
                               int causal, int B, int H, int Lq, int Lk, int dh, float* dQ, int lddq, float* dK, int lddk,
                               float* dV, int lddv, int precision, const int* q_live_len, const int* sample_order, skf_stream_t stream);
+size_t skf_attention_key_scan_bytes(int B);
+int skf_attention_key_scan(const unsigned char* key_mask, int key_mask_ld, int Lk, const int* sample_order, int B, void* scan,
+                           skf_stream_t stream);
+int skf_attention_fwd_scanned(const float* Q, int ldq, const float* K, int ldk, const float* V, int ldv,
+                              const unsigned char* key_mask, int key_mask_ld, int causal, int B, int H, int Lq, int Lk, int dh,
+                              float* O, int ldo, float* stats, int precision, const int* sample_order, const void* key_scan,
+                              skf_stream_t stream);
+int skf_attention_bwd_scanned(const float* Q, int ldq, const float* K, int ldk, const float* V, int ldv, const float* O, int ldo,
+                              const float* dO, int lddo, const float* stats, const unsigned char* key_mask, int key_mask_ld,
+                              int causal, int B, int H, int Lq, int Lk, int dh, float* dQ, int lddq, float* dK, int lddk,
+                              float* dV, int lddv, int precision, const int* q_live_len, const int* sample_order, const void* key_scan,
+                              skf_stream_t stream);
 int skf_attention_weights(const float* Q, int ldq, const float* K, int ldk, const unsigned char* key_mask, int key_mask_ld,
                           int causal, int B, int H, int Lq, int Lk, int dh, float* W, skf_stream_t stream);
 int skf_attention_fwd_float_mask(const float* Q, int ldq, const float* K, int ldk, const float* V, int ldv, const float* mask,
diff --git a/sketchformer_amd/_lib.py b/sketchformer_amd/_lib.py
--- a/sketchformer_amd/_lib.py
+++ b/sketchformer_amd/_lib.py
@@ -171,6 +171,10 @@
     "skf_attention_fwd_ordered": (_I, [_P, _I, _P, _I, _P, _I, _P, _I, _I, _I, _I, _I, _I, _I, _P, _I, _P, _I, _P, _P]),
     "skf_attention_bwd_ordered": (_I, [_P, _I, _P, _I, _P, _I, _P, _I, _P, _I, _P, _P, _I, _I, _I, _I, _I, _I, _I, _P, _I, _P, _I, _P, _I, _I, _P, _P, _P]),
     "skf_sample_order": (_I, [_P, _I, _I, _P, _I, _I, _I, _P, _P]),
+    "skf_attention_key_scan_bytes": (_Z, [_I]),
+    "skf_attention_key_scan": (_I, [_P, _I, _I, _P, _I, _P, _P]),
+    "skf_attention_fwd_scanned": (_I, [_P, _I, _P, _I, _P, _I, _P, _I, _I, _I, _I, _I, _I, _I, _P, _I, _P, _I, _P, _P, _P]),
+    "skf_attention_bwd_scanned": (_I, [_P, _I, _P, _I, _P, _I, _P, _I, _P, _I, _P, _P, _I, _I, _I, _I, _I, _I, _I, _P, _I, _P, _I, _P, _I, _I, _P, _P, _P, _P]),
     "skf_attention_weights": (_I, [_P, _I, _P, _I, _P, _I, _I, _I, _I, _I, _I, _I, _P, _P]),
     "skf_attention_fwd_float_mask": (_I, [_P, _I, _P, _I, _P, _I, _P, C.c_long, C.c_long, C.c_long, _I, _I, _I, _I, _I, _P, _I, _P, _P]),
     "skf_row_mean": (_I, [_P, _P, C.c_long, _I, _I, _P, _P]),
diff --git a/sketchformer_amd/csrc/skf_attention.hip b/sketchformer_amd/csrc/skf_attention.hip
--- a/sketchformer_amd/csrc/skf_attention.hip
+++ b/sketchformer_amd/csrc/skf_attention.hip
@@ -25,9 +25,30 @@
   constexpr int LD = SPLIT ? 3 * KPP / 4 : DH + 4;
   extern __shared__ __attribute__((aligned(16))) float smem[];
   int bh = skf_xcd_remap(blockIdx.x, gridDim.x);
-  if (p.order) { const int k = skf_deal_rank(blockIdx.x, p.H); bh = min(max(p.order[k / p.H], 0), p.B - 1) * p.H + k % p.H; }
+  const int nkt = (p.Lk + 15) >> 4, nqt = (p.Lq + 15) >> 4;
+  constexpr bool SCAN = SPLIT && MAXT <= 13;
+  bool pre = false;
+  int pre_lastk = -1;
+  unsigned pre_key0 = 0u, k_masked = 0u, pre_kb[7] = {0u, 0u, 0u, 0u, 0u, 0u, 0u};
+  if constexpr (SCAN) {
+    typedef const __attribute__((address_space(4))) unsigned* const_u32p;
+    typedef const __attribute__((address_space(4))) int* const_i32p;
+    if (p.scan) {
+      const int k = skf_deal_rank(blockIdx.x, p.H);
+      const const_u32p rp = (const_u32p)(p.scan + k / p.H);
+      bh = min(max((int)rp[0], 0), p.B - 1) * p.H + k % p.H;
+      pre_lastk = min((int)rp[1], p.Lk - 1); pre_key0 = rp[2]; k_masked = rp[3];
+#pragma unroll
+      for (int j = 0; j < 7; ++j) pre_kb[j] = rp[4 + j];
+      pre = true;
+    } else if (!p.key_mask) {
+      if (p.order) { const int k = skf_deal_rank(blockIdx.x, p.H); bh = min(max(((const_i32p)p.order)[k / p.H], 0), p.B - 1) * p.H + k % p.H; }
+      pre_lastk = p.Lk - 1; pre_key0 = 1u; k_masked = (p.Lk & 15) ? 1u << (nkt - 1) : 0u;
+      pre = true;
+    }
+  }
+  if (!pre && p.order) { const int k = skf_deal_rank(blockIdx.x, p.H); bh = min(max(p.order[k / p.H], 0), p.B - 1) * p.H + k % p.H; }
   const int b = bh / p.H, h = bh % p.H;
-  const int nkt = (p.Lk + 15) >> 4, nqt = (p.Lq + 15) >> 4;
   const int VP = nkt * 16 + 8;
   float* Ks = smem;
   float* Vt = smem + nkt * 16 * LD;
@@ -54,9 +75,12 @@
   const int last_key = p.Lk - 1;
   const unsigned char* kmp = p.key_mask ? p.key_mask + (size_t)b * p.key_mask_ld
                                         : reinterpret_cast<const unsigned char*>(p.K + (size_t)b * p.Lk * p.ldk);
-  const unsigned char mk0 = kmp[min(tid, last_key)];
+  unsigned char mk0 = 0;
+  if (!pre) mk0 = kmp[min(tid, last_key)];
+  bool can_skip = p.causal && pre_key0 != 0u;
+  int nkt_eff = (pre && pre_lastk >= 0 && (!p.causal || can_skip)) ? (pre_lastk >> 4) + 1 : nkt;
   constexpr int SB = 4;
-  const int stage_total = nkt * 16 * (DH / 4);
+  const int stage_total = nkt_eff * 16 * (DH / 4);
   for (int e0 = tid; e0 < stage_total; e0 += 256 * SB) {
     float4 kvb[SB], vvb[SB];
 #pragma unroll
@@ -85,7 +109,14 @@
       Vt[(c4 + 0) * VP + row] = vv.x; Vt[(c4 + 1) * VP + row] = vv.y; Vt[(c4 + 2) * VP + row] = vv.z; Vt[(c4 + 3) * VP + row] = vv.w;
     }
   }
-  {
+  if (pre) {
+    if (tid < nkt * 16) {
+      unsigned dw = pre_kb[0];
+#pragma unroll
+      for (int j = 1; j < 7; ++j) dw = (tid >> 5) == j ? pre_kb[j] : dw;
+      Ms[tid] = tid < p.Lk ? (((dw >> (tid & 31)) & 1u) ? -1e9f : 0.f) : -INFINITY;
+    }
+  } else {
     int lv = -1;
     auto mask_keys = [&](int key0 , unsigned char mb) {
       const int key = key0 + lane;
@@ -104,9 +135,16 @@
   }
   __syncthreads();
 
-  const bool can_skip = p.causal && Ms[0] == 0.f;
-  const int lastk = max(max(last_valid[0], last_valid[1]), max(last_valid[2], last_valid[3]));
-  const int nkt_eff = (lastk >= 0 && (!p.causal || can_skip)) ? (lastk >> 4) + 1 : nkt;
+  if (!pre) {
+    can_skip = p.causal && Ms[0] == 0.f;
+    const int lastk = max(max(last_valid[0], last_valid[1]), max(last_valid[2], last_valid[3]));
+    nkt_eff = (lastk >= 0 && (!p.causal || can_skip)) ? (lastk >> 4) + 1 : nkt;
+    if constexpr (SCAN) {
+#pragma unroll
+      for (int t = 0; t < MAXT; ++t) k_masked |= (t < nkt && Tf[t] != 0) ? 1u << t : 0u;
+      k_masked = __builtin_amdgcn_readfirstlane(k_masked);
+    }
+  }
   const float c2 = 1.44269504088896340736f / sqrtf((float)DH);
 
   const char* kp = reinterpret_cast<const char*>(Ks);
@@ -163,7 +201,9 @@
             acc = mfma16(kf.w, qf[c].w, acc);
           }
         }
-        const bool need_mask = __builtin_amdgcn_readfirstlane(Tf[kt]) != 0 || (p.causal && kt >= qt);
+        bool need_mask = p.causal && kt >= qt;
+        if constexpr (SCAN) need_mask = need_mask || ((k_masked >> kt) & 1u) != 0u;
+        else need_mask = need_mask || __builtin_amdgcn_readfirstlane(Tf[kt]) != 0;
         if (need_mask) {
           const float4 m4 = *reinterpret_cast<const float4*>(&Ms[kt * 16 + g * 4]);
           const float mr[4] = {m4.x, m4.y, m4.z, m4.w};
@@ -540,8 +580,18 @@
 extern "C" int skf_attention_fwd_ordered(const float* Q, int ldq, const float* K, int ldk, const float* V, int ldv,
                                          const unsigned char* key_mask, int key_mask_ld, int causal, int B, int H, int Lq, int Lk,
                                          int dh, float* O, int ldo, float* stats, int precision, const int* sample_order, skf_stream_t stream) {
+  return skf_attention_fwd_scanned(Q, ldq, K, ldk, V, ldv, key_mask, key_mask_ld, causal, B, H, Lq, Lk, dh, O, ldo, stats, precision, sample_order,
+                                   nullptr, stream);
+}
+
+extern "C" int skf_attention_fwd_scanned(const float* Q, int ldq, const float* K, int ldk, const float* V, int ldv,
+                                         const unsigned char* key_mask, int key_mask_ld, int causal, int B, int H, int Lq, int Lk,
+                                         int dh, float* O, int ldo, float* stats, int precision, const int* sample_order, const void* key_scan,
+                                         skf_stream_t stream) {
   AttnParams p{};
   p.order = (B & 7) == 0 ? sample_order : nullptr;
+  SKF_CHECK_ARG(!key_scan || (sample_order && key_mask), "a key-scan table belongs to a key mask and a sample order");
+  p.scan = (p.order && dh == 16 && Lk <= kKeyScanMaxLk && fwd_split(dh, precision)) ? static_cast<const SkfKeyScan*>(key_scan) : nullptr;
   p.Q = Q; p.K = K; p.V = V; p.O = O; p.ldq = ldq; p.ldk = ldk; p.ldv = ldv; p.ldo = ldo;
   p.key_mask = key_mask; p.key_mask_ld = key_mask_ld; p.causal = causal; p.B = B; p.H = H; p.Lq = Lq; p.Lk = Lk; p.stats = stats;
   int rc = check_common(p, dh);
@@ -598,10 +648,21 @@
                                          const unsigned char* key_mask, int key_mask_ld, int causal, int B, int H, int Lq, int Lk,
                                          int dh, float* dQ, int lddq, float* dK, int lddk, float* dV, int lddv, int precision,
                                          const int* q_live_len, const int* sample_order, skf_stream_t stream) {
+  return skf_attention_bwd_scanned(Q, ldq, K, ldk, V, ldv, O, ldo, dO, lddo, stats, key_mask, key_mask_ld, causal, B, H, Lq, Lk, dh, dQ, lddq,
+                                   dK, lddk, dV, lddv, precision, q_live_len, sample_order, nullptr, stream);
+}
+
+extern "C" int skf_attention_bwd_scanned(const float* Q, int ldq, const float* K, int ldk, const float* V, int ldv,
+                                         const float* O, int ldo, const float* dO, int lddo, const float* stats,
+                                         const unsigned char* key_mask, int key_mask_ld, int causal, int B, int H, int Lq, int Lk,
+                                         int dh, float* dQ, int lddq, float* dK, int lddk, float* dV, int lddv, int precision,
+                                         const int* q_live_len, const int* sample_order, const void* key_scan, skf_stream_t stream) {
   const bool two_pass = (precision & SKF_ATTN_TWO_PASS) != 0;
   precision &= ~SKF_ATTN_TWO_PASS;
   AttnParams p{};
   p.order = (B & 7) == 0 ? sample_order : nullptr;
+  SKF_CHECK_ARG(!key_scan || (sample_order && key_mask), "a key-scan table belongs to a key mask and a sample order");
+  p.scan = p.order ? static_cast<const SkfKeyScan*>(key_scan) : nullptr;
   p.q_live = q_live_len;
   p.Q = Q; p.K = K; p.V = V; p.O = const_cast<float*>(O); p.ldq = ldq; p.ldk = ldk; p.ldv = ldv; p.ldo = ldo;
   p.key_mask = key_mask; p.key_mask_ld = key_mask_ld; p.causal = causal; p.B = B; p.H = H; p.Lq = Lq; p.Lk = Lk;
diff --git a/sketchformer_amd/csrc/skf_attention_bwd3.hip b/sketchformer_amd/csrc/skf_attention_bwd3.hip
--- a/sketchformer_amd/csrc/skf_attention_bwd3.hip
+++ b/sketchformer_amd/csrc/skf_attention_bwd3.hip
@@ -15,7 +15,7 @@
 constexpr int PB = RMAX * RP;
 constexpr int K_OFF = 0, V_OFF = 3 * PB, Q_OFF = 6 * PB, G_OFF = 9 * PB;
 constexpr int NMX_OFF = 12 * PB, NDL_OFF = NMX_OFF + RMAX * 4, KBITS_OFF = NDL_OFF + RMAX * 4, CTL_OFF = KBITS_OFF + 16 * 4;
-constexpr int SMEM_BYTES = CTL_OFF + 16 + 32;
+constexpr int SMEM_BYTES = CTL_OFF + 16 + 32 + 32;
 constexpr float kLog2e = 1.44269504088896340736f, kLn2 = 0.69314718055994530942f;
 
 __device__ __forceinline__ f32x4 mfma_x(b3_u32x4 a, b3_u32x4 b, f32x4 c) {
@@ -84,6 +84,7 @@
   unsigned* Kbits = reinterpret_cast<unsigned*>(smem + KBITS_OFF);
   int* ctl = reinterpret_cast<int*>(smem + CTL_OFF);
   int* kscan = ctl + 4;
+  int* qlw = kscan + 8;
   const SkfSplitSel sel = skf_split_sel();
   const int tid = threadIdx.x, lane = tid & 63;
   const int wave = __builtin_amdgcn_readfirstlane(tid >> 6);
@@ -91,23 +92,50 @@
   const bool first = g < 2;
   const float c2 = kLog2e * 0.25f;
   int bh = skf_xcd_remap(blockIdx.x, gridDim.x);
-  if (p.order) { const int k = skf_deal_rank(blockIdx.x, p.H); bh = min(max(p.order[k / p.H], 0), p.B - 1) * p.H + k % p.H; }
+  typedef const __attribute__((address_space(4))) unsigned* const_u32p;
+  typedef const __attribute__((address_space(4))) int* const_i32p;
+  const bool pre = p.scan != nullptr || p.key_mask == nullptr;
+  unsigned k_masked = (p.Lk & 15) ? 1u << (nkt - 1) : 0u;
+  int lastk = p.Lk - 1;
+  bool key0_open = true;
+  if (pre) {
+    unsigned kb[7] = {0u, 0u, 0u, 0u, 0u, 0u, 0u};
+    if (p.scan) {
+      const int k = skf_deal_rank(blockIdx.x, p.H);
+      const const_u32p rp = (const_u32p)(p.scan + k / p.H);
+      bh = min(max((int)rp[0], 0), p.B - 1) * p.H + k % p.H;
+      lastk = min((int)rp[1], p.Lk - 1); key0_open = rp[2] != 0u; k_masked = rp[3];
+#pragma unroll
+      for (int t = 0; t < 7; ++t) kb[t] = rp[4 + t];
+    } else if (p.order) {
+      const int k = skf_deal_rank(blockIdx.x, p.H);
+      bh = min(max(((const_i32p)p.order)[k / p.H], 0), p.B - 1) * p.H + k % p.H;
+    }
+    if (tid < 16) {
+      unsigned dw = kb[0];
+#pragma unroll
+      for (int t = 1; t < 7; ++t) dw = (tid >> 1) == t ? kb[t] : dw;
+      Kbits[tid] = tid < MAXT ? (dw >> (16 * (tid & 1))) & 0xffffu : 0u;
+    }
+  } else if (p.order) { const int k = skf_deal_rank(blockIdx.x, p.H); bh = min(max(p.order[k / p.H], 0), p.B - 1) * p.H + k % p.H; }
   const int b = bh / p.H, h = bh % p.H;
-  const int nqt = p.q_live ? min(nqt_all, (max(p.q_live[b], 0) + 15) >> 4) : nqt_all;
-  const unsigned char mb = p.key_mask ? p.key_mask[(size_t)b * p.key_mask_ld + min(tid, p.Lk - 1)] : (unsigned char)0;
-  if (tid == 256) { ctl[1] = 0; ctl[2] = 8; }
-  if (wave < 4) {
-    const unsigned long long padded = __ballot(tid < p.Lk && mb != 0), open = __ballot(tid < p.Lk && mb == 0);
-    const unsigned word = (unsigned)(padded >> (16 * (lane & 3))) & 0xffffu;
-    if (lane < 4) Kbits[4 * wave + lane] = word;
-    const unsigned tiles = (unsigned)__ballot(lane < 4 && word != 0u);
-    if (lane == 0) { kscan[wave] = (int)(tiles << (4 * wave)); kscan[4 + wave] = open ? 64 * wave + 63 - __builtin_clzll(open) : -1; }
-  }
-  __syncthreads();
-  const b3_u32x4 kw = *reinterpret_cast<const b3_u32x4*>(kscan), lw = *reinterpret_cast<const b3_u32x4*>(kscan + 4);
-  const unsigned k_masked = __builtin_amdgcn_readfirstlane((kw[0] | kw[1]) | (kw[2] | kw[3])) | ((p.Lk & 15) ? 1u << (nkt - 1) : 0u);
-  const int lastk = __builtin_amdgcn_readfirstlane(max(max((int)lw[0], (int)lw[1]), max((int)lw[2], (int)lw[3])));
-  const bool can_skip = CAUSAL && !(Kbits[0] & 1u);
+  const int nqt = p.q_live ? min(nqt_all, (max(pre ? ((const_i32p)p.q_live)[b] : p.q_live[b], 0) + 15) >> 4) : nqt_all;
+  if (!pre) {
+    const unsigned char mb = p.key_mask[(size_t)b * p.key_mask_ld + min(tid, p.Lk - 1)];
+    if (wave < 4) {
+      const unsigned long long padded = __ballot(tid < p.Lk && mb != 0), open = __ballot(tid < p.Lk && mb == 0);
+      const unsigned word = (unsigned)(padded >> (16 * (lane & 3))) & 0xffffu;
+      if (lane < 4) Kbits[4 * wave + lane] = word;
+      const unsigned tiles = (unsigned)__ballot(lane < 4 && word != 0u);
+      if (lane == 0) { kscan[wave] = (int)(tiles << (4 * wave)); kscan[4 + wave] = open ? 64 * wave + 63 - __builtin_clzll(open) : -1; }
+    }
+    __syncthreads();
+    const b3_u32x4 kw = *reinterpret_cast<const b3_u32x4*>(kscan), lw = *reinterpret_cast<const b3_u32x4*>(kscan + 4);
+    k_masked |= __builtin_amdgcn_readfirstlane((kw[0] | kw[1]) | (kw[2] | kw[3]));
+    lastk = __builtin_amdgcn_readfirstlane(max(max((int)lw[0], (int)lw[1]), max((int)lw[2], (int)lw[3])));
+    key0_open = !(Kbits[0] & 1u);
+  }
+  const bool can_skip = CAUSAL && key0_open;
   const int nkt_eff = (lastk >= 0 && (!CAUSAL || can_skip)) ? (lastk >> 4) + 1 : nkt;
   float4 kv[2], vv[2], qv[2], gv[2], ov[2];
   float2 sv[2];
@@ -136,12 +164,17 @@
       }
     }
   }
-#pragma unroll
-  for (int u = 0; u < 2; ++u) {
-    const int e = tid + 512 * u, row = e >> 2;
-    const bool nz = row < p.Lq && (gv[u].x != 0.f || gv[u].y != 0.f || gv[u].z != 0.f || gv[u].w != 0.f);
-    if (__ballot(nz) != 0ull && lane == 0 && (e >> 6) < nqt) atomicOr(reinterpret_cast<unsigned*>(&ctl[1]), 1u << (e >> 6));
-  }
+  {
+    unsigned mine = 0u;
+#pragma unroll
+    for (int u = 0; u < 2; ++u) {
+      const int e = tid + 512 * u, row = e >> 2;
+      const bool nz = row < p.Lq && (gv[u].x != 0.f || gv[u].y != 0.f || gv[u].z != 0.f || gv[u].w != 0.f);
+      if (__ballot(nz) != 0ull && (e >> 6) < nqt) mine |= 1u << (e >> 6);
+    }
+    if (lane == 0) qlw[wave] = (int)mine;
+  }
+  if (tid == 256) ctl[2] = 8;
 #pragma unroll
   for (int u = 0; u < 2; ++u) {
     const int e = tid + 512 * u, row = e >> 2, c4 = (e & 3) * 4;
@@ -171,7 +204,8 @@
     }
   }
   __syncthreads();
-  const unsigned q_live = (unsigned)ctl[1];
+  const b3_u32x4 ql0 = *reinterpret_cast<const b3_u32x4*>(qlw), ql1 = *reinterpret_cast<const b3_u32x4*>(qlw + 4);
+  const unsigned q_live = __builtin_amdgcn_readfirstlane(((ql0[0] | ql0[1]) | (ql0[2] | ql0[3])) | ((ql1[0] | ql1[1]) | (ql1[2] | ql1[3])));
 
   const int nA = nqt, nB = nkt_eff, nm = nA < nB ? nA : nB, n_items = nA + nB;
   const int lane_d = j * RP + (g & 1) * 16;
diff --git a/sketchformer_amd/csrc/skf_attention_params.h b/sketchformer_amd/csrc/skf_attention_params.h
--- a/sketchformer_amd/csrc/skf_attention_params.h
+++ b/sketchformer_amd/csrc/skf_attention_params.h
@@ -1,5 +1,16 @@
 #pragma once
 #include "skf_common.h"
+
+struct SkfKeyScan {
+  int b;
+  int lastk;
+  unsigned key0_open;
+  unsigned k_masked;
+  unsigned kbits[7];
+  unsigned reserved[5];
+};
+static_assert(sizeof(SkfKeyScan) == 64, "one record = 16 dwords");
+constexpr int kKeyScanMaxLk = 208;
 
 struct AttnParams {
   const float* Q; const float* K; const float* V; float* O;
@@ -14,6 +25,7 @@
   int lddq, lddk, lddv;
   const int* order;
   const int* q_live;
+  const SkfKeyScan* scan;
 };
 
 constexpr size_t kAttnLdsBytes = 160 * 1024;
diff --git a/sketchformer_amd/csrc/skf_common.h b/sketchformer_amd/csrc/skf_common.h
--- a/sketchformer_amd/csrc/skf_common.h
+++ b/sketchformer_amd/csrc/skf_common.h
@@ -59,6 +59,8 @@
 int skf_stage_inputs_launch(const void* inp, void* dinp, const void* tar, void* dtar, size_t row, size_t src_row, size_t copy, int batch,
                             const void* labels, void* dlabels, hipStream_t st, unsigned char* emask = nullptr, unsigned char* dmask = nullptr,
                             int mask_L = 0);
+int skf_attention_key_scan_pair(const unsigned char* mask_a, int lda, int La, void* scan_a, const unsigned char* mask_b, int ldb, int Lb,
+                                void* scan_b, const int* sample_order, int B, hipStream_t stream);
 int skf_counts_to_offsets_launch(const int* counts, int N, long long* out_offsets, hipStream_t stream);
 
 static inline int skf_cdiv(long a, long b) { return (int)((a + b - 1) / b); }
diff --git a/sketchformer_amd/csrc/skf_model_bwd.hip b/sketchformer_amd/csrc/skf_model_bwd.hip
--- a/sketchformer_amd/csrc/skf_model_bwd.hip
+++ b/sketchformer_amd/csrc/skf_model_bwd.hip
@@ -196,9 +196,9 @@
     SKF_TRY(M->sched.before_write(M, dq2, s));
     SKF_TRY(M->sched.before_write(M, dkv2, s));
     const int* qlive = M->ctx.live_lengths(Md);
-    SKF_TRY(skf_attention_bwd_ordered(M->at<float>(a.q2), d, kv2, 2 * d, kv2 + d, 2 * d, M->at<float>(a.o2), d, dO, d,
+    SKF_TRY(skf_attention_bwd_scanned(M->at<float>(a.q2), d, kv2, 2 * d, kv2 + d, 2 * d, M->at<float>(a.o2), d, dO, d,
                                       M->at<float>(a.astats2), cross_mask, Le, 0, B, H, Ld, Le, dh, dq2, d, dkv2, 2 * d,
-                                      dkv2 + d, 2 * d, M->cfg.gemm_precision, qlive, M->ctx.order, s));
+                                      dkv2 + d, 2 * d, M->cfg.gemm_precision, qlive, M->ctx.order, cross_mask ? M->ctx.key_scan[0] : nullptr, s));
     SKF_TRY(dense_wgrad(M, w.mha2.q, M->at<float>(a.out1), d, dq2, d, Md, s));
     const bool lead = row_owner_takes_ln(M, w.ln1, ln_oproj_partial_bytes(M, Md), Md, &w.mha1.o, &w.mha2.q);
     if (!lead) SKF_TRY(dense_dgrad(M, w.mha2.q, dq2, d, Md, G, d, 1, nullptr, 0, s));
@@ -211,9 +211,9 @@
                          site_dec(N, i, 0), s, M->at<char>(a.img_o1), lead ? dq2 : nullptr, lead ? M->at<char>(a.img_q2t) : nullptr));
     const float* qkv = M->at<float>(a.qkv);
     SKF_TRY(M->sched.before_write(M, dqkv, s));
-    SKF_TRY(skf_attention_bwd_ordered(qkv, 3 * d, qkv + d, 3 * d, qkv + 2 * d, 3 * d, M->at<float>(a.o1), d, dO, d,
+    SKF_TRY(skf_attention_bwd_scanned(qkv, 3 * d, qkv + d, 3 * d, qkv + 2 * d, 3 * d, M->at<float>(a.o1), d, dO, d,
                                       M->at<float>(a.astats1), dmask, Ld, 1, B, H, Ld, Ld, dh, dqkv, 3 * d, dqkv + d, 3 * d,
-                                      dqkv + 2 * d, 3 * d, M->cfg.gemm_precision, qlive, M->ctx.order, s));
+                                      dqkv + 2 * d, 3 * d, M->cfg.gemm_precision, qlive, M->ctx.order, M->ctx.key_scan[1], s));
     SKF_TRY(dense_wgrad(M, w.mha1.qkv, M->at<float>(a.x_in), d, dqkv, 3 * d, Md, s));
     const bool hold = M->ctx.ffn_fused && i > 0;
     hipEvent_t ready = nullptr;
@@ -330,9 +330,9 @@
     }
     const float* qkv = M->at<float>(a.qkv);
     SKF_TRY(M->sched.before_write(M, dqkv, s));
-    SKF_TRY(skf_attention_bwd_ordered(qkv, 3 * d, qkv + d, 3 * d, qkv + 2 * d, 3 * d, M->at<float>(a.o), d, dO, d,
+    SKF_TRY(skf_attention_bwd_scanned(qkv, 3 * d, qkv + d, 3 * d, qkv + 2 * d, 3 * d, M->at<float>(a.o), d, dO, d,
                                       M->at<float>(a.astats), emask, Le, 0, B, H, Le, Le, dh, dqkv, 3 * d, dqkv + d, 3 * d,
-                                      dqkv + 2 * d, 3 * d, M->cfg.gemm_precision, nullptr, M->ctx.order, s));
+                                      dqkv + 2 * d, 3 * d, M->cfg.gemm_precision, nullptr, M->ctx.order, M->ctx.key_scan[0], s));
     SKF_TRY(dense_wgrad(M, w.mha.qkv, M->at<float>(a.x_in), d, dqkv, 3 * d, Me, s));
     if (i == 0) SKF_TRY(M->sched.issue(M, s, nullptr, !M->sched.holding()));
     SKF_TRY(dense_dgrad(M, w.mha.qkv, dqkv, 3 * d, Me, G, d, 1, nullptr, 0, s));
diff --git a/sketchformer_amd/csrc/skf_model_fwd.hip b/sketchformer_amd/csrc/skf_model_fwd.hip
--- a/sketchformer_amd/csrc/skf_model_fwd.hip
+++ b/sketchformer_amd/csrc/skf_model_fwd.hip
@@ -136,6 +136,13 @@
     SKF_TRY(skf_sample_order(emask, Le, Le, encoder_only ? nullptr : dmask, Ld, Ld, B, M->at<int>(P.order), s));
     M->ctx.order = M->at<int>(P.order);
   }
+  M->ctx.key_scan[0] = M->ctx.key_scan[1] = nullptr;
+  if (M->ctx.order && c.d_model / c.num_heads == 16 && Le <= 208 && (B & 7) == 0) {
+    SKF_TRY(skf_attention_key_scan_pair(emask, Le, Le, M->at<char>(P.key_scan[0]), encoder_only ? nullptr : dmask, Ld, Ld,
+                                        M->at<char>(P.key_scan[1]), M->ctx.order, B, s));
+    M->ctx.key_scan[0] = M->at<char>(P.key_scan[0]);
+    if (!encoder_only) M->ctx.key_scan[1] = M->at<char>(P.key_scan[1]);
+  }
   if (masks_ready) SKF_HIP(hipEventRecord(masks_ready, s));
   M->ctx.ffn_fused = ffn_fused_on(M);
   if (M->ctx.ffn_fused) SKF_TRY(build_ffn_images(M, with_backward, encoder_only, s));
@@ -174,8 +181,8 @@
     float* qkv = M->at<float>(a.qkv);
     if (!enc_qkv_done) SKF_TRY(dense_fwd(M, w.mha.qkv, x, Me, qkv, 0, s));
     if (i == 0 && images_ready) SKF_HIP(hipStreamWaitEvent(s, masks_ready, 0));
-    SKF_TRY(skf_attention_fwd_ordered(qkv, 3 * d, qkv + d, 3 * d, qkv + 2 * d, 3 * d, emask, Le, 0, B, H, Le, Le, dh,
-                                      M->at<float>(a.o), d, M->at<float>(a.astats), M->cfg.gemm_precision, order, s));
+    SKF_TRY(skf_attention_fwd_scanned(qkv, 3 * d, qkv + d, 3 * d, qkv + 2 * d, 3 * d, emask, Le, 0, B, H, Le, Le, dh,
+                                      M->at<float>(a.o), d, M->at<float>(a.astats), M->cfg.gemm_precision, order, M->ctx.key_scan[0], s));
     const bool has_next = i + 1 < N;
     if (i == 0 && images_ready) SKF_HIP(hipStreamWaitEvent(s, images_ready, 0));
     SKF_TRY(attn_tail_ffn_fwd(M, w.mha.o, w.ln1, M->at<float>(a.o), x, M->at<float>(a.z1), M->at<float>(a.x1), M->at<float>(a.st1),
@@ -248,8 +255,8 @@
     float* x = M->at<float>(a.x_in);
     float* qkv = M->at<float>(a.qkv);
     if (!dec_qkv_done) SKF_TRY(dense_fwd(M, w.mha1.qkv, x, Md, qkv, 0, s));
-    SKF_TRY(skf_attention_fwd_ordered(qkv, 3 * d, qkv + d, 3 * d, qkv + 2 * d, 3 * d, dmask, Ld, 1, B, H, Ld, Ld, dh,
-                                      M->at<float>(a.o1), d, M->at<float>(a.astats1), M->cfg.gemm_precision, order, s));
+    SKF_TRY(skf_attention_fwd_scanned(qkv, 3 * d, qkv + d, 3 * d, qkv + 2 * d, 3 * d, dmask, Ld, 1, B, H, Ld, Ld, dh,
+                                      M->at<float>(a.o1), d, M->at<float>(a.astats1), M->cfg.gemm_precision, order, M->ctx.key_scan[1], s));
     const bool tail_proj = M->ctx.ffn_fused && w.mha1.o.in == d && w.mha1.o.out == d && chains(M, w.mha2.q) && w.mha2.q.out == d &&
                            w.ln1.b == w.ln1.g + (size_t)d;
     if (tail_proj) {
@@ -269,8 +276,9 @@
     if (!kv_done) SKF_TRY(dense_fwd(M, w.mha2.kv, pre, Me, kv2, 0, s));
     else if (i == 0) SKF_HIP(hipStreamWaitEvent(s, kv_first, 0));
     else if (i == 1) SKF_HIP(hipStreamWaitEvent(s, kv_done, 0));
-    SKF_TRY(skf_attention_fwd_ordered(M->at<float>(a.q2), d, kv2, 2 * d, kv2 + d, 2 * d, cross_mask, Le, 0, B, H, Ld, Le, dh,
-                                      M->at<float>(a.o2), d, M->at<float>(a.astats2), M->cfg.gemm_precision, order, s));
+    SKF_TRY(skf_attention_fwd_scanned(M->at<float>(a.q2), d, kv2, 2 * d, kv2 + d, 2 * d, cross_mask, Le, 0, B, H, Ld, Le, dh,
+                                      M->at<float>(a.o2), d, M->at<float>(a.astats2), M->cfg.gemm_precision, order,
+                                      cross_mask ? M->ctx.key_scan[0] : nullptr, s));
     const bool has_next = i + 1 < N;
     SKF_TRY(attn_tail_ffn_fwd(M, w.mha2.o, w.ln2, M->at<float>(a.o2), M->at<float>(a.out1), M->at<float>(a.z2), M->at<float>(a.out2),
                               M->at<float>(a.st2), site_dec(N, i, 1), M->at<char>(a.img_o2f), w.f1, w.f2, w.ln3, M->at<float>(a.h),
diff --git a/sketchformer_amd/csrc/skf_model_internal.h b/sketchformer_amd/csrc/skf_model_internal.h
--- a/sketchformer_amd/csrc/skf_model_internal.h
+++ b/sketchformer_amd/csrc/skf_model_internal.h
@@ -65,6 +65,7 @@
   size_t bytes = 0;
   size_t inp, tar, labels, enc_mask, dec_mask;
   size_t order;
+  size_t key_scan[2] = {0, 0};
   std::vector<EncAct> enc;
   std::vector<DecAct> dec;
   size_t u, pool_a, emb, pooled, dpooled, cls_logits, cls_probs, pre, logits;
@@ -167,6 +168,7 @@
   const int* live_len = nullptr;
   struct LiveList { int granule; const int* blocks; } lists[2] = {};
   const int* order = nullptr;
+  const void* key_scan[2] = {nullptr, nullptr};
   hipEvent_t pre_ready = nullptr, masks_ready = nullptr;
   bool lists_built = false;
   bool masks_staged = false;
diff --git a/sketchformer_amd/csrc/skf_model_layout.hip b/sketchformer_amd/csrc/skf_model_layout.hip
--- a/sketchformer_amd/csrc/skf_model_layout.hip
+++ b/sketchformer_amd/csrc/skf_model_layout.hip
@@ -261,6 +261,7 @@
   P.dc_logits = b.take(B * Vout * f); P.dc_stats = b.take(B * 2 * f); P.dc_kvnew = b.take(B * 2 * d * f);
   P.live_len = b.take(B * sizeof(int));
   P.order = b.take(B * sizeof(int));
+  P.key_scan[0] = b.take(skf_attention_key_scan_bytes((int)B)); P.key_scan[1] = b.take(skf_attention_key_scan_bytes((int)B));
   P.live16 = b.take(skf_row_blocks_bytes(B * (L - 1), 16)); P.live32 = b.take(skf_row_blocks_bytes(B * (L - 1), 32));
   P.bytes = b.off;
   return P;
diff --git a/sketchformer_amd/csrc/skf_row_blocks.hip b/sketchformer_amd/csrc/skf_row_blocks.hip
--- a/sketchformer_amd/csrc/skf_row_blocks.hip
+++ b/sketchformer_amd/csrc/skf_row_blocks.hip
@@ -1,5 +1,6 @@
 #include "skf_common.h"
 #include "../../include/skf.h"
+#include "skf_attention_params.h"
 
 namespace {
 
@@ -139,6 +140,60 @@
   for (int b = tid; b < B; b += 1024) order[rank[b]] = b;
 }
 
+struct KeyScanJob { const unsigned char* mask; int ld, Lk; SkfKeyScan* scan; };
+__global__ __launch_bounds__(256) void key_scan_kernel(KeyScanJob j0, KeyScanJob j1, const int* __restrict__ order, int B) {
+  const KeyScanJob jb = blockIdx.y ? j1 : j0;
+  const unsigned char* __restrict__ mask = jb.mask;
+  SkfKeyScan* __restrict__ scan = jb.scan;
+  const int ld = jb.ld, Lk = jb.Lk;
+  const int lane = threadIdx.x & 63, pos = blockIdx.x * 4 + (threadIdx.x >> 6);
+  if (pos >= B) return;
+  const int b = min(max(order[pos], 0), B - 1);
+  const unsigned char* row = mask + (size_t)b * ld;
+  unsigned char mb[4];
+#pragma unroll
+  for (int w = 0; w < 4; ++w) mb[w] = row[min(64 * w + lane, Lk - 1)];
+  unsigned word[16];
+  int lastk = -1;
+#pragma unroll
+  for (int w = 0; w < 4; ++w) {
+    const int key = 64 * w + lane;
+    const unsigned long long padded = __ballot(key < Lk && mb[w] != 0), open = __ballot(key < Lk && mb[w] == 0);
+#pragma unroll
+    for (int l = 0; l < 4; ++l) word[4 * w + l] = (unsigned)(padded >> (16 * l)) & 0xffffu;
+    if (open) lastk = 64 * w + 63 - __builtin_clzll(open);
+  }
+  unsigned k_masked = (Lk & 15) ? 1u << (((Lk + 15) >> 4) - 1) : 0u;
+#pragma unroll
+  for (int t = 0; t < 13; ++t) k_masked |= word[t] ? 1u << t : 0u;
+  if (lane == 0) {
+    uint4* dst = reinterpret_cast<uint4*>(scan + pos);
+    dst[0] = make_uint4((unsigned)b, (unsigned)lastk, (word[0] & 1u) ^ 1u, k_masked);
+    dst[1] = make_uint4(word[0] | word[1] << 16, word[2] | word[3] << 16, word[4] | word[5] << 16, word[6] | word[7] << 16);
+    dst[2] = make_uint4(word[8] | word[9] << 16, word[10] | word[11] << 16, word[12], 0u);
+    dst[3] = make_uint4(0u, 0u, 0u, 0u);
+  }
+}
+
+}
+
+extern "C" size_t skf_attention_key_scan_bytes(int B) { return B > 0 ? (size_t)B * sizeof(SkfKeyScan) : 0; }
+
+int skf_attention_key_scan_pair(const unsigned char* mask_a, int lda, int La, void* scan_a, const unsigned char* mask_b, int ldb, int Lb,
+                                void* scan_b, const int* sample_order, int B, hipStream_t stream) {
+  SKF_CHECK_ARG(mask_a && sample_order && scan_a && B > 0 && (!mask_b || scan_b), "bad argument");
+  SKF_CHECK_ARG(La > 0 && La <= kKeyScanMaxLk && lda >= La && (!mask_b || (Lb > 0 && Lb <= kKeyScanMaxLk && ldb >= Lb)),
+                "bad mask shape (the table covers Lk <= 208)");
+  SKF_CHECK_ARG((((uintptr_t)scan_a | (uintptr_t)scan_b) & 15) == 0, "the table must be 16-byte aligned");
+  const KeyScanJob j0{mask_a, lda, La, static_cast<SkfKeyScan*>(scan_a)}, j1{mask_b, ldb, Lb, static_cast<SkfKeyScan*>(scan_b)};
+  hipLaunchKernelGGL(key_scan_kernel, dim3(skf_cdiv(B, 4), mask_b ? 2 : 1), dim3(256), 0, stream, j0, j1, sample_order, B);
+  SKF_LAUNCH_CHECK();
+  return SKF_OK;
+}
+
+extern "C" int skf_attention_key_scan(const unsigned char* key_mask, int key_mask_ld, int Lk, const int* sample_order, int B, void* scan,
+                                      skf_stream_t stream) {
+  return skf_attention_key_scan_pair(key_mask, key_mask_ld, Lk, scan, nullptr, 0, 0, nullptr, sample_order, B, (hipStream_t)stream);
 }
 
 extern "C" int skf_sample_order(const unsigned char* mask_a, int lda, int La, const unsigned char* mask_b, int ldb, int Lb, int B, int* order,
diff --git a/sketchformer_amd/ops.py b/sketchformer_amd/ops.py
--- a/sketchformer_amd/ops.py
+++ b/sketchformer_amd/ops.py
@@ -208,11 +208,24 @@
     return out
 
 
-def attention_fwd(q, k, v, num_heads, key_mask=None, causal=False, precision=None, sample_order=None):
+def attention_key_scan(key_mask, sample_order):
+    B, Lk = key_mask.shape
+    nbytes = _lib.load().skf_attention_key_scan_bytes(B)
+    out = torch.zeros(nbytes // 4, dtype=torch.int32, device=key_mask.device).view(B, 16)
+    _lib.call("skf_attention_key_scan", _p(key_mask), key_mask.stride(0), Lk, _p(sample_order), B, _p(out), _stream())
+    return out
+
+
+def attention_fwd(q, k, v, num_heads, key_mask=None, causal=False, precision=None, sample_order=None, key_scan=None):
     B, Lq, d = q.shape
     Lk = k.shape[1]
     o = torch.empty(B, Lq, d, dtype=torch.float32, device=q.device)
     stats = torch.empty(B, num_heads, Lq, 2, dtype=torch.float32, device=q.device)
+    if key_scan is not None:
+        _lib.call("skf_attention_fwd_scanned", _p(q), q.stride(1), _p(k), k.stride(1), _p(v), v.stride(1), _p(key_mask),
+                  key_mask.stride(0) if key_mask is not None else 0, int(causal), B, num_heads, Lq, Lk, d // num_heads,
+                  _p(o), o.stride(1), _p(stats), _prec(precision), _p(sample_order), _p(key_scan), _stream())
+        return o, stats
     _lib.call("skf_attention_fwd_ordered", _p(q), q.stride(1), _p(k), k.stride(1), _p(v), v.stride(1), _p(key_mask),
               key_mask.stride(0) if key_mask is not None else 0, int(causal), B, num_heads, Lq, Lk, d // num_heads,
               _p(o), o.stride(1), _p(stats), _prec(precision), _p(sample_order), _stream())
@@ -273,12 +286,19 @@
 
 
 def attention_bwd(q, k, v, o, do, stats, num_heads, key_mask=None, causal=False, precision=None, q_live_len=None, two_pass=False,
-                  sample_order=None):
+                  sample_order=None, key_scan=None):
     B, Lq, d = q.shape
     Lk = k.shape[1]
     dq = torch.full((B, Lq, d), float("nan"), dtype=torch.float32, device=q.device)
     dk = torch.empty(B, Lk, d, dtype=torch.float32, device=q.device)
     dv = torch.empty(B, Lk, d, dtype=torch.float32, device=q.device)
+    if key_scan is not None:
+        _lib.call("skf_attention_bwd_scanned", _p(q), q.stride(1), _p(k), k.stride(1), _p(v), v.stride(1), _p(o), o.stride(1),
+                  _p(do), do.stride(1), _p(stats), _p(key_mask), key_mask.stride(0) if key_mask is not None else 0,
+                  int(causal), B, num_heads, Lq, Lk, d // num_heads, _p(dq), dq.stride(1), _p(dk), dk.stride(1),
+                  _p(dv), dv.stride(1), _prec(precision) | (_lib.ATTN_TWO_PASS if two_pass else 0), _p(q_live_len), _p(sample_order),
+                  _p(key_scan), _stream())
+        return dq, dk, dv
     _lib.call("skf_attention_bwd_ordered", _p(q), q.stride(1), _p(k), k.stride(1), _p(v), v.stride(1), _p(o), o.stride(1),
               _p(do), do.stride(1), _p(stats), _p(key_mask), key_mask.stride(0) if key_mask is not None else 0,
               int(causal), B, num_heads, Lq, Lk, d // num_heads, _p(dq), dq.stride(1), _p(dk), dk.stride(1),
```

Result: no change. 7.269 million stroke-tokens/sec (-0.2%).
